# evfro/polara

Hardware: AMD Instinct MI355X
Metric: users scored/sec + SVD build time, ML-20M rank-50 PureSVD (higher is better)
Workload: dtype bf16x3

## Files before the change

include/polara_hip.h:

```cpp
#ifndef POLARA_HIP_H
#define POLARA_HIP_H

#include <stdint.h>

#ifdef __cplusplus
extern "C" {
#endif

#define PK_OK 0
#define PK_E_INVALID (-1)
#define PK_E_LAUNCH (-2)
#define PK_E_UNSUPPORTED (-3)
#define PK_E_NOCONV (-4)

#define PK_VAL_F32 0
#define PK_VAL_F64 1

const char *pk_last_error(void);
int pk_version(void);
int pk_set_option(const char *name, int32_t value, int32_t unset);
int pk_copy_to_host_async(void *stream, void *dst_host, const void *src_dev, int64_t bytes);
int pk_device_info(int device, char *name, int name_len, int *cu_count, int64_t *hbm_bytes);
int pk_warm_up(void);

// ... 5 lines not shown
                    const int32_t *indices_dev, const void *vals_dev, int val_kind,
                    const double *X_dev, int64_t ldx, int32_t nc,
                    double *out_dev, int64_t ldo, double *partial_dev );
int pk_spmm_csr_x(void *stream,
                  int64_t n_tasks, const int32_t *task_row_dev, const int64_t *task_begin_dev,
                  const int64_t *task_end_dev, const int32_t *task_slot_dev,
                  int64_t n_long, const int32_t *long_row_dev, const int32_t *long_slot_begin_dev,
                  const int32_t *long_slot_end_dev,
                  const int32_t *indices_dev, const void *vals_dev, int val_kind,
                  const void *X_dev, int x_kind, int64_t ldx, int32_t nc,
                  double *out_dev, int64_t ldo, double *partial_dev);
int pk_spmm_csr_ex(void *stream,
                   int64_t n_tasks, const int32_t *task_row_dev, const int64_t *task_begin_dev,
                   const int64_t *task_end_dev, const int32_t *task_slot_dev,
                   int64_t n_long, const int32_t *long_row_dev, const int32_t *long_slot_begin_dev,
                   const int32_t *long_slot_end_dev,
                   const int32_t *indices_dev, const void *vals_dev, int val_kind,
                   const void *X_dev, int x_kind, int64_t ldx, int32_t nc,
                   double *out_dev, int64_t ldo, double *partial_dev, int64_t row_base, int32_t accumulate,
                   int64_t x_rows );

int64_t pk_scan_work_bytes(int64_t n);
int pk_exclusive_scan_i32(void *stream, int64_t n, const int32_t *in_dev, int64_t *out_dev, void *work_dev);
int64_t pk_radix_work_bytes(int64_t n);
int pk_radix_sort_pairs(void *stream, int64_t n, int32_t key_bytes, void *keys_dev, uint32_t *vals_dev,
                        void *keys_tmp_dev, uint32_t *vals_tmp_dev, int32_t key_bits, void *work_dev,
                        int32_t *result_in_tmp);
int64_t pk_row_norm_order_work_bytes(int64_t n);
int pk_row_norm_order_f64(void *stream, int64_t n, int32_t K, const double *V_dev, int64_t ldv, int32_t *order_dev,
                          int32_t *rank_dev, double *V_sorted_dev, void *work_dev);
int64_t pk_coo_to_csr_work_bytes(int64_t nnz);
int pk_coo_to_csr(void *stream, int64_t nnz, const int64_t *rows_dev, const int64_t *cols_dev, int64_t idx_stride,
                  const void *vals_dev,
                  int val_kind, int64_t n_rows, int64_t n_cols, int64_t *indptr_dev, int32_t *indices_dev,
                  void *values_dev, int64_t *n_unique_dev, int32_t *err_dev, void *work_dev);
int64_t pk_csr_transpose_work_bytes(int64_t nnz);
int pk_csr_transpose(void *stream, int64_t n_rows, int64_t n_cols, int64_t nnz, const int64_t *indptr_dev,
                     const int32_t *indices_dev, const void *values_dev, int val_kind, int64_t rows_per_block,
                     int64_t *t_indptr_dev, int32_t *t_indices_dev, void *t_values_dev, void *work_dev);
int64_t pk_csr_relabel_work_bytes(int64_t nnz);
int pk_csr_relabel_sorted(void *stream, int64_t n_rows, int64_t n_cols, int64_t nnz, const int64_t *indptr_dev,
                          const int32_t *indices_dev, const void *values_dev, int val_kind, const int32_t *col_map_dev,
                          int32_t *indices_out_dev, void *values_out_dev, void *work_dev);
int64_t pk_csr_rows_by_length_work_bytes(int64_t n_rows);
int pk_csr_rows_by_length(void *stream, int64_t n_rows, int64_t nnz, const int64_t *indptr_dev, const int32_t *indices_dev,
                          const void *values_dev, int val_kind, int32_t *perm_out_dev, int64_t *new_indptr_dev,
                          int32_t *indices_out_dev, void *values_out_dev, void *work_dev);
int pk_count_i32(void *stream, int64_t n, const int32_t *keys_dev, int64_t n_bins, int32_t *counts_dev);
int pk_csr_scale_f64(void *stream, int64_t n_rows, const int64_t *indptr_dev, const int32_t *indices_dev, const void *vals_dev,
                     int val_kind, const double *row_scale_dev, const double *col_scale_dev, double *vals_out_dev);
int64_t pk_row_plan_work_bytes(int64_t n_rows);
int pk_row_plan_count(void *stream, int64_t n_rows, const int64_t *indptr_dev, int32_t split, int64_t *counts_dev,
                      void *work_dev);
int pk_row_plan_fill(void *stream, int64_t n_rows, const int64_t *indptr_dev, const void *work_dev,
                     int32_t *task_row_dev, int64_t *task_begin_dev, int64_t *task_end_dev, int32_t *task_slot_dev,
                     int32_t *long_row_dev, int32_t *long_slot_begin_dev, int32_t *long_slot_end_dev,
                     int64_t *row_first_task_dev, int64_t *row_long_index_dev);

int64_t pk_gram_work_bytes(int64_t n, int32_t la, int32_t lb);
int pk_gram_f64(void *stream, int64_t n, int32_t la, int32_t lb, const double *A_dev, int64_t lda,
                const double *B_dev, int64_t ldb, double *G_dev, int64_t ldg, void *work_dev);
int pk_tsmm_f64(void *stream, int64_t n, int32_t lin, int32_t lout, const double *X_dev, int64_t ldx,
                const double *C_dev, int64_t ldc, double *out_dev, int64_t ldo);
int pk_tsmm_sub_f64(void *stream, int64_t n, int32_t lin, int32_t lout, const double *X_dev, int64_t ldx,
                    const double *C_dev, int64_t ldc, const double *Z_dev, int64_t ldz, double *out_dev, int64_t ldo);
int pk_tsmm_axpby_f64(void *stream, int64_t n, int32_t lin, int32_t lout, const double *X_dev, int64_t ldx,
                      const double *C_dev, int64_t ldc, double alpha, double beta, const double *Z1_dev, int64_t ldz1,
                      double gamma, const double *Z2_dev, int64_t ldz2, double *out_dev, int64_t ldo);
int pk_orth_check_f64(void *stream, int32_t l, const double *G_dev, int64_t ldg, int32_t *info_dev, int32_t n_info,
                      double *flags_dev);
int pk_eigh_psd_f64(void *stream, int32_t n, double *S_dev, int64_t lds_, double *evecs_dev, int64_t ldv,
                    double *evals_dev, int32_t max_sweeps, double tol, int32_t *info_dev);
int pk_eigh_psd_rounds_f64(void *stream, int32_t n, double *S_dev, int64_t lds_, double *evecs_dev, int64_t ldv,
                           double *evals_dev, int32_t max_sweeps, double tol, int32_t *info_dev);
int pk_eigh_top_supported(int32_t n, int32_t r);
int64_t pk_eigh_top_work_bytes(int32_t n);
int pk_eigh_top_f64(void *stream, int32_t n, const double *S_dev, int64_t lds_, int32_t r, double *evecs_dev, int64_t ldv,
                    double *evals_dev, void *work_dev, int32_t *info_dev);
int64_t pk_chol_work_bytes(int32_t n);
int pk_chol_rinv_f64(void *stream, int32_t n, const double *G_dev, int64_t ldg, double shift_rel, double *Rinv_dev,
                     int64_t ldr, void *work_dev, int32_t *info_dev);
int pk_chol_rinv_scaled_f64(void *stream, int32_t n, const double *G_dev, int64_t ldg, double shift_rel, double *Rinv_dev,
                     int64_t ldr, void *work_dev, int32_t *info_dev);
int pk_axpbypcz_f64(void *stream, int64_t n_elems, double alpha, const double *Z_dev, double beta,
                    const double *Y_dev, double gamma, const double *X_dev, double *out_dev);
int32_t pk_resid_blocks(int64_t n);
int pk_resid_colnorm2_f64(void *stream, int64_t n, int32_t l, const double *Z_dev, int64_t ldz,
                          const double *X_dev, int64_t ldx, const double *theta_dev, double *partial_dev);
int pk_dgemm_small_f64(void *stream, int transA, int transB, int32_t M, int32_t N, int32_t K,
                       const double *A_dev, int64_t lda, const double *B_dev, int64_t ldb,
                       double *C_dev, int64_t ldc);
int pk_scale_cols_f64(void *stream, int64_t n, int32_t l, double *X_dev, int64_t ldx, const double *s_dev);

int64_t pk_pack_elems(int64_t n, int32_t K);
int32_t pk_pack_kq(int32_t K);
int pk_pack_frag_f32(void *stream, int64_t n, int32_t K, const double *src_dev, int64_t ld, float *dst_dev);
int32_t pk_candidate_capacity(int32_t topk);
int64_t pk_score_state_bytes(int64_t n_users, int32_t splits);
int32_t pk_score_splits(int64_t n_users, int32_t KC);
int pk_seen_tiles_build(void *stream, int64_t n_users, const int64_t *seen_ptr_dev, const int32_t *seen_idx_dev,
                        int32_t rows_sorted ,
                        int64_t max_row_len ,
                        uint64_t *tiles_dev, int32_t *ntiles_dev);
int32_t pk_seen_tiles_max_unsorted_row(void);
int pk_score_candidates_f32(void *stream, int64_t n_users, int64_t n_items, int32_t K,
                            const float *Vp_dev, const float *Ep_dev,
                            const int64_t *seen_ptr_dev, const uint64_t *seen_tiles_dev,
                            const int32_t *seen_ntiles_dev ,
                            int32_t KC, int32_t splits ,
                            float *cand_score_dev, int32_t *cand_idx_dev ,
                            void *state_dev ,
                            int32_t tiles_per_chunk ,
                            const float *user_bound_dev ,
                            const float *tile_bound_dev ,
                            const uint32_t *seen_dense_dev, const int32_t *seen_skip_dev,
                            int32_t dense_tiles );
int pk_sweep_takes_rows(void);
int pk_score_candidates_rows_f32(void *stream, int64_t n_users, int64_t n_items, int32_t K, const float *Vp_dev,
                                 const double *E_dev, int64_t lde, const double *extra_dev, int64_t extra_ld,
                                 double extra_scale, const int64_t *seen_ptr_dev, const uint64_t *seen_tiles_dev,
                                 const int32_t *seen_ntiles_dev, int32_t KC, int32_t splits, float *cand_score_dev,
                                 int32_t *cand_idx_dev, void *state_dev, int32_t tiles_per_chunk ,
                                 const float *tile_bound_dev , const uint32_t *seen_dense_dev,
                                 const int32_t *seen_skip_dev, int32_t dense_tiles);
int pk_score_two_phase_plan(int64_t n_users, int64_t n_items, int32_t KC, int32_t *head_tiles, int32_t *splits);
int pk_score_two_phase_f32(void *stream, int64_t n_users, int64_t n_items, int32_t K,
                           const float *Vp_dev, const float *Ep_dev,
                           const int64_t *seen_ptr_dev, const uint64_t *seen_tiles_dev, const int32_t *seen_ntiles_dev,
                           int32_t KC, int32_t head_tiles, int32_t splits ,
                           float *work_score_dev, int32_t *work_idx_dev, float *cand_score_dev, int32_t *cand_idx_dev,
                           void *state_dev, int32_t tiles_per_chunk ,
                           const float *user_bound_dev, const float *tile_bound_dev ,
                           const uint32_t *seen_dense_dev, const int32_t *seen_skip_dev, int32_t dense_tiles);
int pk_score_two_phase_rows_f32(void *stream, int64_t n_users, int64_t n_items, int32_t K, const float *Vp_dev,
                                const double *E_dev, int64_t lde, const double *extra_dev, int64_t extra_ld,
                                double extra_scale, const int64_t *seen_ptr_dev, const uint64_t *seen_tiles_dev,
                                const int32_t *seen_ntiles_dev, int32_t KC, int32_t head_tiles, int32_t splits,
                                float *work_score_dev, int32_t *work_idx_dev, float *cand_score_dev, int32_t *cand_idx_dev,
                                void *state_dev, int32_t tiles_per_chunk, const float *tile_bound_dev,
                                const uint32_t *seen_dense_dev, const int32_t *seen_skip_dev, int32_t dense_tiles);
int64_t pk_seen_dense_bytes(int64_t n_users, int32_t dense_tiles);
int pk_seen_dense_build(void *stream, int64_t n_users, const int64_t *seen_ptr_dev, const uint64_t *seen_tiles_dev,
                        const int32_t *seen_ntiles_dev, int32_t dense_tiles, uint32_t *dense_dev, int32_t *skip_dev);
int32_t pk_score_chunk_launches(int64_t n_items, int32_t K, int32_t splits, int32_t tiles_per_chunk, int32_t pruned);
int pk_row_norm_bound_f32(void *stream, int64_t n, int32_t K, const double *src_dev, int64_t ld, float *out_dev);
int pk_v32_image_f32(void *stream, int64_t n, int32_t K, int32_t ld32, const double *V_dev, int64_t ldv, const float *bound_dev,
                     float *out_dev, uint32_t *stat_dev);
int pk_pack_frag_bound_f32(void *stream, int64_t n, int32_t K, const double *src_dev, int64_t ld, float *dst_dev,
                           float *bound_dev, const double *extra_dev, int64_t extra_ld, double extra_scale);
int pk_tile_norm_bound_f32(void *stream, int64_t n_items, int32_t K, const double *V_dev, int64_t ld,
                           float *work_dev, float *out_dev);
int pk_rescore_topk_f64(void *stream, int64_t n_users, int64_t n_items, int32_t K,
                        const double *V_dev, int64_t ldv, const double *E_dev, int64_t lde,
                        const int64_t *seen_ptr_dev, int32_t KC, int32_t splits,
                        const float *cand_score_dev, const int32_t *cand_idx_dev, int32_t topk,
                        double v_row_norm_max,
                        int64_t *out_idx_dev, double *out_score_dev , int32_t *flags_dev);
int pk_rescore_topk_rows_f64(void *stream, int64_t n_rows, const int32_t *rows_dev,
                             const int32_t *n_rows_dev ,
                             int64_t n_users, int64_t n_items,
                             int32_t K, const double *V_dev, int64_t ldv,
                             const float *V32_dev , int64_t ldv32,
                             const double *E_dev, int64_t lde,
                             const double *e_err_dev, int64_t e_err_ld ,
                             int32_t e_exact ,
                             const int64_t *seen_ptr_dev, int32_t KC, int32_t splits,
// ... 212 lines not shown
```

polara_amd/_lib.py:

```python
import ctypes as C
import os

_HERE = os.path.dirname(os.path.abspath(__file__))
LIB_PATH = os.environ.get('POLARA_HIP_LIB') or os.path.join(_HERE, 'libpolarahip.so')

PK_VAL_F32, PK_VAL_F64 = 0, 1

_vp, _i32, _i64, _f64 = C.c_void_p, C.c_int32, C.c_int64, C.c_double

PROTOTYPES = {
    'pk_last_error': (C.c_char_p, []),
    'pk_version': (C.c_int, []),
    'pk_warm_up': (C.c_int, []),
    'pk_device_info': (C.c_int, [C.c_int, C.c_char_p, C.c_int, C.POINTER(C.c_int), C.POINTER(_i64)]),
    'pk_spmm_csr_f64': (C.c_int, [_vp, _i64, _vp, _vp, _vp, _vp, _i64, _vp, _vp, _vp, _vp, _vp, C.c_int,
                                  _vp, _i64, _i32, _vp, _i64, _vp]),
    'pk_spmm_csr_x': (C.c_int, [_vp, _i64, _vp, _vp, _vp, _vp, _i64, _vp, _vp, _vp, _vp, _vp, C.c_int,
                                _vp, C.c_int, _i64, _i32, _vp, _i64, _vp]),
    'pk_spmm_csr_ex': (C.c_int, [_vp, _i64, _vp, _vp, _vp, _vp, _i64, _vp, _vp, _vp, _vp, _vp, C.c_int,
                                 _vp, C.c_int, _i64, _i32, _vp, _i64, _vp, _i64, _i32, _i64]),
    'pk_scan_work_bytes': (_i64, [_i64]),
    'pk_exclusive_scan_i32': (C.c_int, [_vp, _i64, _vp, _vp, _vp]),
    'pk_radix_work_bytes': (_i64, [_i64]),
    'pk_radix_sort_pairs': (C.c_int, [_vp, _i64, _i32, _vp, _vp, _vp, _vp, _i32, _vp, C.POINTER(_i32)]),
# ... 45 lines not shown
                                              _vp, _vp, _vp, _vp, _vp, _i32, _vp, _vp, _vp, _i32]),
    'pk_score_two_phase_plan': (C.c_int, [_i64, _i64, _i32, _vp, _vp]),
    'pk_score_two_phase_f32': (C.c_int, [_vp, _i64, _i64, _i32, _vp, _vp, _vp, _vp, _vp, _i32, _i32, _i32, _vp, _vp, _vp, _vp, _vp,
                                         _i32, _vp, _vp, _vp, _vp, _i32]),
    'pk_seen_dense_bytes': (_i64, [_i64, _i32]),
    'pk_seen_dense_build': (C.c_int, [_vp, _i64, _vp, _vp, _vp, _i32, _vp, _vp]),
    'pk_score_chunk_launches': (_i32, [_i64, _i32, _i32, _i32, _i32]),
    'pk_pack_frag_bound_f32': (C.c_int, [_vp, _i64, _i32, _vp, _i64, _vp, _vp, _vp, _i64, _f64]),
    'pk_row_norm_bound_f32': (C.c_int, [_vp, _i64, _i32, _vp, _i64, _vp]),
    'pk_tile_norm_bound_f32': (C.c_int, [_vp, _i64, _i32, _vp, _i64, _vp, _vp]),
    'pk_rescore_topk_f64': (C.c_int, [_vp, _i64, _i64, _i32, _vp, _i64, _vp, _i64, _vp, _i32, _i32, _vp, _vp,
                                      _i32, _f64, _vp, _vp, _vp]),
    'pk_flag_compact': (C.c_int, [_vp, _i64, _vp, _i32, _vp, _vp]),
    'pk_fold_rows_f64': (C.c_int, [_vp, _i64, _vp, _vp, _i64, _vp, _vp, _vp, C.c_int, _vp, _i64, _i32, _vp, _i64]),
    'pk_spmm_csr_flagged_f64': (C.c_int, [_vp, _i64, _vp, _vp, _vp, _vp, _i64, _vp, _vp, _vp, _vp, _vp, C.c_int, _vp, _i64, _i32,
                                          _vp, _i64, _vp, _i64, _vp, _i32]),
    'pk_spmm_csr_rows_list_f64': (C.c_int, [_vp, _i64, _vp, _vp, _i64, _vp, _vp, _vp, _vp, _vp, _i64, _vp, _vp, _vp, _vp, _vp, C.c_int,
                                            _vp, _i64, _i32, _vp, _i64, _vp, _i64, _vp, _i32]),
    'pk_q20_lanes': (_i32, [_i32]),
    'pk_q20_kappa': (_f64, [_i32]),
    'pk_q20_image_bytes': (_i64, [_i64, _i32]),
    'pk_q20_encode_f64': (C.c_int, [_vp, _i64, _i32, _vp, _i64, _vp, _vp, _vp, _vp]),
    'pk_q20_decode_f64': (C.c_int, [_vp, _i64, _i32, _vp, _vp, _vp, _i64]),
    'pk_fold_q20': (C.c_int, [_vp, _i64, _vp, _vp, _vp, _vp, _i64, _vp, _vp, _vp, _vp, _vp, C.c_int, _vp, _vp, _i64, _i32, _i32,
                              _vp, _i64, _vp]),
    'pk_rescore_topk_rows_f64': (C.c_int, [_vp, _i64, _vp, _vp, _i64, _i64, _i32, _vp, _i64, _vp, _i64, _vp, _i64, _vp, _i64, _i32, _vp, _i32, _i32,
                                           _vp, _vp, _i32, _f64, _vp, _vp, _vp]),
    'pk_rescore_topk_rows_list_f64': (C.c_int, [_vp, _i64, _vp, _vp, _i64, _i64, _i32, _vp, _i64, _vp, _i64, _vp, _i64, _vp, _i64, _i32, _vp, _i32, _i32,
                                           _vp, _vp, _i32, _f64, _vp, _vp, _vp, _vp, _vp, _i32]),
    'pk_rescore_topk_rows_norms_f64': (C.c_int, [_vp, _i64, _vp, _vp, _i64, _i64, _i32, _vp, _i64, _vp, _i64, _vp, _i64, _vp, _i64, _i32, _vp, _i32, _i32,
                                           _vp, _vp, _i32, _f64, _vp, _vp, _vp, _vp, _vp, _i32, _vp]),
    'pk_zero_i32': (C.c_int, [_vp, _vp, _i32]),
    'pk_scatter_rows_i64': (C.c_int, [_vp, _i64, _i32, _vp, _vp, _vp]),
    'pk_map_ids_i64': (C.c_int, [_vp, _i64, _vp, _vp, _i64, _vp]),
    'pk_exact_work_bytes': (_i64, [_i32, _i64]),
    'pk_score_exact_rows_f64': (C.c_int, [_vp, _i32, _vp, _i64, _i32, _vp, _i64, _vp, _i64, _vp, _vp, _i32,
                                          _vp, _vp, _vp]),
    'pk_score_exact_list_f64': (C.c_int, [_vp, _i32, _vp, _vp, _i64, _i32, _vp, _i64, _vp, _i64, _vp, _vp, _i32,
                                          _vp, _vp, _vp]),
    'pk_eval_ranks': (C.c_int, [_vp, _i64, _vp, _i32, _vp, _vp, _vp]),
    'pk_eval_cols': (_i32, []),
    'pk_eval_user_metrics': (C.c_int, [_vp, _i64, _i32, _vp, _i64, _vp, _vp, _vp, _vp, _f64, _f64, _i32, _vp]),
    'pk_eval_reduce_work_bytes': (_i64, [_i64]),
    'pk_eval_reduce': (C.c_int, [_vp, _i64, _vp, _vp, _vp]),
    'pk_unique_count_i64': (C.c_int, [_vp, _i64, _vp, _i64, _vp, _vp]),
    'pk_dense_scores_f64': (C.c_int, [_vp, _i32, _i64, _i32, _vp, _i64, _vp, _i64, _vp, _i64]),
    'pk_topk_rows_f64': (C.c_int, [_vp, _i64, _i64, _vp, _i64, _i32, _vp]),
    'pk_i2i_max_topk': (_i32, []),
    'pk_i2i_window': (_i32, []),
    'pk_i2i_build_window': (_i32, []),
    'pk_i2i_ld': (_i64, [_i64]),
    'pk_i2i_chunk_users': (_i64, [_i64, _i64, _i32]),
    'pk_i2i_topk_work_bytes': (_i64, [_i64, _i64, _i32]),
    'pk_i2i_build_f64': (C.c_int, [_vp, _i64, _i64, _vp, _vp, _vp, C.c_int, _vp, _vp, _vp, _vp, _i64]),
    'pk_i2i_image_f32': (C.c_int, [_vp, _i64, _vp, _vp, _vp]),
    'pk_i2i_topk': (C.c_int, [_vp, _i64, _i64, _vp, _vp, _vp, C.c_int, _vp, C.c_int, _i64, _i32, _i32, _i32, _vp, _vp, _vp]),
    'pk_popular_order_work_bytes': (_i64, [_i64]),
    'pk_popular_order': (C.c_int, [_vp, _i64, _vp, _vp, _vp]),
    'pk_popular_topk': (C.c_int, [_vp, _i64, _i64, _vp, _vp, _vp, _i32, _i32, _vp]),
    'pk_hybrid_ld': (_i64, [_i64]),
    'pk_hybrid_max_nc': (_i32, []),
    'pk_trmm_work_bytes': (_i64, [_i64, _i32]),
    'pk_hybrid_densify_f64': (C.c_int, [_vp, _i64, _vp, _vp, _vp, _vp, _f64, _vp, _i64]),
    'pk_chol_f64': (C.c_int, [_vp, _i64, _vp, _i64, _vp]),
    'pk_trmm_f64': (C.c_int, [_vp, _i32, _i64, _i32, _vp, _i64, _vp, _i64, _vp, _i64, _vp]),
    'pk_trsm_f64': (C.c_int, [_vp, _i64, _i32, _vp, _i64, _vp, _i64]),
    'pk_lce_fused_max_rank': (_i32, []),
    'pk_lce_update_f64': (C.c_int, [_vp, _i64, _i32, _vp, _i64, _vp, _i64, _vp, _i64, _f64, _vp, _i64, _f64, _f64, _f64, _vp]),
    'pk_lce_update_ew_f64': (C.c_int, [_vp, _i64, _i32, _vp, _i64, _vp, _i64, _vp, _i64, _f64, _f64, _vp]),
    'pk_lce_dot_blocks': (_i32, [_i64]),
    'pk_lce_dots_work_bytes': (_i64, []),
    'pk_lce_dots_f64': (C.c_int, [_vp, _i32, _vp, _vp, _vp, _vp, _vp, _vp, _vp, _vp, _f64, _vp, _vp]),
    'pk_clamp_min_f64': (C.c_int, [_vp, _i64, _i32, _vp, _i64, _f64]),
    'pk_ctx_create': (C.c_int, [_i32, C.POINTER(_vp)]),
    'pk_ctx_destroy': (None, [_vp]),
    'pk_ctx_error': (C.c_char_p, [_vp]),
    'pk_mat_from_csr': (C.c_int, [_vp, _i64, _i64, _i64, _vp, _vp, _vp, _i32, C.POINTER(_vp)]),
    'pk_mat_from_coo': (C.c_int, [_vp, _i64, _i64, _i64, _vp, _vp, _i64, _vp, _i32, C.POINTER(_vp)]),
    'pk_mat_free': (None, [_vp, _vp]),
    'pk_mat_nnz': (_i64, [_vp]),
    'pk_svd_build': (C.c_int, [_vp, _vp, _i32, _i32, _f64, _i32, C.c_uint64, _vp, _vp, _vp, _vp]),
    'pk_sym_eig_topk_f64': (C.c_int, [_vp, _vp, _i32, _vp, _i64, _i32, _i32, _vp, _i64, _i32, _f64, _i32, C.c_uint64,
                                      _vp, _i64, _vp, _vp, _vp, _vp, _f64]),
    'pk_svd_build_sharded': (C.c_int, [_vp, _vp, _vp, _i32, _i32, _f64, _i32, C.c_uint64, _vp, _vp, _vp, _vp]),
    'pk_ctx_stream': (_vp, [_vp]),
    'pk_ctx_set_option': (C.c_int, [_vp, C.c_char_p, _i32]),
    'pk_set_option': (C.c_int, [C.c_char_p, _i32, _i32]),
    'pk_copy_to_host_async': (C.c_int, [_vp, _vp, _vp, _i64]),
    'pk_v32_image_f32': (C.c_int, [_vp, _i64, _i32, _i32, _vp, _i64, _vp, _vp, _vp]),
    'pk_row_norm_order_work_bytes': (_i64, [_i64]),
    'pk_row_norm_order_f64': (C.c_int, [_vp, _i64, _i32, _vp, _i64, _vp, _vp, _vp, _vp]),
    'pk_sweep_takes_rows': (C.c_int, []),
    'pk_ctx_spmm_timings': (_i64, [_vp, _vp, _vp, _i64]),
    'pk_mat_wrap_device': (C.c_int, [_vp, _vp, _i64, _i64, _i64, _vp, _vp, _vp, _i32, _i32, C.POINTER(_vp)]),
    'pk_lanczos_steps': (C.c_int, [_vp, _vp, _vp, _i32, _i32, _i32, _i32, _vp, _i64, _vp, _i64, _vp, _vp, _i32]),
    'pk_gramian_apply_f64': (C.c_int, [_vp, _vp, _vp, _i32, _vp, _i64, _vp, _i64]),
    'pk_lanczos_products': (C.c_int, [_vp, _vp, _vp, _i32, _i32, _vp, _i64, _vp, _i32]),
    'pk_lanczos_orth': (C.c_int, [_vp, _vp, _i64, _i32, _i32, _i32, _vp, _i64, _vp, _i64, _vp, _vp, _vp, _i32]),
    'pk_score_topk': (C.c_int, [_vp, _i64, _i32, _vp, _vp, _i32, _i32, _vp, _vp]),
    'pk_serving_create': (C.c_int, [_vp, _i64, _i32, _vp, _vp, C.POINTER(_vp)]),
    'pk_serving_score': (C.c_int, [_vp, _vp, _i32, _i32, _vp, _vp]),
    'pk_serving_free': (None, [_vp, _vp]),
    'pk_hooi': (C.c_int, [_vp, _i64, _vp, _vp, _vp, _vp, _i32, _f64, _vp, _vp, C.c_uint64, _vp, _vp, _vp, _vp, _vp, _vp]),
    'pk_ttm_f64': (C.c_int, [_vp, _i64, _vp, _vp, _vp, _vp, _i64, _vp, _vp, _vp, _vp, _vp, _vp,
                             _vp, _i64, _i32, _vp, _i64, _i32, _vp, _i64, _vp]),
    'pk_tucker_predict_f64': (C.c_int, [_vp, _i64, _vp, _vp, _vp, _i64, _vp, _i64, _vp, _i64, _vp, _i32, _i32, _i32, _i32, _vp, _vp]),
}


class PolaraHipError(RuntimeError):
    pass


_lib = None


def load():
    global _lib
    if _lib is not None:
        return _lib
    import torch
    if not os.path.exists(LIB_PATH):
        raise PolaraHipError(
            'libpolarahip.so is not built (%s). Run `python -m polara_amd.build_native` '
            '(needs hipcc; cross-compiles for gfx950 without a GPU). There is no CPU fallback.' % LIB_PATH)
    lib = C.CDLL(LIB_PATH)
    for name, (res, args) in PROTOTYPES.items():
        fn = getattr(lib, name)
        fn.restype = res
        fn.argtypes = args
    _lib = lib
    return lib


def check(rc, what='', lib=None, ctx=None):
    if rc != 0:
        lib = lib or load()
        msg = lib.pk_ctx_error(ctx) if ctx is not None else None
        msg = msg or lib.pk_last_error()
        raise PolaraHipError('%s failed (rc=%d): %s' % (what, rc, msg.decode() if msg else ''))


def device_info(device=0):
    lib = load()
    name = C.create_string_buffer(64)
    cu = C.c_int(0)
    mem = C.c_int64(0)
    n = lib.pk_device_info(device, name, 64, C.byref(cu), C.byref(mem))
    if n <= 0:
        check(n, 'pk_device_info')
    return dict(n_devices=n, arch=name.value.decode(), cu_count=cu.value, hbm_bytes=mem.value)
```

polara_amd/csrc/api.cpp:

```cpp
#include "pk_common.h"
#include <string.h>

static thread_local char g_err[512] = "";

void pk_set_error(const char *fmt, ...) {
    va_list ap;
    va_start(ap, fmt);
    vsnprintf(g_err, sizeof(g_err), fmt, ap);
    va_end(ap);
}

extern "C" const char *pk_last_error(void) { return g_err; }

#include <atomic>
namespace {
struct Option { const char *name; std::atomic<int> value; std::atomic<bool> set; };
Option g_options[] = {{"score_boot_tiles", {0}, {false}}, {"score_head_tiles", {0}, {false}}, {"score_phase2_splits", {0}, {false}}};
}
int pk_option(const char *name, int dflt) {
    for (auto &o : g_options)
        if (!strcmp(o.name, name)) return o.set.load() ? o.value.load() : dflt;
    return dflt;
}
extern "C" int pk_set_option(const char *name, int32_t value, int32_t unset) {
    if (name)
        for (auto &o : g_options)
            if (!strcmp(o.name, name)) {
                o.value.store(value);
                o.set.store(!unset);
                return PK_OK;
            }
    pk_set_error("pk_set_option: unknown option '%s'", name ? name : "(null)");
    return PK_E_INVALID;
}
extern "C" int pk_version(void) { return 100; }

extern "C" int pk_copy_to_host_async(void *stream, void *dst_host, const void *src_dev, int64_t bytes) {
    if (bytes < 0 || (bytes > 0 && (!dst_host || !src_dev))) {
        pk_set_error("pk_copy_to_host_async: bad arguments");
        return PK_E_INVALID;
    }
    if (bytes == 0) return PK_OK;
    const hipError_t e = hipMemcpyAsync(dst_host, src_dev, (size_t)bytes, hipMemcpyDeviceToHost, static_cast<hipStream_t>(stream));
    if (e != hipSuccess) {
        pk_set_error("pk_copy_to_host_async: %s", hipGetErrorString(e));
        return PK_E_LAUNCH;
    }
    return PK_OK;
}

extern "C" int pk_device_info(int device, char *name, int name_len, int *cu_count, int64_t *hbm_bytes) {
    int n = 0;
    hipError_t e = hipGetDeviceCount(&n);
    if (e != hipSuccess || n <= 0) {
        pk_set_error("pk_device_info: no HIP device visible (%s)", hipGetErrorString(e));
        return PK_E_LAUNCH;
    }
    if (device < 0 || device >= n) {
        pk_set_error("pk_device_info: device %d out of range [0,%d)", device, n);
        return PK_E_INVALID;
    }
    hipDeviceProp_t prop;
    e = hipGetDeviceProperties(&prop, device);
    if (e != hipSuccess) {
        pk_set_error("pk_device_info: %s", hipGetErrorString(e));
        return PK_E_LAUNCH;
    }
    if (name && name_len > 0) {
        strncpy(name, prop.gcnArchName, name_len - 1);
        name[name_len - 1] = 0;
    }
    if (cu_count) *cu_count = prop.multiProcessorCount;
    if (hbm_bytes) *hbm_bytes = (int64_t)prop.totalGlobalMem;
    return n;
}

hipError_t pk_tu_load_dense();
hipError_t pk_tu_load_driver();
hipError_t pk_tu_load_eigh();
hipError_t pk_tu_load_eigh_top();
hipError_t pk_tu_load_evalmetrics();
hipError_t pk_tu_load_hybrid();
hipError_t pk_tu_load_i2i();
hipError_t pk_tu_load_foldq();
hipError_t pk_tu_load_ingest();
hipError_t pk_tu_load_lce();
hipError_t pk_tu_load_rescore();
hipError_t pk_tu_load_score();
hipError_t pk_tu_load_spmm();
hipError_t pk_tu_load_ttm();

extern "C" int pk_warm_up(void) {
    hipError_t (*const loaders[])() = {pk_tu_load_dense, pk_tu_load_driver, pk_tu_load_eigh, pk_tu_load_eigh_top, pk_tu_load_evalmetrics, pk_tu_load_foldq, pk_tu_load_hybrid, pk_tu_load_i2i, pk_tu_load_ingest, pk_tu_load_lce, pk_tu_load_rescore, pk_tu_load_score, pk_tu_load_spmm, pk_tu_load_ttm};
    for (auto f : loaders) {
        const hipError_t e = f();
        if (e != hipSuccess) {
            pk_set_error("pk_warm_up: %s", hipGetErrorString(e));
            return PK_E_LAUNCH;
        }
    }
    return PK_OK;
}
```

polara_amd/csrc/dense.hip:

```cpp
#include "pk_common.h"

static int gram_splits(int64_t n, int la, int lb) {
    int64_t tiles = pk_ceil_div(la, 64) * pk_ceil_div(lb, 64);
    int64_t s = pk_ceil_div(tiles >= 4 ? 1024 : 2048, tiles);
    int64_t max_by_rows = pk_ceil_div(n, 64);
    if (s > max_by_rows) s = max_by_rows;
    if (s > 1024) s = 1024;
    if (n <= 64) s = 1;
    if (s < 1) s = 1;
    return (int)s;
}

extern "C" int64_t pk_gram_work_bytes(int64_t n, int32_t la, int32_t lb) {
    return (int64_t)gram_splits(n, la, lb) * la * lb * (int64_t)sizeof(double);
}

typedef double f64x4 __attribute__((ext_vector_type(4)));

__global__ __launch_bounds__(256) void gram_kernel(int64_t n, int la, int lb, const double *__restrict__ A,
                                                   int64_t lda, const double *__restrict__ B, int64_t ldb,
                                                   double *__restrict__ partial, int tiles_j,
                                                   int64_t rows_per_split) {
    constexpr int RT = 32;
    __shared__ __attribute__((aligned(16))) double sA[RT][64];
    __shared__ __attribute__((aligned(16))) double sB[RT][64];
    const int tid = threadIdx.x;
    const int lane = tid & 63, wave = tid >> 6;
    const int ti = blockIdx.x / tiles_j, tj = blockIdx.x % tiles_j;
    const int split = blockIdx.y;
    const int64_t r_begin = (int64_t)split * rows_per_split;
    int64_t r_end = r_begin + rows_per_split;
    if (r_end > n) r_end = n;
    const bool vec = ((lda | ldb) & 1) == 0 && ((((uintptr_t)A) | ((uintptr_t)B)) & 15) == 0 && (la & 1) == 0 && (lb & 1) == 0;
    f64x4 acc[4];
#pragma unroll
    for (int b = 0; b < 4; ++b) acc[b] = f64x4{0.0, 0.0, 0.0, 0.0};
    double2 ra[4], rb[4];
    auto fetch = [&](int64_t r0) {
#pragma unroll
        for (int q = 0; q < 4; ++q) {
            const int slot = tid + 256 * q;
            const int rr = slot >> 5, c = (slot & 31) * 2;
            const int64_t row = r0 + rr;
            const int ca = ti * 64 + c, cb = tj * 64 + c;
            double2 va = make_double2(0.0, 0.0), vb = make_double2(0.0, 0.0);
            if (row < r_end) {
                const double *pa = A + row * lda + ca, *pb = B + row * ldb + cb;
                if (vec && ca + 1 < la) va = *reinterpret_cast<const double2 *>(pa);
                else {
                    if (ca < la) va.x = pa[0];
                    if (ca + 1 < la) va.y = pa[1];
                }
                if (vec && cb + 1 < lb) vb = *reinterpret_cast<const double2 *>(pb);
                else {
                    if (cb < lb) vb.x = pb[0];
                    if (cb + 1 < lb) vb.y = pb[1];
                }
            }
            ra[q] = va;
            rb[q] = vb;
        }
    };
    if (r_begin < r_end) fetch(r_begin);
    for (int64_t r0 = r_begin; r0 < r_end; r0 += RT) {
#pragma unroll
        for (int q = 0; q < 4; ++q) {
            const int slot = tid + 256 * q;
            *reinterpret_cast<double2 *>(&sA[slot >> 5][(slot & 31) * 2]) = ra[q];
            *reinterpret_cast<double2 *>(&sB[slot >> 5][(slot & 31) * 2]) = rb[q];
        }
        __syncthreads();
        if (r0 + RT < r_end) fetch(r0 + RT);
#pragma unroll
        for (int k0 = 0; k0 < RT; k0 += 4) {
            const double p = sA[k0 + (lane >> 4)][16 * wave + (lane & 15)];
#pragma unroll
            for (int b = 0; b < 4; ++b)
                acc[b] = __builtin_amdgcn_mfma_f64_16x16x4f64(p, sB[k0 + (lane >> 4)][16 * b + (lane & 15)], acc[b], 0, 0, 0);
        }
        __syncthreads();
    }
    double *dst = partial + (int64_t)split * la * lb;
#pragma unroll
// ... 286 lines not shown
                acc = fma(d, d, acc);
            }
        }
        red[tid] = acc;
        __syncthreads();
        for (int s = nrl / 2; s > 0; s >>= 1) {
            if (rl < s) red[tid] += red[tid + s * cw];
            __syncthreads();
        }
        if (rl == 0 && j < l) partial[(int64_t)blockIdx.x * l + j] = red[tid];
        __syncthreads();
    }
}

extern "C" int pk_resid_colnorm2_f64(void *stream, int64_t n, int32_t l, const double *Z_dev, int64_t ldz,
                                     const double *X_dev, int64_t ldx, const double *theta_dev,
                                     double *partial_dev) {
    PK_REQUIRE(n >= 1 && l >= 1 && ldz >= l && ldx >= l, "pk_resid_colnorm2_f64: bad sizes");
    hipLaunchKernelGGL(resid_colnorm2_kernel, dim3((unsigned)pk_resid_blocks(n)), dim3(256), 0, pk_stream(stream),
                       n, l, Z_dev, ldz, X_dev, ldx, theta_dev, partial_dev);
    PK_CHECK_LAUNCH("resid_colnorm2_kernel");
    return PK_OK;
}

__global__ __launch_bounds__(256) void scale_cols_kernel(int64_t n, int l, double *__restrict__ X, int64_t ldx,
                                                         const double *__restrict__ s) {
    int64_t e = (int64_t)blockIdx.x * blockDim.x + threadIdx.x;
    const int64_t total = n * l, stride = (int64_t)gridDim.x * blockDim.x;
    for (; e < total; e += stride) {
        int64_t i = e / l;
        int j = (int)(e % l);
        X[i * ldx + j] *= s[j];
    }
}

extern "C" int pk_scale_cols_f64(void *stream, int64_t n, int32_t l, double *X_dev, int64_t ldx,
                                 const double *s_dev) {
    PK_REQUIRE(n >= 1 && l >= 1 && ldx >= l, "pk_scale_cols_f64: bad sizes");
    int64_t blocks = pk_ceil_div(n * l, 256);
    if (blocks > 8192) blocks = 8192;
    hipLaunchKernelGGL(scale_cols_kernel, dim3((unsigned)blocks), dim3(256), 0, pk_stream(stream), n, l, X_dev, ldx,
                       s_dev);
    PK_CHECK_LAUNCH("scale_cols_kernel");
    return PK_OK;
}

__global__ __launch_bounds__(256) void dgemm_small_kernel(int tA, int tB, int M, int N, int K,
                                                          const double *__restrict__ A, int64_t lda,
                                                          const double *__restrict__ B, int64_t ldb,
                                                          double *__restrict__ C, int64_t ldc) {
    int64_t e = (int64_t)blockIdx.x * blockDim.x + threadIdx.x;
    if (e >= (int64_t)M * N) return;
    const int i = (int)(e / N), j = (int)(e % N);
    double acc = 0.0;
    for (int k = 0; k < K; ++k) {
        double a = tA ? A[(int64_t)k * lda + i] : A[(int64_t)i * lda + k];
        double b = tB ? B[(int64_t)j * ldb + k] : B[(int64_t)k * ldb + j];
        acc = fma(a, b, acc);
    }
    C[(int64_t)i * ldc + j] = acc;
}

extern "C" int pk_dgemm_small_f64(void *stream, int transA, int transB, int32_t M, int32_t N, int32_t K,
                                  const double *A_dev, int64_t lda, const double *B_dev, int64_t ldb,
                                  double *C_dev, int64_t ldc) {
    PK_REQUIRE(M >= 1 && N >= 1 && K >= 1 && ldc >= N, "pk_dgemm_small_f64: bad sizes");
    hipLaunchKernelGGL(dgemm_small_kernel, dim3((unsigned)pk_ceil_div((int64_t)M * N, 256)), dim3(256), 0,
                       pk_stream(stream), transA, transB, M, N, K, A_dev, lda, B_dev, ldb, C_dev, ldc);
    PK_CHECK_LAUNCH("dgemm_small_kernel");
    return PK_OK;
}

#define PK_CHOL_LDS_MAX 136
#define PK_CHOL_THREADS 1024
template <bool IN_LDS, bool SCALED = false>
__global__ __launch_bounds__(PK_CHOL_THREADS) void chol_rinv_kernel(int n, const double *__restrict__ G, int64_t ldg,
                                                                    double shift_rel, double *__restrict__ Rinv,
                                                                    int64_t ldr, double *__restrict__ work,
                                                                    int32_t *__restrict__ info, int tx_log2) {
    extern __shared__ double chol_lds[];
    __shared__ double s_shift;
    double *A = IN_LDS ? chol_lds : work;
    const int ld = IN_LDS ? n + 1 : n;
    const int tid = threadIdx.x;
    const int TX = 1 << tx_log2, TY = (int)blockDim.x >> tx_log2;
    const int tx = tid & (TX - 1), ty = tid >> tx_log2;
    if (tid < 64) {
        double tr = 0.0;
        for (int i = tid; i < n; i += 64) tr += SCALED ? 1.0 : G[(int64_t)i * ldg + i];
        for (int o = 32; o > 0; o >>= 1) tr += __shfl_xor(tr, o);
        if (tid == 0) s_shift = shift_rel * tr;
    }
    __syncthreads();
    const double shift = s_shift;
    for (int i = ty; i < n; i += TY)
        for (int c = tx; c < n; c += TX) {
            double g = (c >= i) ? G[(int64_t)i * ldg + c] : 0.0;
            if constexpr (SCALED) {
                const double gi = G[(int64_t)i * ldg + i], gc = G[(int64_t)c * ldg + c];
                g = (c > i) ? g / (sqrt(gi) * sqrt(gc)) : (c == i ? (gi > 0.0 ? 1.0 : -1.0) : 0.0);
            }
            A[i * ld + c] = (c > i) ? g : (c == i ? g + shift : 0.0);
        }
    int fail = 0;
    for (int j = 0; j < n; ++j) {
        __syncthreads();
        const double d = A[j * ld + j];
        if (!(d > 0.0)) {
            fail = j + 1;
            break;
        }
        const double invd = 1.0 / d;
        for (int c = tx; c < n; c += TX) {
            const double pj = (c == j) ? 1.0 : A[j * ld + c];
            for (int i = j + 1 + ty; i < n; i += TY)
                if (c <= j || c >= i) {
                    const double f = A[j * ld + i] * invd;
                    A[i * ld + c] = fma(-f, pj, A[i * ld + c]);
                }
        }
    }
    __syncthreads();
    if (tid == 0) info[0] = fail;
    if (fail) return;
    for (int k = ty; k < n; k += TY)
        for (int c = tx; c < n; c += TX) {
            double v = 0.0;
            if (c >= k) {
                const double rs = 1.0 / sqrt(A[c * ld + c]);
                v = (c == k) ? rs : A[c * ld + k] * rs;
                if constexpr (SCALED) v /= sqrt(G[(int64_t)k * ldg + k]);
            }
            Rinv[(int64_t)k * ldr + c] = v;
        }
}

extern "C" int64_t pk_chol_work_bytes(int32_t n) { return (n > PK_CHOL_LDS_MAX) ? (int64_t)n * n * 8 : 0; }

static int chol_rinv_launch(void *stream, int32_t n, const double *G_dev, int64_t ldg, double shift_rel, double *Rinv_dev, int64_t ldr,
                            void *work_dev, int32_t *info_dev, bool scaled);

extern "C" int pk_chol_rinv_f64(void *stream, int32_t n, const double *G_dev, int64_t ldg, double shift_rel,
                                double *Rinv_dev, int64_t ldr, void *work_dev, int32_t *info_dev) {
    return chol_rinv_launch(stream, n, G_dev, ldg, shift_rel, Rinv_dev, ldr, work_dev, info_dev, false);
}

extern "C" int pk_chol_rinv_scaled_f64(void *stream, int32_t n, const double *G_dev, int64_t ldg, double shift_rel,
                                       double *Rinv_dev, int64_t ldr, void *work_dev, int32_t *info_dev) {
    return chol_rinv_launch(stream, n, G_dev, ldg, shift_rel, Rinv_dev, ldr, work_dev, info_dev, true);
}

static int chol_rinv_launch(void *stream, int32_t n, const double *G_dev, int64_t ldg, double shift_rel, double *Rinv_dev, int64_t ldr,
                            void *work_dev, int32_t *info_dev, bool scaled) {
    PK_REQUIRE(n >= 1 && n <= 1024 && ldg >= n && ldr >= n, "pk_chol_rinv_f64: bad sizes");
    PK_REQUIRE(G_dev && Rinv_dev && info_dev && (n <= PK_CHOL_LDS_MAX || work_dev), "pk_chol_rinv_f64: bad pointers");
    static PkDeviceOnce attr_set;   
    if (attr_set.pending()) {
        hipError_t e1 = hipFuncSetAttribute(reinterpret_cast<const void *>(&chol_rinv_kernel<true, false>),
                                            hipFuncAttributeMaxDynamicSharedMemorySize,
                                            PK_CHOL_LDS_MAX * (PK_CHOL_LDS_MAX + 1) * 8);
        if (e1 == hipSuccess)
            e1 = hipFuncSetAttribute(reinterpret_cast<const void *>(&chol_rinv_kernel<true, true>),
                                     hipFuncAttributeMaxDynamicSharedMemorySize, PK_CHOL_LDS_MAX * (PK_CHOL_LDS_MAX + 1) * 8);
        if (e1 != hipSuccess) {
            pk_set_error("pk_chol_rinv_f64: cannot raise the dynamic LDS limit: %s", hipGetErrorString(e1));
            return PK_E_LAUNCH;
        }
        attr_set.done();   
    }
    int tx_log2 = 4;
    while ((1 << tx_log2) < n && tx_log2 < 8) ++tx_log2;
    const int threads = PK_CHOL_THREADS;
#define PK_CHOL_LAUNCH(SC)                                                                                                   \
    do {                                                                                                                     \
        if (n <= PK_CHOL_LDS_MAX)                                                                                            \
            hipLaunchKernelGGL((chol_rinv_kernel<true, SC>), dim3(1), dim3(threads), (size_t)n * (n + 1) * sizeof(double),   \
                               pk_stream(stream), n, G_dev, ldg, shift_rel, Rinv_dev, ldr, static_cast<double *>(work_dev),  \
                               info_dev, tx_log2);                                                                           \
        else                                                                                                                 \
            hipLaunchKernelGGL((chol_rinv_kernel<false, SC>), dim3(1), dim3(PK_CHOL_THREADS), 0, pk_stream(stream), n, G_dev, \
                               ldg, shift_rel, Rinv_dev, ldr, static_cast<double *>(work_dev), info_dev, tx_log2);           \
    } while (0)
    if (scaled) PK_CHOL_LAUNCH(true); else PK_CHOL_LAUNCH(false);
#undef PK_CHOL_LAUNCH
    PK_CHECK_LAUNCH("chol_rinv_kernel");
    return PK_OK;
}

hipError_t pk_tu_load_dense() {
    hipFuncAttributes a;
    return hipFuncGetAttributes(&a, reinterpret_cast<const void *>(&gram_reduce_kernel));
}
```

polara_amd/csrc/driver.hip:

```cpp
#include "pk_common.h"
#include <algorithm>
#include <cmath>
#include <cstdarg>
#include <cstring>
#include <map>
#include <memory>
#include <mutex>
#include <numeric>
#include <random>
#include <string>
#include <type_traits>
#include <vector>

namespace model {
constexpr double kDenseF64Flops = 20e12;
constexpr double kLanczosStepFixedS = 0.3e-3;
constexpr double kNestedSolveS = 1.5e-3;
constexpr double kXgmiBusBps = 100e9;
constexpr double kCollectiveStepS = 5e-6;
}

struct DevPool {
    std::multimap<size_t, void *> free_blocks;
    void *get(size_t &bytes) {
        auto it = free_blocks.lower_bound(bytes);
        if (it != free_blocks.end() && it->first <= bytes + bytes / 4 + 4096) {
            void *p = it->second;
            bytes = it->first;
            free_blocks.erase(it);
            return p;
        }
        void *p = nullptr;
        if (hipMalloc(&p, bytes) != hipSuccess) {
            trim();
            if (hipMalloc(&p, bytes) != hipSuccess) return nullptr;
        }
        return p;
    }
    void put(void *p, size_t bytes) { free_blocks.emplace(bytes, p); }
    void trim() {
        for (auto &kv : free_blocks) (void)hipFree(kv.second);
        free_blocks.clear();
    }
};

struct CtxOptions {
    int svd_method = 0;
    int krylov_block = 0;
    int dist_overlap = 1;
    int hooi_ttm = 0;
    int time_spmm = 0;
};

struct SpmmTiming {
    hipEvent_t e0, e1;
    int64_t meta[6];
};

struct pk_ctx {
    int device = 0;
    hipStream_t stream = nullptr;
    std::mutex mu;
    std::string err;
    DevPool pool;
    CtxOptions opt;
    std::vector<SpmmTiming> spmm_timings;
    std::vector<hipEvent_t> event_pool;
};

static thread_local DevPool *g_pool = nullptr;
struct PoolScope {
    DevPool *prev;
    explicit PoolScope(pk_ctx *ctx) : prev(g_pool) { g_pool = &ctx->pool; }
    ~PoolScope() { g_pool = prev; }
};

namespace {

int fail(pk_ctx *ctx, int code, const char *fmt, ...) {
    char buf[512];
    va_list ap;
    va_start(ap, fmt);
    vsnprintf(buf, sizeof(buf), fmt, ap);
    va_end(ap);
    if (ctx) ctx->err = buf;
    pk_set_error("%s", buf);
    return code;
}
#define CK(call)                                                          \
    do {                                                                  \
        int rc_ = (call);                                                 \
        if (rc_ != PK_OK) {                                               \
            ctx->err = pk_last_error();                                   \
            return rc_;                                                   \
        }                                                                 \
    } while (0)
#define HIPCK(call)                                                                              \
    do {                                                                                         \
        hipError_t e_ = (call);                                                                  \
        if (e_ != hipSuccess) return fail(ctx, PK_E_LAUNCH, "%s: %s", #call, hipGetErrorString(e_)); \
    } while (0)

struct Dev {
    void *p = nullptr;
    size_t bytes = 0;
    size_t cap = 0;
    DevPool *pool = nullptr;
    bool borrowed = false;
    Dev() {}
    explicit Dev(size_t b) { alloc(b); }
    Dev(const Dev &) = delete;
    Dev &operator=(const Dev &) = delete;
    Dev(Dev &&o) noexcept : p(o.p), bytes(o.bytes), cap(o.cap), pool(o.pool), borrowed(o.borrowed) { o.p = nullptr; o.bytes = o.cap = 0; o.borrowed = false; }
    Dev &operator=(Dev &&o) noexcept {
        if (this != &o) {
            release();
            p = o.p; bytes = o.bytes; cap = o.cap; pool = o.pool; borrowed = o.borrowed; o.p = nullptr; o.bytes = o.cap = 0; o.borrowed = false;
        }
        return *this;
    }
    void borrow(const void *ptr, size_t b) {
        release();
        p = const_cast<void *>(ptr); bytes = b; cap = 0; pool = nullptr; borrowed = true;
    }
    ~Dev() { release(); }
    bool alloc(size_t b) {
        release();
        bytes = b;
        if (b == 0) return true;
        pool = g_pool;
        cap = ((b + 65535) / 65536) * 65536;
        if (pool) p = pool->get(cap);
        else if (hipMalloc(&p, cap) != hipSuccess) p = nullptr;
        if (!p) { bytes = cap = 0; return false; }
// ... 430 lines not shown
        const int nb = pk_resid_blocks(Z.n);
        Dev part((size_t)nb * Z.l * 8);
        if (!part.p) return fail(ctx, PK_E_LAUNCH, "out of device memory (resid)");
        CK(pk_resid_colnorm2_f64(st, Z.n, Z.l, Z.p(), Z.l, X.p(), X.l, theta_dev.as<double>(), part.as<double>()));
        std::vector<double> h((size_t)nb * Z.l);
        CK(to_host(part.p, h.data(), h.size() * 8));
        res.assign((size_t)Z.l, 0.0);
        for (int b = 0; b < nb; ++b)
            for (int j = 0; j < Z.l; ++j) res[(size_t)j] += h[(size_t)b * Z.l + j];
        for (auto &v : res) v = std::sqrt(std::max(v, 0.0));
        return PK_OK;
    }
};

int cheb_degree(double theta_top, double b, double spread, int m_max) {
    if (b <= 0.0) return 2;
    const double x_top = 2.0 * theta_top / b - 1.0;
    if (x_top <= 1.0 + 1e-12) return m_max;
    const int m = (int)(std::log(2.0 * spread) / std::acosh(x_top));
    return std::max(2, std::min(m_max, m));
}

int upload_csr(pk_ctx *ctx, Csr &M, int64_t n_rows, int64_t n_cols, int64_t nnz, const int64_t *indptr, const int32_t *indices,
               const void *values, int val_kind) {
    M.n_rows = n_rows; M.n_cols = n_cols; M.nnz = nnz; M.val_kind = val_kind;
    const size_t ve = val_kind == PK_VAL_F32 ? 4 : 8;
    if (!M.indptr.alloc((size_t)(n_rows + 1) * 8) || !M.indices.alloc((size_t)std::max<int64_t>(nnz, 1) * 4) ||
        !M.values.alloc((size_t)std::max<int64_t>(nnz, 1) * ve))
        return fail(ctx, PK_E_LAUNCH, "out of device memory (matrix)");
    HIPCK(hipMemcpyAsync(M.indptr.p, indptr, (size_t)(n_rows + 1) * 8, hipMemcpyHostToDevice, ctx->stream));
    if (nnz) {
        HIPCK(hipMemcpyAsync(M.indices.p, indices, (size_t)nnz * 4, hipMemcpyHostToDevice, ctx->stream));
        HIPCK(hipMemcpyAsync(M.values.p, values, (size_t)nnz * ve, hipMemcpyHostToDevice, ctx->stream));
    }
    HIPCK(hipStreamSynchronize(ctx->stream));
    return PK_OK;
}

}

extern "C" int pk_ctx_create(int32_t device, pk_ctx **out) {
    if (!out) return PK_E_INVALID;
    int n = 0;
    if (hipGetDeviceCount(&n) != hipSuccess || device < 0 || device >= n) {
        pk_set_error("pk_ctx_create: device %d not available (%d visible)", device, n);
        return PK_E_LAUNCH;
    }
    auto *ctx = new pk_ctx();
    ctx->device = device;
    if (hipSetDevice(device) != hipSuccess || hipStreamCreate(&ctx->stream) != hipSuccess) {
        delete ctx;
        pk_set_error("pk_ctx_create: cannot create a stream on device %d", device);
        return PK_E_LAUNCH;
    }
    if (pk_warm_up() != PK_OK) {
        (void)hipStreamDestroy(ctx->stream);
        delete ctx;
        return PK_E_LAUNCH;
    }
    *out = ctx;
    return PK_OK;
}

extern "C" void pk_ctx_destroy(pk_ctx *ctx) {
    if (!ctx) return;
    for (auto &t : ctx->spmm_timings) { (void)hipEventDestroy(t.e0); (void)hipEventDestroy(t.e1); }
    for (hipEvent_t e : ctx->event_pool) (void)hipEventDestroy(e);
    ctx->spmm_timings.clear();
    ctx->event_pool.clear();
    (void)hipSetDevice(ctx->device);
    (void)hipStreamSynchronize(ctx->stream);
    ctx->pool.trim();
    (void)hipStreamDestroy(ctx->stream);
    delete ctx;
}

extern "C" const char *pk_ctx_error(pk_ctx *ctx) { return ctx ? ctx->err.c_str() : "null context"; }

extern "C" int pk_ctx_set_option(pk_ctx *ctx, const char *name, int32_t value) {
    if (!ctx || !name) return PK_E_INVALID;
    std::lock_guard<std::mutex> lock(ctx->mu);
    struct { const char *name; int *slot; int lo, hi; } table[] = {
        {"svd_method", &ctx->opt.svd_method, 0, 2},   {"krylov_block", &ctx->opt.krylov_block, 0, 1024},
        {"dist_overlap", &ctx->opt.dist_overlap, 0, 2}, {"hooi_ttm", &ctx->opt.hooi_ttm, 0, 1}, {"time_spmm", &ctx->opt.time_spmm, 0, 1}};
    for (auto &e : table)
        if (!strcmp(name, e.name)) {
            if (value < e.lo || value > e.hi) return fail(ctx, PK_E_INVALID, "pk_ctx_set_option: %s takes %d..%d", name, e.lo, e.hi);
            *e.slot = value;
            return PK_OK;
        }
    return fail(ctx, PK_E_INVALID, "pk_ctx_set_option: unknown option '%s'", name);
}

extern "C" int64_t pk_ctx_spmm_timings(pk_ctx *ctx, double *ms_out, int64_t *meta_out, int64_t cap) {
    if (!ctx) return -1;
    std::lock_guard<std::mutex> lock(ctx->mu);
    (void)hipSetDevice(ctx->device);
    const int64_t count = (int64_t)ctx->spmm_timings.size();
    for (int64_t i = 0; i < count; ++i) {
        SpmmTiming &t = ctx->spmm_timings[(size_t)i];
        float ms = 0.f;
        (void)hipEventSynchronize(t.e1);
        (void)hipEventElapsedTime(&ms, t.e0, t.e1);
        if (i < cap && ms_out && meta_out) {
            ms_out[i] = (double)ms;
            for (int q = 0; q < 6; ++q) meta_out[6 * i + q] = t.meta[q];
        }
        ctx->event_pool.push_back(t.e0);
        ctx->event_pool.push_back(t.e1);
    }
    ctx->spmm_timings.clear();
    return count;
}

extern "C" int pk_mat_from_csr(pk_ctx *ctx, int64_t n_rows, int64_t n_cols, int64_t nnz, const int64_t *indptr,
                               const int32_t *indices, const void *values, int32_t val_kind, pk_mat **out) {
    if (!ctx || !out) return PK_E_INVALID;
    std::lock_guard<std::mutex> lock(ctx->mu);
    PoolScope pool_scope(ctx);
    (void)hipSetDevice(ctx->device);
    if (n_rows < 1 || n_cols < 1 || nnz < 0 || !indptr || (nnz && (!indices || !values)) ||
        (val_kind != PK_VAL_F32 && val_kind != PK_VAL_F64))
        return fail(ctx, PK_E_INVALID, "pk_mat_from_csr: bad arguments");
    if (indptr[0] != 0 || indptr[n_rows] != nnz) return fail(ctx, PK_E_INVALID, "pk_mat_from_csr: indptr does not span [0, nnz]");
    for (int64_t p = 0; p < nnz; ++p)
        if (indices[p] < 0 || indices[p] >= n_cols) return fail(ctx, PK_E_INVALID, "pk_mat_from_csr: column index out of bounds");
    auto m = std::make_unique<pk_mat>();
    int rc = upload_csr(ctx, m->A, n_rows, n_cols, nnz, indptr, indices, values, val_kind);
    if (rc != PK_OK) return rc;
    m->nonneg = true;
    if (val_kind == PK_VAL_F32) { const float *v = static_cast<const float *>(values); for (int64_t p = 0; p < nnz; ++p) if (v[p] < 0) { m->nonneg = false; break; } }
    else { const double *v = static_cast<const double *>(values); for (int64_t p = 0; p < nnz; ++p) if (v[p] < 0) { m->nonneg = false; break; } }
    rc = build_plan(ctx, m->A);
    if (rc != PK_OK) return rc;
    *out = m.release();
    return PK_OK;
}

static int mat_from_coo_impl(pk_ctx *ctx, int64_t n_rows, int64_t n_cols, int64_t nnz, const int64_t *rows, const int64_t *cols,
                             int64_t idx_stride, const void *values, int32_t val_kind, pk_mat **out);

extern "C" int pk_mat_from_coo(pk_ctx *ctx, int64_t n_rows, int64_t n_cols, int64_t nnz, const int64_t *rows, const int64_t *cols,
                               int64_t idx_stride, const void *values, int32_t val_kind, pk_mat **out) {
    if (!ctx || !out) return PK_E_INVALID;
    std::lock_guard<std::mutex> lock(ctx->mu);
    PoolScope pool_scope(ctx);
    (void)hipSetDevice(ctx->device);
    return mat_from_coo_impl(ctx, n_rows, n_cols, nnz, rows, cols, idx_stride, values, val_kind, out);
}

static int mat_from_coo_impl(pk_ctx *ctx, int64_t n_rows, int64_t n_cols, int64_t nnz, const int64_t *rows, const int64_t *cols,
                             int64_t idx_stride, const void *values, int32_t val_kind, pk_mat **out) {
    if (n_rows < 1 || n_cols < 1 || nnz < 0 || idx_stride < 1 || (nnz && (!rows || !cols || !values)) ||
        (val_kind != PK_VAL_F32 && val_kind != PK_VAL_F64))
        return fail(ctx, PK_E_INVALID, "pk_mat_from_coo: bad arguments");
    hipStream_t st = ctx->stream;
    const size_t ve = val_kind == PK_VAL_F32 ? 4 : 8, n1 = (size_t)std::max<int64_t>(nnz, 1);
    const bool interleaved = idx_stride == 2 && cols == rows + 1;
    Dev idx(interleaved ? n1 * 16 : n1 * 16), vals(n1 * ve), info(16), work((size_t)pk_coo_to_csr_work_bytes(nnz));
    auto m = std::make_unique<pk_mat>();
    Csr &A = m->A;
    A.n_rows = n_rows; A.n_cols = n_cols; A.val_kind = val_kind;
    if (!idx.p || !vals.p || !info.p || !work.p || !A.indptr.alloc((size_t)(n_rows + 1) * 8) || !A.indices.alloc(n1 * 4) || !A.values.alloc(n1 * ve))
        return fail(ctx, PK_E_LAUNCH, "out of device memory (pk_mat_from_coo)");
    const int64_t *r_dev, *c_dev;
    int64_t stride_dev;
    if (nnz) {
// ... 200 lines not shown
        return 2.0 * (comm->world - 1) / comm->world * (double)A->A.n_cols * l * 8.0 / model::kXgmiBusBps >= 4e-4;
    }
    int ritz(const DMat &X, DMat &H, DMat &Y) {
        Y = DMat(A->A.n_rows, X.l);
        if (!Y.ok()) return fail(ctx, PK_E_LAUNCH, "out of device memory (Rayleigh-Ritz)");
        CK(spmm_full(ctx, A->A, X, Y));
        CK(S.gram(Y, Y, H));
        return allreduce(H);
    }
    int rotate(const DMat &Y, const DMat &Cm, DMat &Z) {
        DMat Yr;
        CK(S.tsmm(Y, Cm, Yr));
        Z = DMat(A->A.n_cols, Yr.l);
        if (!Z.ok()) return fail(ctx, PK_E_LAUNCH, "out of device memory (Rayleigh-Ritz)");
        CK(spmm_t(ctx, A, Yr, Z));
        ++steps;
        return allreduce(Z);
    }
    int apply_rounded(const DMat &Xb, DMat &Z) {
        if (comm || Xb.l % 4 != 0) return apply(Xb, Z);
        const int64_t nr = A->A.n_rows, nc = A->A.n_cols;
        const int l = Xb.l;
        Dev X32((size_t)nc * l * 4), Y32((size_t)nr * l * 4);
        DMat Y(nr, l);
        Z = DMat(nc, l);
        if (!X32.p || !Y32.p || !Y.ok() || !Z.ok()) return fail(ctx, PK_E_LAUNCH, "out of device memory (rounded gramian step)");
        hipLaunchKernelGGL(f64_to_f32_kernel, dim3((unsigned)((nc * l + 255) / 256)), dim3(256), 0, ctx->stream, nc * l, Xb.p(), X32.as<float>());
        CK(spmm(ctx, A->A, X32.p, PK_VAL_F32, l, l, Y.p(), l, Range{0, A->A.plan.n_tasks, 0, A->A.plan.n_long}));
        hipLaunchKernelGGL(f64_to_f32_kernel, dim3((unsigned)((nr * l + 255) / 256)), dim3(256), 0, ctx->stream, nr * l, Y.p(), Y32.as<float>());
        for (int64_t bk = 0; bk < A->n_blocks; ++bk) {
            const int64_t shape3[3] = {bk == 0 ? nc : 0, A->rows_per_block, A->block_nnz[(size_t)bk]};
            CK(spmm(ctx, *A->Tb, Y32.p, PK_VAL_F32, l, l, Z.p(), l, A->block_ranges[(size_t)bk], bk * nc, bk > 0, shape3));
        }
        ++steps;
        return PK_OK;
    }
    int apply(const DMat &Xb, DMat &Z) {
        DMat Y(A->A.n_rows, Xb.l);
        if (!Y.ok()) return fail(ctx, PK_E_LAUNCH, "out of device memory (gramian step)");
        CK(spmm_full(ctx, A->A, Xb, Y));
        ++steps;
        if (!split_product(Xb.l)) {
            Z = DMat(A->A.n_cols, Xb.l);
            if (!Z.ok()) return fail(ctx, PK_E_LAUNCH, "out of device memory (gramian step)");
            CK(spmm_t(ctx, A, Y, Z));
            return allreduce(Z);
        }
        if (!side) {
            HIPCK(hipStreamCreateWithFlags(&side, hipStreamNonBlocking));
            HIPCK(hipEventCreateWithFlags(&ev_panel, hipEventDisableTiming));
            HIPCK(hipEventCreateWithFlags(&ev_summed, hipEventDisableTiming));
        }
        const int w0 = Xb.l / 2, w1 = Xb.l - w0;
        DMat Z0(A->A.n_cols, w0), Z1(A->A.n_cols, w1);
        if (!Z0.ok() || !Z1.ok()) return fail(ctx, PK_E_LAUNCH, "out of device memory (gramian step panels)");
        auto rest = [&]() -> int {
            CK(spmm_t_cols(ctx, A, Y, 0, w0, Z0));
            HIPCK(hipEventRecord(ev_panel, ctx->stream));
            HIPCK(hipStreamWaitEvent(side, ev_panel, 0));
            CK(allreduce(Z0, side));
            CK(spmm_t_cols(ctx, A, Y, w0, w1, Z1));
            CK(allreduce(Z1));
            HIPCK(hipEventRecord(ev_summed, side));
            HIPCK(hipStreamWaitEvent(ctx->stream, ev_summed, 0));
            CK(S.hcat(&Z0, Z1, Z));
            return PK_OK;
        };
        const int rc = rest();
        if (rc != PK_OK) {
            (void)hipStreamSynchronize(side);
            (void)hipStreamSynchronize(ctx->stream);
            return rc;
        }
        ++overlapped_panels;
        return PK_OK;
    }
};

struct DenseOp {
    pk_ctx *ctx;
    Solver &S;
    const DMat &T;
    int products = 0;
    int apply(const DMat &X, DMat &Z) {
        ++products;
        return S.tsmm(T, X, Z);
    }
    int filter_step(const DMat &Yc, double a, double b, double c, const DMat &Xc, DMat &Yn) {
        ++products;
        return S.tsmm_axpby(T, Yc, a, b, &Yc, c, &Xc, Yn);
    }
    int ritz(const DMat &X, DMat &H, DMat &Z) {
        DMat G;
        CK(apply(X, Z));
        CK(S.gram(X, Z, G));
        H = DMat(G.l, G.l);
        if (!H.ok()) return fail(ctx, PK_E_LAUNCH, "out of device memory (Rayleigh-Ritz)");
        hipLaunchKernelGGL(symmetrize_kernel, dim3((unsigned)((G.l * G.l + 255) / 256)), dim3(256), 0, S.st, G.l, G.p(), H.p());
        return PK_OK;
    }
    int rotate(const DMat &Z, const DMat &Cm, DMat &out) { return S.tsmm(Z, Cm, out); }
};

static int dense_topk_segments(pk_ctx *ctx, Solver &S, DenseOp &dop, int k, DMat &X, double tol, const double *lam0, double r0_rel,
                               SubspaceOut &out, bool &ok) {
    ok = false;
    const int l = X.l;
    const int64_t N = X.n;
    const double spread = 1e7, u = 1.1102230246251565e-16;
    const int m_max = 24;
    std::vector<double> lam, res;
    DMat Zr;
    auto ritz = [&]() -> int {
        DMat H, Z, Cm, Xr;
        Dev theta_dev;
        CK(dop.ritz(X, H, Z));
        CK(S.eigh(H, lam, Cm, theta_dev));
        CK(S.tsmm(X, Cm, Xr));
        CK(S.tsmm(Z, Cm, Zr));
        CK(S.resid(Zr, Xr, theta_dev, res));
        X = std::move(Xr);
        out.outer += 1;
        return PK_OK;
    };
    auto worst_of = [&]() {
        double w = 0.0;
        const double lam1 = std::max(lam.empty() ? 0.0 : lam[0], 1e-300);
        for (int j = 0; j < k && j < (int)res.size(); ++j) w = std::max(w, res[(size_t)j] / lam1);
        return w;
    };
    double worst = 1e-2;
    bool have_z = false;
    if (lam0) {
        lam.assign(lam0, lam0 + l);
        if (r0_rel >= 0) worst = std::max(r0_rel, tol);
    } else {
        CK(ritz());
        have_z = true;
        worst = worst_of();
        if (worst <= tol) {
            out.lam_all = lam; out.res_act = res; out.n_lock = 0; out.converged = true;
            out.basis = std::move(X);
            ok = true;
            return PK_OK;
        }
    }
    Dev chol_work((size_t)std::max<int64_t>(pk_chol_work_bytes(l), 8)), info(6 * 3 * 4);
    if (!chol_work.p || !info.p) return fail(ctx, PK_E_LAUNCH, "out of device memory (dense_topk_segments)");
    for (int round = 0; round < 10; ++round) {
        const double a0 = lam[0], bnd = lam[(size_t)l - 1];
        const double e = 0.5 * bnd, c = 0.5 * bnd;
        if (!(bnd > 0.0) || !(a0 > c) || k > l) return PK_OK;
        const int m = cheb_degree(a0, bnd, spread, m_max);
        const double xk = std::max(2.0 * lam[(size_t)std::min(k, l) - 1] / bnd - 1.0, 1.0 + 1e-9);
        const double amp = std::cosh(m * std::acosh(xk));
        const double need = std::max(worst / tol, 1.0) * 30.0;
        const int nseg = std::max(1, std::min(6, (int)std::ceil(std::log(need) / std::log(std::max(amp, 1.5)))));
        HIPCK(hipMemsetAsync(info.p, 0, 6 * 3 * 4, S.st));
        for (int seg = 0; seg < nseg; ++seg) {
            DMat Z, Yc, Xc;
            if (seg == 0 && have_z) Z = std::move(Zr); else CK(dop.apply(X, Z));
            have_z = false;
            double sigma = e / (a0 - c);
            const double tau = 2.0 / sigma;
            Xc = std::move(X);
            CK(S.axpbypcz(sigma / e, Z, -c * sigma / e, &Xc, 0.0, nullptr, Yc));
            for (int s2 = 2; s2 <= m; ++s2) {
                const double sigma_new = 1.0 / (tau - sigma);
                DMat Yn;
                CK(dop.filter_step(Yc, 2.0 * sigma_new / e, -2.0 * sigma_new * c / e, -sigma * sigma_new, Xc, Yn));
                Xc = std::move(Yc);
                Yc = std::move(Yn);
                sigma = sigma_new;
            }
            const int passes = (seg + 1 == nseg) ? 2 : 1;
            for (int p = 0; p < passes; ++p) {
                DMat G, Rinv(l, l), Yn;
                if (!Rinv.ok()) return fail(ctx, PK_E_LAUNCH, "out of device memory (dense_topk_segments)");
                CK(S.gram(Yc, Yc, G));
                if (p == 0)
                    CK(pk_chol_rinv_scaled_f64(S.st, l, G.p(), l, 11.0 * ((double)N * l + (double)l * (l + 1)) * u, Rinv.p(), l, chol_work.p,
                                               info.as<int32_t>() + 3 * seg + p));
                else
                    CK(pk_chol_rinv_f64(S.st, l, G.p(), l, 0.0, Rinv.p(), l, chol_work.p, info.as<int32_t>() + 3 * seg + p));
                CK(S.tsmm(Yc, Rinv, Yn));
                Yc = std::move(Yn);
            }
            X = std::move(Yc);
        }
        CK(ritz());
        have_z = true;
        int32_t verdicts[18];
        CK(S.to_host(info.p, verdicts, sizeof verdicts));
        bool broke = false;
        for (int32_t v : verdicts) broke = broke || v != 0;
        for (double v : lam) broke = broke || !(v == v);
        if (broke) {
            X = DMat();
            return PK_OK;
        }
        const double now = worst_of();
        if (now <= tol) {
            out.lam_all = lam; out.res_act = res; out.n_lock = 0; out.converged = true;
            out.basis = std::move(X);
            ok = true;
            return PK_OK;
        }
        if (round >= 1 && now > 0.5 * worst) return PK_OK;
        worst = now;
    }
    return PK_OK;
}

static int dense_topk(pk_ctx *ctx, Solver &S, DenseOp &dop, int k, DMat X, double tol, int max_outer, uint64_t seed, const double *lam0,
                      double r0_rel, SubspaceOut &out, bool cold = false) {
    std::vector<double> lam_cold;
    const int l = X.l;
    const int64_t N = X.n;
    if (cold && l <= 64 && N >= 2 * (int64_t)l) {
        const int w = 2 * l;
        DMat Tl(w, w), C2;
        Dev lam_dev;
        if (!Tl.ok()) return fail(ctx, PK_E_LAUNCH, "out of device memory (dense_topk)");
        HIPCK(hipMemcpy2DAsync(Tl.p(), (size_t)w * 8, dop.T.p(), (size_t)dop.T.l * 8, (size_t)w * 8, (size_t)w, hipMemcpyDeviceToDevice, S.st));
        std::vector<double> lam2;
        CK(S.eigh(Tl, lam2, C2, lam_dev));
        HIPCK(hipMemsetAsync(X.p(), 0, (size_t)N * l * 8, S.st));
        HIPCK(hipMemcpy2DAsync(X.p(), (size_t)l * 8, C2.p(), (size_t)w * 8, (size_t)l * 8, (size_t)w, hipMemcpyDeviceToDevice, S.st));
        lam_cold.assign(lam2.begin(), lam2.begin() + l);
        lam0 = lam_cold.data();
        r0_rel = -1.0;
        out.outer += 1;
    }
    DMat X0;
    CK(S.col_slice(X, 0, X.l, X0));
    bool ok = false;
    if (X.l <= 64) CK(dense_topk_segments(ctx, S, dop, k, X, tol, lam0, r0_rel, out, ok));
    if (ok) return PK_OK;
    const int outer0 = out.outer;
    SubspaceOut so;
    CK(subspace_iteration(ctx, S, dop, k, X.ok() && X.l == X0.l ? std::move(X) : std::move(X0), tol, max_outer, 24, 1e7, seed, false, so));
    so.outer += outer0;
    out = std::move(so);
    return PK_OK;
}

struct LanczosOut {
    DMat Vk;
    std::vector<double> lam_k, res_k;
    int steps = 0, looks = 0, nested_outer = 0, nested_products = 0;
    bool ok = false;
};

struct RitzLook {
    DMat basis, Yk;
    std::vector<double> lam_all, est;
    Dev lam_k_dev;
    double worst = 0.0;
    bool conv = false;
};

static int ritz_look(pk_ctx *ctx, Solver &S, const DMat &T, const DMat &Sc, const DMat *warm, const std::vector<double> *warm_lam, int k,
                     int b, int width, double est_tol, double prior, uint64_t seed, LanczosOut &lo, RitzLook &out) {
    const int N = (int)T.n;
    DMat X0;
    auto pad = [&](const DMat *src, int l) -> int {
        X0 = DMat(N, l);
        if (!X0.ok()) return fail(ctx, PK_E_LAUNCH, "out of device memory (ritz_look)");
        if (src) {
            HIPCK(hipMemsetAsync(X0.p(), 0, (size_t)N * l * 8, S.st));
            HIPCK(hipMemcpy2DAsync(X0.p(), (size_t)l * 8, src->p(), (size_t)src->l * 8, (size_t)l * 8, (size_t)src->n, hipMemcpyDeviceToDevice, S.st));
        } else {
            hipLaunchKernelGGL(unit_block_kernel, dim3((unsigned)(((int64_t)N * l + 255) / 256)), dim3(256), 0, S.st, (int64_t)N, l, X0.p());
        }
        return PK_OK;
    };
    CK(pad(warm, warm ? warm->l : std::min(N, std::max(b, width))));
    double t_in = std::max(0.3 * est_tol, prior < 0 ? 1e-4 : 0.03 * prior);
    bool first_pass = true;
    for (;;) {
        DenseOp dop{ctx, S, T};
        SubspaceOut so;
        const bool warm_pairs = warm && warm_lam && (int)warm_lam->size() == X0.l && prior >= 0;
        CK(dense_topk(ctx, S, dop, k, std::move(X0), t_in, 200, seed, warm_pairs ? warm_lam->data() : nullptr, warm_pairs ? prior : -1.0, so,
                      !warm && first_pass));
        warm_lam = nullptr;
        first_pass = false;
        lo.nested_outer += so.outer;
        lo.nested_products += dop.products;
        out.basis = std::move(so.basis);
        out.lam_all = so.lam_all;
        out.conv = so.converged;
        CK(S.col_slice(out.basis, 0, k, out.Yk));
        DMat TY;
        CK(S.gram(T, out.Yk, TY));
        if (!out.lam_k_dev.alloc((size_t)k * 8)) return fail(ctx, PK_E_LAUNCH, "out of device memory (ritz_look)");
        CK(S.upload(out.lam_all.data(), out.lam_k_dev.p, (size_t)k * 8));
        std::vector<double> r_in;
        CK(S.resid(TY, out.Yk, out.lam_k_dev, r_in));
        DMat yl(b, k), M(b, k);
        if (!yl.ok() || !M.ok()) return fail(ctx, PK_E_LAUNCH, "out of device memory (ritz_look)");
        HIPCK(hipMemcpyAsync(yl.p(), out.Yk.p() + (size_t)(N - b) * k, (size_t)b * k * 8, hipMemcpyDeviceToDevice, S.st));
        CK(pk_dgemm_small_f64(S.st, 0, 0, b, k, b, Sc.p(), b, yl.p(), k, M.p(), k));
        std::vector<double> hy((size_t)b * k), hm((size_t)b * k);
        CK(S.to_host(yl.p(), hy.data(), hy.size() * 8));
        CK(S.to_host(M.p(), hm.data(), hm.size() * 8));
        const double lam1 = std::max(out.lam_all.empty() ? 0.0 : out.lam_all[0], 1e-300);
        out.est.assign((size_t)k, 0.0);
        double cmax = 0.0;
        out.worst = 0.0;
        for (int j = 0; j < k; ++j) {
            double c2 = 0.0;
            for (int i = 0; i < b; ++i) c2 += hy[(size_t)i * k + j] * hm[(size_t)i * k + j];
            c2 = std::max(c2, 0.0);
            cmax = std::max(cmax, c2);
            out.est[(size_t)j] = std::sqrt(r_in[(size_t)j] * r_in[(size_t)j] + c2) / lam1;
            out.worst = std::max(out.worst, out.est[(size_t)j]);
        }
        const double coupling = std::sqrt(cmax) / lam1;
        if (t_in <= 0.3 * est_tol || coupling >= 4.0 * t_in || !out.conv) break;
        t_in = std::max(0.3 * est_tol, 0.1 * coupling);
        CK(pad(&out.basis, out.basis.l));
    }
    lo.looks += 1;
    return PK_OK;
}

__global__ void sym_block_kernel(int N, int ld, const double *__restrict__ T, double *__restrict__ out) {
    const int i = blockIdx.x * blockDim.x + threadIdx.x;
    if (i >= N * N) return;
    const int r = i / N, c = i - r * N;
    out[i] = 0.5 * (T[(int64_t)r * ld + c] + T[(int64_t)c * ld + r]);
}
__global__ void mirror_block_kernel(int rows, int b, int ldt, const double *__restrict__ C, double *__restrict__ T) {
    const int i = blockIdx.x * blockDim.x + threadIdx.x;
    if (i >= rows * b) return;
    const int r = i / b, c = i - r * b;
    T[(int64_t)(rows + c) * ldt + r] = C[i];
}
__global__ void band_block_kernel(int N, int b, int ldt, const double *__restrict__ C, double *__restrict__ T) {
    const int i = blockIdx.x * blockDim.x + threadIdx.x;
    if (i >= N * b) return;
    const int r = i / b, c = i - r * b;
    const bool in_band = r >= N - 2 * b;
    T[(int64_t)r * ldt + (N - b) + c] = in_band ? C[i] : 0.0;
    if (r < N - b) T[(int64_t)(N - b + c) * ldt + r] = in_band ? C[i] : 0.0;
}
__global__ void lanczos_flags_kernel(int l, const double *__restrict__ G, const int32_t *__restrict__ info, double *__restrict__ flags) {
    __shared__ double s_max[256];
    double m = 0.0;
    for (int i = threadIdx.x; i < l * l; i += blockDim.x) {
        const int r = i / l, c = i - r * l;
        const double d = fabs(G[i] - (r == c ? 1.0 : 0.0));
        m = (d == d) ? fmax(m, d) : 1.0;
    }
    s_max[threadIdx.x] = m;
    __syncthreads();
    for (int s = 128; s > 0; s >>= 1) {
        if ((int)threadIdx.x < s) s_max[threadIdx.x] = fmax(s_max[threadIdx.x], s_max[threadIdx.x + s]);
        __syncthreads();
    }
    if (threadIdx.x == 0) {
        flags[0] += (double)(abs(info[0]) + abs(info[1]) + abs(info[2]));
        flags[1] = fmax(flags[1], s_max[0]);
// ... 407 lines not shown
    if (!info.p || !chol_work.p) return fail(ctx, PK_E_LAUNCH, "out of device memory (pk_lanczos_orth)");
    DMat W = DMat::view(W_dev, n_items, b), Sc;
    CK(lanczos_orth(ctx, S, n_items, b, j, last_closes != 0, LanczosBuffers{Q_dev, ldq, T_dev, ldt, flags_dev, info.as<int32_t>(), chol_work.p}, W, Sc,
                    rounded != 0));
    HIPCK(hipMemcpyAsync(S_out_dev, Sc.p(), (size_t)b * b * 8, hipMemcpyDeviceToDevice, ctx->stream));
    return PK_OK;
}

extern "C" int pk_gramian_apply_f64(pk_ctx *ctx, void *stream, pk_mat *A, int32_t nc, const double *X_dev, int64_t ldx, double *Z_dev,
                                    int64_t ldz) {
    if (!ctx || !A) return PK_E_INVALID;
    std::lock_guard<std::mutex> lock(ctx->mu);
    PoolScope pool_scope(ctx);
    StreamScope stream_scope(ctx, stream);
    (void)hipSetDevice(ctx->device);
    if (nc < 1 || nc > 1024 || !X_dev || !Z_dev || ldx < nc || ldz < nc || !A->Tb)
        return fail(ctx, PK_E_INVALID, "pk_gramian_apply_f64: bad arguments (nc=%d)", nc);
    const int64_t n = A->A.n_cols;
    Solver S{ctx, ctx->stream, Dev()};
    GramianOp gop{ctx, S, A, nullptr};
    DMat X(n, nc), Z;
    if (!X.ok()) return fail(ctx, PK_E_LAUNCH, "out of device memory (pk_gramian_apply_f64)");
    HIPCK(hipMemcpy2DAsync(X.p(), (size_t)nc * 8, X_dev, (size_t)ldx * 8, (size_t)nc * 8, (size_t)n, hipMemcpyDeviceToDevice, ctx->stream));
    CK(gop.apply(X, Z));
    HIPCK(hipMemcpy2DAsync(Z_dev, (size_t)ldz * 8, Z.p(), (size_t)nc * 8, (size_t)nc * 8, (size_t)n, hipMemcpyDeviceToDevice, ctx->stream));
    return PK_OK;
}

__global__ void v32_image_stat_kernel(int64_t n, int K, int ld32, const double *__restrict__ V, int64_t ldv, const float *__restrict__ bound,
                                      float *__restrict__ out, uint32_t *__restrict__ stat) {
    const int64_t i = (int64_t)blockIdx.x * blockDim.x + threadIdx.x;
    if (i >= n * ld32) return;
    const int64_t r = i / ld32;
    const int c = (int)(i - r * ld32);
    float v = 0.0f;
    if (c < K) {
        const double d = V[r * ldv + c];
        v = (float)d;
        if (!(fabs(d) <= 1.7976931348623157e308)) atomicOr(&stat[1], 1u);
    } else if (c == K) {
        v = bound[r];
        if (!(v >= 0.0f && v <= 3.4028234e38f)) atomicOr(&stat[1], 1u); else atomicMax(&stat[0], __float_as_uint(v));
    }
    out[i] = v;
}

extern "C" int pk_v32_image_f32(void *stream, int64_t n, int32_t K, int32_t ld32, const double *V_dev, int64_t ldv, const float *bound_dev,
                                float *out_dev, uint32_t *stat_dev) {
    PK_REQUIRE(n >= 0 && K >= 1 && ld32 > K && ldv >= K && V_dev && bound_dev && out_dev && stat_dev, "pk_v32_image_f32: bad arguments");
    hipStream_t st = pk_stream(stream);
    (void)hipMemsetAsync(stat_dev, 0, 8, st);
    if (n > 0)
        hipLaunchKernelGGL(v32_image_stat_kernel, dim3((unsigned)(((size_t)n * ld32 + 255) / 256)), dim3(256), 0, st, n, K, ld32, V_dev, ldv, bound_dev,
                           out_dev, stat_dev);
    PK_CHECK_LAUNCH("v32_image_stat_kernel");
    return PK_OK;
}

extern "C" int pk_sym_eig_topk_f64(pk_ctx *ctx, void *stream, int32_t n, const double *T_dev, int64_t ldt, int32_t k, int32_t l,
                                   const double *X0_dev, int64_t ldx0, int32_t x0_rows, double tol, int32_t max_outer, uint64_t seed,
                                   double *basis_out_dev, int64_t ldb, double *lam_out_host, double *res_out_host,
                                   int32_t *counts_out, const double *lam0_host, double r0_rel) {
    if (!ctx) return PK_E_INVALID;
    std::lock_guard<std::mutex> lock(ctx->mu);
    PoolScope pool_scope(ctx);
    (void)hipSetDevice(ctx->device);
    if (n < 1 || k < 1 || l < k || l > n || l > 1024 || !T_dev || ldt < n || !basis_out_dev || ldb < l || !lam_out_host || !res_out_host ||
        !counts_out || (X0_dev && (x0_rows < 1 || x0_rows > n || ldx0 < l)))
        return fail(ctx, PK_E_INVALID, "pk_sym_eig_topk_f64: bad arguments (n=%d, k=%d, l=%d)", n, k, l);
    if (tol <= 0) tol = 1e-13;
    if (max_outer <= 0) max_outer = 200;
    hipStream_t st = stream ? pk_stream(stream) : ctx->stream;
    Solver S{ctx, st, Dev()};
    DMat T(n, n), X(n, l);
    if (!T.ok() || !X.ok()) return fail(ctx, PK_E_LAUNCH, "out of device memory (pk_sym_eig_topk_f64)");
    HIPCK(hipMemcpy2DAsync(T.p(), (size_t)n * 8, T_dev, (size_t)ldt * 8, (size_t)n * 8, (size_t)n, hipMemcpyDeviceToDevice, st));
    if (X0_dev) {
        HIPCK(hipMemsetAsync(X.p(), 0, (size_t)n * l * 8, st));
        HIPCK(hipMemcpy2DAsync(X.p(), (size_t)l * 8, X0_dev, (size_t)ldx0 * 8, (size_t)l * 8, (size_t)x0_rows, hipMemcpyDeviceToDevice, st));
    } else {
        hipLaunchKernelGGL(unit_block_kernel, dim3((unsigned)(((int64_t)n * l + 255) / 256)), dim3(256), 0, st, (int64_t)n, l, X.p());
    }
    DenseOp dop{ctx, S, T};
    SubspaceOut so;
    CK(dense_topk(ctx, S, dop, k, std::move(X), tol, max_outer, seed, X0_dev ? lam0_host : nullptr, r0_rel, so, X0_dev == nullptr));
    const int w = std::min<int>(l, so.basis.l);
    HIPCK(hipMemcpy2DAsync(basis_out_dev, (size_t)ldb * 8, so.basis.p(), (size_t)so.basis.l * 8, (size_t)w * 8, (size_t)n,
                           hipMemcpyDeviceToDevice, st));
    HIPCK(hipStreamSynchronize(st));
    for (int j = 0; j < l; ++j) lam_out_host[j] = j < (int)so.lam_all.size() ? so.lam_all[(size_t)j] : 0.0;
    for (int j = 0; j < l; ++j) res_out_host[j] = j < (int)so.res_act.size() ? so.res_act[(size_t)j] : 0.0;
    counts_out[0] = so.n_lock;
    counts_out[1] = w - so.n_lock;
    counts_out[2] = so.converged ? 1 : 0;
    counts_out[3] = so.outer;
    counts_out[4] = dop.products;
    return PK_OK;
}

struct pk_serving {
    int64_t n_items = 0, n_users = 0;
    int K = 0, ld32 = 0, Kx_full = 0;
    double vmax = 0.0;
    bool nonneg = true, have_tiles = false, have_v32 = false, fused = false;
    Dev inv64;
    DMat V;
    Csr Ts;
    Dev Vp, tile_bound, V32, tiles, ntiles, dense, skip;
    Dev vnorm, q20_raw, q20_tab;
    char *q20_img = nullptr;
    int dense_tiles = 0;
};

namespace {

int serving_build(pk_ctx *ctx, pk_serving *sv, int64_t n_items, int32_t K, const double *V_host, pk_mat *T) {
    hipStream_t st = ctx->stream;
    const int64_t n_users = T->A.n_rows;
    Solver S{ctx, st, Dev()};
    sv->n_items = n_items; sv->n_users = n_users; sv->K = K; sv->nonneg = T->nonneg; sv->fused = K <= 256;
    std::vector<double> norm((size_t)n_items, 0.0);
    for (int j = 0; j < K; ++j)
        for (int64_t i = 0; i < n_items; ++i) { const double v = V_host[(size_t)j * n_items + i]; norm[(size_t)i] += v * v; }
    double vmax = 0.0;
    for (auto &v : norm) { v = std::sqrt(v); vmax = std::max(vmax, v); }
    if (!std::isfinite(vmax) || (vmax != 0.0 && !(vmax > 1e-30 && vmax < 1e30)))
        return fail(ctx, PK_E_INVALID, "pk_score_topk: item factors with max row norm %g are outside the fp32 range of the candidate sweep", vmax);
    sv->vmax = vmax;
    std::vector<int32_t> inv((size_t)n_items), rank_of((size_t)n_items);
    std::iota(inv.begin(), inv.end(), 0);
    std::stable_sort(inv.begin(), inv.end(), [&](int32_t a, int32_t b) { return norm[(size_t)a] > norm[(size_t)b]; });
    for (int64_t i = 0; i < n_items; ++i) rank_of[(size_t)inv[(size_t)i]] = (int32_t)i;
    {
        std::vector<int64_t> inv_l(inv.begin(), inv.end());
        if (!sv->inv64.alloc((size_t)n_items * 8)) return fail(ctx, PK_E_LAUNCH, "out of device memory (item ids)");
        CK(S.upload(inv_l.data(), sv->inv64.p, (size_t)n_items * 8));
    }
    std::vector<double> vr((size_t)n_items * K);
    for (int64_t i = 0; i < n_items; ++i)
        for (int j = 0; j < K; ++j) vr[(size_t)i * K + j] = V_host[(size_t)j * n_items + inv[(size_t)i]];
    sv->V = DMat(n_items, K);
    DMat &V = sv->V;
    if (!V.ok()) return fail(ctx, PK_E_LAUNCH, "out of device memory (factors)");
    CK(S.upload(vr.data(), V.p(), vr.size() * 8));
    Csr &Ts = sv->Ts;
    Ts.n_rows = n_users; Ts.n_cols = n_items; Ts.nnz = T->A.nnz; Ts.val_kind = T->A.val_kind;
    const size_t ve = Ts.val_kind == PK_VAL_F32 ? 4 : 8, n1 = (size_t)std::max<int64_t>(Ts.nnz, 1);
    {
        Dev cmap((size_t)n_items * 4), work((size_t)pk_csr_relabel_work_bytes(Ts.nnz));
        if (!cmap.p || !work.p || !Ts.indptr.alloc((size_t)(n_users + 1) * 8) || !Ts.indices.alloc(n1 * 4) || !Ts.values.alloc(n1 * ve))
            return fail(ctx, PK_E_LAUNCH, "out of device memory (test matrix)");
        CK(S.upload(rank_of.data(), cmap.p, (size_t)n_items * 4));
        HIPCK(hipMemcpyAsync(Ts.indptr.p, T->A.indptr.p, (size_t)(n_users + 1) * 8, hipMemcpyDeviceToDevice, st));
        CK(pk_csr_relabel_sorted(st, n_users, n_items, Ts.nnz, T->A.indptr.as<int64_t>(), T->A.indices.as<int32_t>(), T->A.values.p,
                                 Ts.val_kind, cmap.as<int32_t>(), Ts.indices.as<int32_t>(), Ts.values.p, work.p));
        HIPCK(hipStreamSynchronize(st));
    }
    CK(build_plan(ctx, Ts));
    if (!sv->fused) return PK_OK;
    Dev tb_work((size_t)n_items * 4), rowb((size_t)n_items * 4);
    if (!sv->Vp.alloc((size_t)pk_pack_elems(n_items, K) * 4) || !sv->tile_bound.alloc((size_t)((n_items + 31) / 32) * 4) || !tb_work.p || !rowb.p)
        return fail(ctx, PK_E_LAUNCH, "out of device memory (factor images)");
    CK(pk_pack_frag_f32(st, n_items, K, V.p(), K, sv->Vp.as<float>()));
    CK(pk_tile_norm_bound_f32(st, n_items, K, V.p(), K, tb_work.as<float>(), sv->tile_bound.as<float>()));
    sv->Kx_full = ((K + 1 + 3) / 4) * 4;
    sv->ld32 = sv->Kx_full > 16 ? ((sv->Kx_full + 31) / 32) * 32 : (sv->Kx_full <= 4 ? 4 : sv->Kx_full <= 8 ? 8 : 16);
// ... 499 lines not shown
```

polara_amd/csrc/eigh.hip:

```cpp
#include "pk_common.h"
#include <math.h>

#define EIGH_THREADS 1024
#define EIGH_WAVES (EIGH_THREADS / 64)

__device__ __forceinline__ void rr_pair(int m, int step, int k, int &p, int &q) {
    const int r = m - 1;
    if (k == 0) {
        p = r;
        q = step;
    } else {
        p = step + k;
        p -= (p >= r) ? r : 0;
        q = step - k + r;
        q -= (q >= r) ? r : 0;
    }
    if (p > q) {
        int t = p;
        p = q;
        q = t;
    }
}

__device__ __forceinline__ double eigh_rsqrt(double x, int newton) {
    double y = __builtin_amdgcn_rsq(x);
    for (int i = 0; i < newton; ++i) y = y * fma(-0.5 * x, y * y, 1.5);
    return y;
}
__device__ __forceinline__ bool eigh_rotation(double alpha, double beta, double gamma, double tol2, double &cs, double &sn) {
    const int e = __builtin_amdgcn_frexp_exp(fmax(alpha, beta));
    alpha = ldexp(alpha, -e);
    beta = ldexp(beta, -e);
    gamma = ldexp(gamma, -e);
    if (!(gamma * gamma > tol2 * alpha * beta) || gamma == 0.0) return false;
    const double d = beta - alpha, g2 = 2.0 * gamma;
    const double x = fma(d, d, g2 * g2);
    const double h = x * eigh_rsqrt(x, 2);
    const double s = fabs(d) + h;
    double r = __builtin_amdgcn_rcp(s);
    r = r * fma(-s, r, 2.0);
    r = r * fma(-s, r, 2.0);
    const double t = (d >= 0.0 ? g2 : -g2) * r;
    cs = eigh_rsqrt(fma(t, t, 1.0), 3);
    sn = cs * t;
    return true;
}

#define EIGH_PW 4

template <int CTRL>
__device__ __forceinline__ double eigh_dpp_add(double v) {
    const int lo = __double2loint(v), hi = __double2hiint(v);
    const int lo2 = __builtin_amdgcn_update_dpp(0, lo, CTRL, 0xf, 0xf, false);
    const int hi2 = __builtin_amdgcn_update_dpp(0, hi, CTRL, 0xf, 0xf, false);
    return v + __hiloint2double(hi2, lo2);
}
__device__ __forceinline__ double eigh_row16_sum(double v) {
    v = eigh_dpp_add<0xB1>(v);
    v = eigh_dpp_add<0x4E>(v);
    v = eigh_dpp_add<0x141>(v);
    v = eigh_dpp_add<0x140>(v);
    return v;
}

template <int NC>
__device__ __forceinline__ bool eigh_pair_step(double *wp, double *wq, int n, int t, bool act, double tol2) {
    double alpha = 0.0, beta = 0.0, gamma = 0.0;
    double cs = 1.0, sn = 0.0;
    if constexpr (NC > 0) {
        double a[NC], b[NC];
#pragma unroll
        for (int j = 0; j < NC; ++j) {
            const int c = t + 16 * j;
            const bool in = act && c < n;
            a[j] = in ? wp[c] : 0.0;
            b[j] = in ? wq[c] : 0.0;
            alpha = fma(a[j], a[j], alpha);
            beta = fma(b[j], b[j], beta);
            gamma = fma(a[j], b[j], gamma);
        }
        alpha = eigh_row16_sum(alpha);
        beta = eigh_row16_sum(beta);
        gamma = eigh_row16_sum(gamma);
        const bool rot = act && eigh_rotation(alpha, beta, gamma, tol2, cs, sn);
        if (rot) {
#pragma unroll
            for (int j = 0; j < NC; ++j) {
                const int c = t + 16 * j;
                if (c < n) {
                    wp[c] = cs * a[j] - sn * b[j];
                    wq[c] = sn * a[j] + cs * b[j];
                }
            }
        }
        return rot;
    } else {
        if (act) {
            for (int c = t; c < n; c += 16) {
                const double a = wp[c], b = wq[c];
                alpha = fma(a, a, alpha);
                beta = fma(b, b, beta);
                gamma = fma(a, b, gamma);
            }
        }
        alpha = eigh_row16_sum(alpha);
        beta = eigh_row16_sum(beta);
        gamma = eigh_row16_sum(gamma);
        const bool rot = act && eigh_rotation(alpha, beta, gamma, tol2, cs, sn);
        if (rot) {
            for (int c = t; c < n; c += 16) {
                const double a = wp[c], b = wq[c];
                wp[c] = cs * a - sn * b;
                wq[c] = sn * a + cs * b;
            }
        }
        return rot;
    }
}
#define EIGH_LDS_MAX 136
template <bool IN_LDS, int NC>
__global__ __launch_bounds__(EIGH_THREADS) void eigh_psd_kernel(int n, double *__restrict__ Wg, int64_t ldwg,
                                                                double *__restrict__ Rg, int64_t ldrg,
                                                                double *__restrict__ evals, int max_sweeps,
                                                                double tol, int *__restrict__ info, int precondition,
                                                                const int *__restrict__ chol_flag) {
    extern __shared__ __attribute__((aligned(16))) double eigh_smem[];
    constexpr int NMAX = IN_LDS ? EIGH_LDS_MAX : 1024;
    __shared__ int s_rot;
    __shared__ int s_flag;
    __shared__ double s_lam[NMAX];
    __shared__ int s_rank[NMAX];
    __shared__ double s_vec[NMAX];
    const int tid = threadIdx.x;
    const int lane = tid & 63;
    const int wave = __builtin_amdgcn_readfirstlane(tid >> 6);
    double *W = IN_LDS ? eigh_smem : Wg;
    const int64_t ldw = IN_LDS ? n : ldwg;
    if (IN_LDS) {
        for (int e = tid; e < n * n; e += EIGH_THREADS) W[e] = Wg[(int64_t)(e / n) * ldwg + (e % n)];
    }
    __syncthreads();
    bool chol_ok = (!IN_LDS && chol_flag) ? (*chol_flag != 0) : false;
    if (IN_LDS && n >= 4 && max_sweeps > 0 && precondition) {
        int tx_log2 = 4;
        while ((1 << tx_log2) < n) ++tx_log2;
        const int TX = 1 << tx_log2, TY = EIGH_THREADS >> tx_log2;
        const int tx = tid & (TX - 1), ty = tid >> tx_log2;
        int fail = 0;
        for (int j = 0; j < n; ++j) {
            __syncthreads();
            const double d = W[j * n + j];
            if (!(d > 0.0)) {
                fail = 1;
                break;
            }
            const double invd = 1.0 / d;
            for (int c = j + 1 + tx; c < n; c += TX) {
                const double pj = W[j * n + c];
                for (int i = j + 1 + ty; i <= c; i += TY) W[i * n + c] = fma(-W[j * n + i] * invd, pj, W[i * n + c]);
            }
        }
        __syncthreads();
        if (!fail) {
            for (int i = tid; i < n; i += EIGH_THREADS) s_lam[i] = 1.0 / sqrt(W[i * n + i]);
            __syncthreads();
            for (int e = tid; e < n * n; e += EIGH_THREADS) {
                const int i = e / n, c = e - i * n;
                W[e] = (c >= i) ? W[e] * s_lam[i] : 0.0;
            }
            chol_ok = true;
        } else {
            for (int e = tid; e < n * n; e += EIGH_THREADS) W[e] = Wg[(int64_t)(e / n) * ldwg + (e % n)];
        }
        __syncthreads();
    }

    const int m = (n + 1) & ~1;
    const double tol2 = tol * tol;
    int sweep = 0, converged = (n <= 1);
    for (; sweep < max_sweeps && !converged; ++sweep) {
        if (tid == 0) s_rot = 0;
        __syncthreads();
        for (int step = 0; step < m - 1; ++step) {
            for (int k0 = wave * EIGH_PW; k0 < m / 2; k0 += EIGH_WAVES * EIGH_PW) {
                const int slot = lane >> 4, t = lane & 15;
                const int k = k0 + slot;
                bool act = k < m / 2;
                int p = 0, q = 0;
                if (act) {
                    rr_pair(m, step, k, p, q);
                    act = q < n;
                }
                double *wp = W + (int64_t)p * ldw, *wq = W + (int64_t)q * ldw;
                const bool rot = eigh_pair_step<NC>(wp, wq, n, t, act, tol2);
                const unsigned long long rb = __ballot(rot && t == 0);
                if (lane == 0 && rb) atomicAdd(&s_rot, __popcll(rb));
            }
            __syncthreads();
        }
        converged = (s_rot == 0);
        __syncthreads();
    }

    for (int i = wave; i < n; i += EIGH_WAVES) {
        const double *wi = W + (int64_t)i * ldw;
        double a = 0.0;
        for (int c = lane; c < n; c += 64) a = fma(wi[c], wi[c], a);
        a = sqrt(pk_wave_sum(a));
        if (lane == 0) s_lam[i] = a;
    }
    __syncthreads();
    if (tid == 0) {
        double mx = 0.0;
        for (int i = 0; i < n; ++i) mx = fmax(mx, s_lam[i]);
        s_vec[0] = mx * 1e-100;
    }
    __syncthreads();
    const double noise = s_vec[0];
    __syncthreads();
    for (int i = wave; i < n; i += EIGH_WAVES) {
        double *wi = W + (int64_t)i * ldw;
        const double a = s_lam[i];
        const bool ok = (a > noise) && (a > 1e-290);
        const double inv = ok ? 1.0 / a : 0.0;
        for (int c = lane; c < n; c += 64) wi[c] *= inv;
        if (lane == 0) s_rank[i] = ok ? 1 : 0;
    }
    __syncthreads();
    if (chol_ok) {
        for (int i = tid; i < n; i += EIGH_THREADS) s_lam[i] *= s_lam[i];
        __syncthreads();
    }
    for (int i = 0; i < n; ++i) {
        if (s_rank[i]) continue;
        for (int j = 0; j < n; ++j) {
            for (int c = tid; c < n; c += EIGH_THREADS) {
                double v = (c == j) ? 1.0 : 0.0;
                for (int r = 0; r < n; ++r) {
                    if (!s_rank[r]) continue;
                    const double *wr = W + (int64_t)r * ldw;
                    v -= wr[j] * wr[c];
                }
                s_vec[c] = v;
            }
            __syncthreads();
            if (tid == 0) {
                double nn = 0.0;
                for (int c = 0; c < n; ++c) nn += s_vec[c] * s_vec[c];
                s_flag = (nn > 0.25);
                if (s_flag) {
                    const double inv = 1.0 / sqrt(nn);
                    double *wi = W + (int64_t)i * ldw;
                    for (int c = 0; c < n; ++c) wi[c] = s_vec[c] * inv;
                    s_rank[i] = 1;
                }
            }
            __syncthreads();
            const int done = s_flag;
            __syncthreads();
            if (done) break;
        }
    }
    __syncthreads();
    for (int i = tid; i < n; i += EIGH_THREADS) {
        const double li = s_lam[i];
        int r = 0;
        for (int j = 0; j < n; ++j) {
            const double lj = s_lam[j];
            r += (lj > li) || (lj == li && j < i);
        }
        s_rank[i] = r;
        evals[r] = li;
    }
    __syncthreads();
    for (int i = wave; i < n; i += EIGH_WAVES) {
        const double *ri = W + (int64_t)i * ldw;
        double best = 0.0;
        int bestc = 0x7fffffff;
        for (int c = lane; c < n; c += 64) {
            double v = fabs(ri[c]);
            if (v > best) {
                best = v;
                bestc = c;
            }
        }
#pragma unroll
        for (int off = 32; off > 0; off >>= 1) {
            double ob = __shfl_xor(best, off, 64);
            int oc = __shfl_xor(bestc, off, 64);
            if (ob > best || (ob == best && oc < bestc)) {
                best = ob;
                bestc = oc;
            }
        }
        const double sgn = (bestc != 0x7fffffff && ri[bestc] < 0.0) ? -1.0 : 1.0;
        double *dst = Rg + (int64_t)s_rank[i] * ldrg;
        for (int c = lane; c < n; c += 64) dst[c] = sgn * ri[c];
    }
    if (tid == 0 && info) {
        info[0] = sweep;
        info[1] = converged;
    }
}

#define EIGH_BLOCK_LDS (144 * 1024)
template <int NC>
__device__ __forceinline__ void eigh_block_round_body(int n, double *__restrict__ Wg, int64_t ldwg, int w, int nb, int round,
                                                      int pair, int sweep, int *__restrict__ counters, double tol,
                                                      double *W, int *s_rot) {
    const int tid = threadIdx.x;
    const int lane = tid & 63;
    const int wave = __builtin_amdgcn_readfirstlane(tid >> 6);
    int bi, bj;
    rr_pair(nb, round, pair, bi, bj);
    const int i0 = bi * w, j0 = bj * w;
    const int ci = max(0, min(n, i0 + w) - i0), cj = max(0, min(n, j0 + w) - j0);
    const int nr = ci + cj;
    if (nr < 2) return;
    for (int e = tid; e < nr * n; e += EIGH_THREADS) {
        const int r = e / n, c = e - r * n;
        const int gr = r < ci ? i0 + r : j0 + (r - ci);
        W[e] = Wg[(int64_t)gr * ldwg + c];
    }
    if (tid == 0) *s_rot = 0;
    __syncthreads();
    const int m = (nr + 1) & ~1;
    const double tol2 = tol * tol;
    for (int step = 0; step < m - 1; ++step) {
        for (int k0 = wave * EIGH_PW; k0 < m / 2; k0 += EIGH_WAVES * EIGH_PW) {
            const int slot = lane >> 4, t = lane & 15;
            const int k = k0 + slot;
            bool act = k < m / 2;
            int p = 0, q = 0;
            if (act) {
                rr_pair(m, step, k, p, q);
                act = q < nr;
            }
            double *wp = W + (int64_t)p * n, *wq = W + (int64_t)q * n;
            const bool rot = eigh_pair_step<NC>(wp, wq, n, t, act, tol2);
            const unsigned long long rb = __ballot(rot && t == 0);
            if (lane == 0 && rb) atomicAdd(s_rot, __popcll(rb));
        }
        __syncthreads();
    }
    for (int e = tid; e < nr * n; e += EIGH_THREADS) {
        const int r = e / n, c = e - r * n;
        const int gr = r < ci ? i0 + r : j0 + (r - ci);
        Wg[(int64_t)gr * ldwg + c] = W[e];
    }
    if (tid == 0 && *s_rot) atomicAdd(&counters[sweep], *s_rot);
}

template <int NC>
__global__ __launch_bounds__(EIGH_THREADS) void eigh_block_round_kernel(int n, double *__restrict__ Wg, int64_t ldwg, int w,
                                                                        int nb, int round, int sweep,
                                                                        int *__restrict__ counters, double tol) {
    extern __shared__ __attribute__((aligned(16))) double eigh_smem[];
    __shared__ int s_rot;
    if (sweep > 0 && counters[sweep - 1] == 0) return;
    eigh_block_round_body<NC>(n, Wg, ldwg, w, nb, round, blockIdx.x, sweep, counters, tol, eigh_smem, &s_rot);
}

__device__ __forceinline__ void eigh_grid_barrier(int *bar, int n_wg, int &epoch, int *err) {
    __threadfence();
    __syncthreads();
    if (threadIdx.x == 0) {
        ++epoch;
        __hip_atomic_fetch_add(bar, 1, __ATOMIC_RELEASE, __HIP_MEMORY_SCOPE_AGENT);
        const int target = epoch * n_wg;
        long spins = 0;
        while (__hip_atomic_load(bar, __ATOMIC_ACQUIRE, __HIP_MEMORY_SCOPE_AGENT) < target) {
            __builtin_amdgcn_s_sleep(2);
            if (++spins > (1L << 24)) {
                atomicExch(err, 1);
                break;
            }
        }
    }
    __syncthreads();
    __threadfence();
}

template <int NC>
__global__ __launch_bounds__(EIGH_THREADS) void eigh_block_persistent_kernel(int n, double *__restrict__ Wg, int64_t ldwg, int w,
                                                                             int nb, int max_sweeps, int *__restrict__ counters,
// ... 173 lines not shown
```

polara_amd/csrc/pk_common.h:

```cpp
#pragma once
#include <hip/hip_runtime.h>
#include <stdint.h>
#include <stdio.h>
#include <stdarg.h>
#include <atomic>
#include "../../include/polara_hip.h"

#define PK_WAVE 64

void pk_set_error(const char *fmt, ...);
int pk_option(const char *name, int dflt);

#define PK_REQUIRE(cond, ...)                 \
    do {                                      \
        if (!(cond)) {                        \
            pk_set_error(__VA_ARGS__);        \
            return PK_E_INVALID;              \
        }                                     \
    } while (0)

#define PK_CHECK_LAUNCH(name)                                                          \
    do {                                                                               \
        hipError_t e_ = hipGetLastError();                                             \
        if (e_ != hipSuccess) {                                                        \
            pk_set_error("%s: launch failed: %s", name, hipGetErrorString(e_));        \
            return PK_E_LAUNCH;                                                        \
        }                                                                              \
    } while (0)

static inline hipStream_t pk_stream(void *s) { return reinterpret_cast<hipStream_t>(s); }

static inline int64_t pk_ceil_div(int64_t a, int64_t b) { return (a + b - 1) / b; }

struct PkDeviceOnce {
    std::atomic<uint64_t> mask{0};
    uint64_t bit() const {
        int d = 0;
        (void)hipGetDevice(&d);
        return 1ull << (d & 63);
    }
    bool pending() const { return (mask.load(std::memory_order_acquire) & bit()) == 0; }
    void done() { mask.fetch_or(bit(), std::memory_order_release); }
};

__device__ __forceinline__ double pk_wave_sum(double v) {
#pragma unroll
    for (int off = 32; off > 0; off >>= 1) v += __shfl_xor(v, off, 64);
    return v;
}
__device__ __forceinline__ float pk_wave_max(float v) {
#pragma unroll
    for (int off = 32; off > 0; off >>= 1) v = fmaxf(v, __shfl_xor(v, off, 64));
    return v;
}
__device__ __forceinline__ int pk_lane() { return threadIdx.x & 63; }

template <int J>
__device__ __forceinline__ int pk_lane_xor(int v) {
    static_assert(J == 1 || J == 2 || J == 4 || J == 8 || J == 16 || J == 32, "pk_lane_xor: J must be a power of two < 64");
    if constexpr (J == 1) {
        return __builtin_amdgcn_update_dpp(0, v, 0xB1, 0xf, 0xf, true);
    } else if constexpr (J == 2) {
        return __builtin_amdgcn_update_dpp(0, v, 0x4E, 0xf, 0xf, true);
    } else if constexpr (J == 4) {
        const int y = __builtin_amdgcn_update_dpp(0, v, 0x141, 0xf, 0xf, true);
        return __builtin_amdgcn_update_dpp(0, y, 0x1B, 0xf, 0xf, true);
    } else if constexpr (J == 8) {
        return __builtin_amdgcn_update_dpp(0, v, 0x128, 0xf, 0xf, true);
    } else if constexpr (J == 16) {
        const auto r = __builtin_amdgcn_permlane16_swap((unsigned)v, (unsigned)v, false, false);
        return ((threadIdx.x >> 4) & 1) ? (int)r[0] : (int)r[1];
    } else {
        const auto r = __builtin_amdgcn_permlane32_swap((unsigned)v, (unsigned)v, false, false);
        return ((threadIdx.x >> 5) & 1) ? (int)r[0] : (int)r[1];
    }
}
template <int J>
__device__ __forceinline__ float pk_lane_xor(float v) {
    return __int_as_float(pk_lane_xor<J>(__float_as_int(v)));
}
template <int J>
__device__ __forceinline__ double pk_lane_xor(double v) {
    const long long b = __double_as_longlong(v);
    const int lo = pk_lane_xor<J>((int)(unsigned)(b & 0xffffffffll)), hi = pk_lane_xor<J>((int)(b >> 32));
    return __longlong_as_double(((long long)hi << 32) | (unsigned)lo);
}
```

polara_amd/ops.py:

```python
import ctypes as C

import numpy as np
import torch

from . import _lib
from .csr import SPLIT_NNZ


_PTR_KEEP = None


def _ptr(t, offset=0):
    if t is None:
        return None
    if _PTR_KEEP is not None:
        _PTR_KEEP.append(t)
    return C.c_void_p(t.data_ptr() + offset * t.element_size())


def _raw_stream(index):
    return torch._C._cuda_getCurrentRawStream(index)


class _KernelTimer:
    __slots__ = ('ops', 'name', 'meta', 'e0', 'e1')

    def __init__(self, ops, name, meta):
        self.ops, self.name, self.meta = ops, name, meta

    def __enter__(self):
        if self.ops.timers is not None:
            self.e0 = torch.cuda.Event(enable_timing=True)
            self.e1 = torch.cuda.Event(enable_timing=True)
            self.e0.record(torch.cuda.current_stream(self.ops.device))

    def __exit__(self, *exc):
        if self.ops.timers is not None:
            self.e1.record(torch.cuda.current_stream(self.ops.device))
            self.ops.timers.setdefault(self.name, []).append((self.e0, self.e1, self.meta))
        return False


class DeviceCSR:

    def __init__(self, ops, indptr, indices, values, shape, split=SPLIT_NNZ):
        indptr = np.ascontiguousarray(indptr, dtype=np.int64)
        indices = np.ascontiguousarray(indices, dtype=np.int32)
        values = np.ascontiguousarray(values)
        if values.dtype == np.float64:
            v32 = values.astype(np.float32)
            if np.array_equal(v32.astype(np.float64), values):
                values = v32
        elif values.dtype != np.float32:
            values = values.astype(np.float64)
        dev = ops.device
        self._setup(ops, torch.from_numpy(indptr).to(dev), torch.from_numpy(indices).to(dev),
                    torch.from_numpy(values).to(dev), shape, split, nnz=int(indptr[-1]))
        self._host = (indptr, indices, values)

    def _setup(self, ops, indptr, indices, values, shape, split, nnz=None):
        self.ops = ops
        self.shape = (int(shape[0]), int(shape[1]))
        self.indptr, self.indices, self.values = indptr, indices, values
        self.val_kind = _lib.PK_VAL_F32 if values.dtype == torch.float32 else _lib.PK_VAL_F64
        self._host = None
        self.split = split
        self._partial = None
        self._T = None
        self._seen_tiles = None
        self._seen_dense = None
        self.sorted_cols = True
        self._nnz = nnz
        self._plan = None

    @property
    def nnz(self):
        if self._nnz is None:
            self._nnz = int(self.indptr[-1].item()) - int(self.indptr[0].item())
        return self._nnz

    def _ensure_plan(self):
        if self._plan is None:
            self._plan = self.ops.row_plan(self.indptr, self.shape[0], self.split)
# ... 176 lines not shown
    def _timing(self):
        want = 1 if self.ops.timers is not None else 0
        if want != getattr(self.ops, '_rec_timing_on', 0):
            _lib.check(self.ops.lib.pk_ctx_set_option(self.ctx, b'time_spmm', want), 'pk_ctx_set_option', self.ops.lib, self.ctx)
            if not want:
                self.ops.lib.pk_ctx_spmm_timings(self.ctx, None, None, 0)
            self.ops._rec_timing_on = want

    def collect_timings(self):
        if not getattr(self.ops, '_rec_timing_on', 0):
            return
        cap = 1 << 14
        ms = np.zeros(cap)
        meta = np.zeros((cap, 6), dtype=np.int64)
        n = int(self.ops.lib.pk_ctx_spmm_timings(self.ctx, ms.ctypes.data_as(C.c_void_p), meta.ctypes.data_as(C.c_void_p), cap))
        if self.ops.timers is not None:
            rows = self.ops.timers.setdefault('spmm', [])
            for i in range(min(n, cap)):
                rows.append((_Elapsed(float(ms[i])), None, tuple(int(v) for v in meta[i])))

    def steps(self, Q, T, S_out, flags, j0, m, last_closes, rounded=False):
        self._timing()
        assert Q.stride(1) == 1 and T.stride(1) == 1 and S_out.is_contiguous() and S_out.shape == (self.b, self.b)
        _lib.check(self.ops.lib.pk_lanczos_steps(self.ctx, self._stream(), self.handle, self.b, int(j0), int(m), 1 if last_closes else 0,
                                                 _ptr(Q), Q.stride(0), _ptr(T), T.stride(0), _ptr(S_out), _ptr(flags), 1 if rounded else 0),
                   'pk_lanczos_steps', self.ops.lib, self.ctx)

    def products(self, Q, j, rounded=False):
        self._timing()
        assert Q.stride(1) == 1
        W = self.ops.empty(Q.shape[0], self.b)
        _lib.check(self.ops.lib.pk_lanczos_products(self.ctx, self._stream(), self.handle, self.b, int(j), _ptr(Q), Q.stride(0), _ptr(W),
                                                    1 if rounded else 0), 'pk_lanczos_products', self.ops.lib, self.ctx)
        return W

    def orth(self, Q, T, S_out, flags, W, j, last_closes, rounded=False):
        assert Q.stride(1) == 1 and T.stride(1) == 1 and W.is_contiguous() and W.shape == (Q.shape[0], self.b)
        _lib.check(self.ops.lib.pk_lanczos_orth(self.ctx, self._stream(), Q.shape[0], self.b, int(j), 1 if last_closes else 0, _ptr(Q),
                                                Q.stride(0), _ptr(T), T.stride(0), _ptr(W), _ptr(S_out), _ptr(flags), 1 if rounded else 0),
                   'pk_lanczos_orth', self.ops.lib, self.ctx)

    def gramian(self, X):
        self._timing()
        X = X.contiguous()
        Z = self.ops.empty(X.shape[0], X.shape[1])
        _lib.check(self.ops.lib.pk_gramian_apply_f64(self.ctx, self._stream(), self.handle, X.shape[1], _ptr(X), X.stride(0), _ptr(Z),
                                                     Z.stride(0)), 'pk_gramian_apply_f64', self.ops.lib, self.ctx)
        return Z

    def __del__(self):
        try:
            if getattr(self, 'handle', None):
                self.ops._pending_mat_free.append((self.ctx, self.handle, self._keep))
                self.handle = None
        except Exception:
            pass


class HipOps:
    name = 'hip'

    _queues_warned = False
    _warmed = {}
    _warm_lock = __import__('threading').Lock()

    def __init__(self, device=None, warm=None):
        self.lib = _lib.load()
        if not torch.cuda.is_available():
            raise _lib.PolaraHipError('no HIP device visible: polara_amd has no CPU fallback')
        self.device = torch.device(device if device is not None else 'cuda:%d' % torch.cuda.current_device())
        self._dev_index = self.device.index if self.device.index is not None else torch.cuda.current_device()
        self._gram_work = None
        self._score_state = None
        self._score_states = None
        import threading
        self.pass_lock = threading.RLock()
        self._aux_streams = []
        self._pending_mat_free = []
        self.score_tiles_per_chunk = 0
        self.score_splits_override = 0
        self.seen_dense_tiles = None
        self._info = torch.zeros(2, dtype=torch.int32, device=self.device)
        self._ctx = None
        self.timers = None
        self.warm_up_s = 0.0
        from . import runtime_info
        rt = runtime_info()
        if not rt['ok'] and not HipOps._queues_warned:
            import warnings
            HipOps._queues_warned = True
            warnings.warn('polara_amd: the HIP runtime of this process works with %s hardware queue(s) (%s); the solver\'s '
                          'monitor stream, the scoring pass streams and RCCL then share queues and serialise: builds under a '
                          'process group were measured 25 %% slower, pipelined scoring 20 %%.  Import polara_amd (or call '
                          'polara_amd.configure_runtime()) before the first use of the device, or export GPU_MAX_HW_QUEUES=8.'
                          % (rt['hw_queues'], rt['source']), RuntimeWarning, stacklevel=2)
        if warm is None or warm is True:
            warm = 'code'
        if warm not in (False, 'code', 'pipeline'):
            raise ValueError("warm must be False, 'code' or 'pipeline'")
        if warm:
            self.warm_up(pipeline=(warm == 'pipeline'))

    def warm_up(self, pipeline=False):
        key = (self.device.index if self.device.index is not None else torch.cuda.current_device())
        import time
        t0 = time.perf_counter()
        with HipOps._warm_lock:
            done = HipOps._warmed.setdefault(key, set())
            with torch.cuda.device(self.device):
                if 'code' not in done:
                    _lib.check(self.lib.pk_warm_up(), 'pk_warm_up')
                    done.add('code')
                if pipeline and 'pipeline' not in done:
                    self._warm_pipeline()
                    torch.cuda.synchronize(self.device)
                    done.add('pipeline')
        self.warm_up_s += time.perf_counter() - t0

    def _warm_pipeline(self):
        from . import scoring
        from .solver import svd_topk
        rng = np.random.default_rng(0)
        n_users, n_items, per, k = 640, 256, 12, 4
        base = (np.arange(n_users) % 8)[:, None] * 32
        cols = np.sort(base + np.argsort(rng.random((n_users, 32)), axis=1)[:, :per], axis=1).astype(np.int32)
        indptr = np.arange(n_users + 1, dtype=np.int64) * per
        vals = rng.integers(1, 6, n_users * per).astype(np.float32)
        A = self.csr(indptr, cols.ravel(), vals, (n_users, n_items))
        _, _, _, rank_dev = self.item_order(A)
        A = self.csr_relabel_cols(A, rank_dev)
        A.transpose_operator()
        V = None
        for method in ('lanczos', 'subspace'):
            _, _, V, _ = svd_topk(self, A, k, tol=1e-8, max_outer=12, max_steps=8, method=method)
        F = scoring.FactorImage(self, V)
        Ta, perm = A.by_activity()
        self.scatter_rows(scoring.recommend(self, F, Ta, 5, True, order_users=False), perm)
        scoring.recommend(self, F, A, 5, True, return_scores=True)
        scoring.recommend(self, F, A, 5, False)

    def _timed(self, name, meta):
        return _KernelTimer(self, name, meta)

    def stream(self):
        return C.c_void_p(_raw_stream(self._dev_index))

    def stream_key(self):
        return _raw_stream(self._dev_index)

    def recurrence_ctx(self):
        if getattr(self, '_ctx_rec', None) is None:
            ctx = C.c_void_p()
            _lib.check(self.lib.pk_ctx_create(self.device.index or 0, C.byref(ctx)), 'pk_ctx_create')
            self._ctx_rec = ctx
        return self._ctx_rec

    def free_pending_handles(self):
        if not self._pending_mat_free or torch.cuda.is_current_stream_capturing():
            return
        pending, self._pending_mat_free = self._pending_mat_free, []
        torch.cuda.synchronize(self.device)
        for ctx, handle, _keep in pending:
            self.lib.pk_mat_free(ctx, handle)

    def lanczos_recurrence(self, A, block_cols):
        self.free_pending_handles()
# ... 357 lines not shown
        if int(info.item()) != 0:
            return None
        return img, tab

    def q20_decode(self, image, K):
        img, tab = image
        n = img.shape[0]
        out = self.empty(n, K + 1)
        _lib.check(self.lib.pk_q20_decode_f64(self.stream(), n, K, _ptr(img), _ptr(tab), _ptr(out), out.stride(0)),
                   'pk_q20_decode_f64')
        return out

    def fold_q20(self, A, image, K, out, rows=None):
        img, tab = image
        Kx = out.shape[1]
        assert out.dtype == torch.float64 and out.stride(1) == 1 and Kx >= K + 1 and img.shape[0] == A.shape[1]
        t0, n_tasks, l0, n_long = (0, A.n_tasks, 0, A.n_long) if rows is None else A.task_range(int(rows[0]), int(rows[1]))
        p = A.plan
        meta = None
        if self.timers is not None:
            meta = (A.shape[0], A.shape[1], A.nnz, Kx, A.values.element_size(), img.shape[1])
        with self._timed('fold_q20', meta):
            _lib.check(self.lib.pk_fold_q20(
                self.stream(), n_tasks, _ptr(p['task_row'], t0), _ptr(p['task_begin'], t0), _ptr(p['task_end'], t0),
                _ptr(p['task_slot'], t0), n_long, _ptr(p['long_row'], l0), _ptr(p['long_slot_begin'], l0),
                _ptr(p['long_slot_end'], l0), _ptr(A.indices), _ptr(A.values), A.val_kind, _ptr(img), _ptr(tab),
                int(A.shape[1]), int(K), int(Kx), _ptr(out), out.stride(0), _ptr(A.partial(Kx))), 'pk_fold_q20')
        return out

    def gram(self, A, B=None):
        B = A if B is None else B
        assert A.stride(1) == 1 and B.stride(1) == 1 and A.shape[0] == B.shape[0]
        n, la = A.shape
        lb = B.shape[1]
        need = self.lib.pk_gram_work_bytes(n, la, lb)
        key = self.stream_key()
        if self._gram_work is None:
            self._gram_work = {}
        work = self._gram_work.get(key)
        if work is None or work.numel() * 8 < need:
            work = self._gram_work[key] = self.empty((need + 7) // 8)
        G = self.empty(la, lb)
        _lib.check(self.lib.pk_gram_f64(self.stream(), n, la, lb, _ptr(A), A.stride(0), _ptr(B), B.stride(0),
                                        _ptr(G), G.stride(0), _ptr(work)), 'pk_gram_f64')
        return G

    def tsmm(self, X, Cm, out=None):
        assert X.stride(1) == 1 and Cm.stride(1) == 1 and Cm.shape[0] == X.shape[1]
        n, lin = X.shape
        lout = Cm.shape[1]
        if out is None:
            out = self.empty(n, lout)
        _lib.check(self.lib.pk_tsmm_f64(self.stream(), n, lin, lout, _ptr(X), X.stride(0), _ptr(Cm), Cm.stride(0),
                                        _ptr(out), out.stride(0)), 'pk_tsmm_f64')
        return out

    def eigh_psd(self, S, max_sweeps=0, tol=0.0):
        n = S.shape[0]
        W = S.clone().contiguous()
        R = self.empty(n, n)
        lam = self.empty(n)
        info = self._info if n <= 136 else torch.zeros(2, dtype=torch.int32, device=self.device)
        _lib.check(self.lib.pk_eigh_psd_f64(self.stream(), n, _ptr(W), n, _ptr(R), n, _ptr(lam), max_sweeps, tol,
                                            _ptr(info)), 'pk_eigh_psd_f64')
        if n > 136:
            if int(info[1].item()) == 0:
                W.copy_(S)
                _lib.check(self.lib.pk_eigh_psd_rounds_f64(self.stream(), n, _ptr(W), n, _ptr(R), n, _ptr(lam), max_sweeps, tol,
                                                           _ptr(info)), 'pk_eigh_psd_rounds_f64')
                if int(info[1].item()) == 0:
                    raise RuntimeError('pk_eigh_psd_f64: the block Jacobi sweeps did not converge (n=%d)' % n)
        return lam, R.t()

    def tsmm_sub(self, Z, X, Cm, out=None):
        assert X.stride(1) == 1 and Cm.stride(1) == 1 and Z.stride(1) == 1 and Cm.shape[0] == X.shape[1] and Z.shape == (X.shape[0], Cm.shape[1])
        n, lin = X.shape
        lout = Cm.shape[1]
        if out is None:
            out = self.empty(n, lout)
        _lib.check(self.lib.pk_tsmm_sub_f64(self.stream(), n, lin, lout, _ptr(X), X.stride(0), _ptr(Cm), Cm.stride(0),
                                            _ptr(Z), Z.stride(0), _ptr(out), out.stride(0)), 'pk_tsmm_sub_f64')
        return out

    def sym_eig_topk(self, T, k, X0=None, tol=1e-13, max_outer=200, seed=0, stats=None, lam0=None, r0_rel=-1.0, width=None):
        n = int(T.shape[0])
        assert T.stride(1) == 1 and T.shape[1] == n
        if X0 is not None:
            X0 = X0.contiguous()
            l = int(X0.shape[1])
            if lam0 is not None:
                lam0 = np.ascontiguousarray(lam0, dtype=np.float64)
                lam0 = lam0 if len(lam0) == l else None
        else:
            l = min(n, max(int(k), 8, int(width or 0)))
        if self._ctx is None:
            ctx = C.c_void_p()
            _lib.check(self.lib.pk_ctx_create(self.device.index or 0, C.byref(ctx)), 'pk_ctx_create')
            self._ctx = ctx
        basis = self.empty(n, l)
        lam = np.zeros(l)
        res = np.zeros(l)
        counts = np.zeros(5, dtype=np.int32)
        rc = self.lib.pk_sym_eig_topk_f64(self._ctx, self.stream(), n, _ptr(T), T.stride(0), int(k), l,
                                          _ptr(X0) if X0 is not None else None, l, int(X0.shape[0]) if X0 is not None else 0,
                                          float(tol), int(max_outer), int(seed) & 0xFFFFFFFFFFFFFFFF, _ptr(basis), l,
                                          lam.ctypes.data_as(C.c_void_p), res.ctypes.data_as(C.c_void_p),
                                          counts.ctypes.data_as(C.c_void_p),
                                          lam0.ctypes.data_as(C.c_void_p) if lam0 is not None else None, float(r0_rel))
        if rc != 0:
            raise RuntimeError('pk_sym_eig_topk_f64: ' + (self.lib.pk_ctx_error(self._ctx) or b'').decode())
        if stats is not None:
            stats['outer'] = stats.get('outer', 0) + int(counts[3])
            stats['steps'] = stats.get('steps', 0) + int(counts[4])
        n_lock, n_act = int(counts[0]), int(counts[1])
        return basis[:, :n_lock + n_act], lam[:n_lock + n_act], res[:n_act], n_lock, bool(counts[2])

    def eigh_top(self, S, r):
        n = int(S.shape[0])
        r = int(r)
        if self.lib.pk_eigh_top_supported(n, r):
            S = S.contiguous()
            R = self.empty(r, n)
            lam = self.empty(r)
            info = torch.zeros(1, dtype=torch.int32, device=self.device)
            work = self._work(self.lib.pk_eigh_top_work_bytes(n))
            _lib.check(self.lib.pk_eigh_top_f64(self.stream(), n, _ptr(S), n, r, _ptr(R), n, _ptr(lam), _ptr(work), _ptr(info)),
                       'pk_eigh_top_f64')
            if int(info.item()) == 1:
                return lam, R.t()
        lam, C = self.eigh_psd(S)
        return lam[:r], C[:, :r]

    def eigh_top_deferred(self, S, r):
        n, r = int(S.shape[0]), int(r)
        assert self.lib.pk_eigh_top_supported(n, r)
        S = S.contiguous()
        R = self.zeros(r, n)
        lam = self.zeros(r)
        info = torch.zeros(1, dtype=torch.int32, device=self.device)
        work = self._work(self.lib.pk_eigh_top_work_bytes(n))
        _lib.check(self.lib.pk_eigh_top_f64(self.stream(), n, _ptr(S), n, r, _ptr(R), n, _ptr(lam), _ptr(work), _ptr(info)),
                   'pk_eigh_top_f64')
        return lam, R.t(), info

    def chol_rinv(self, G, shift_rel=0.0, info=None):
        n = G.shape[0]
        assert G.stride(1) == 1
        Rinv = self.empty(n, n)
        if info is None:
            info = torch.zeros(1, dtype=torch.int32, device=self.device)
        need = self.lib.pk_chol_work_bytes(n)
        work = self.empty((need + 7) // 8) if need else None
        _lib.check(self.lib.pk_chol_rinv_f64(self.stream(), n, _ptr(G), G.stride(0), float(shift_rel), _ptr(Rinv), n,
                                             _ptr(work), _ptr(info)), 'pk_chol_rinv_f64')
        return Rinv, info

    def orth_check(self, G, info, flags):
        assert G.stride(1) == 1 and G.shape[0] == G.shape[1] and info.dtype == torch.int32 and flags.dtype == torch.float64
        _lib.check(self.lib.pk_orth_check_f64(self.stream(), G.shape[0], _ptr(G), G.stride(0), _ptr(info), info.numel(),
                                              _ptr(flags)), 'pk_orth_check_f64')

    def axpbypcz(self, alpha, Z, beta=0.0, Y=None, gamma=0.0, X=None, out=None):
        assert Z.is_contiguous() and (Y is None or Y.is_contiguous()) and (X is None or X.is_contiguous())
        if out is None:
            out = torch.empty_like(Z)
        _lib.check(self.lib.pk_axpbypcz_f64(self.stream(), Z.numel(), float(alpha), _ptr(Z), float(beta), _ptr(Y),
                                            float(gamma), _ptr(X), _ptr(out)), 'pk_axpbypcz_f64')
        return out

    def resid_colnorm2(self, Z, X, theta):
        assert Z.stride(1) == 1 and X.stride(1) == 1 and theta.is_contiguous()
        n, l = Z.shape
        nb = self.lib.pk_resid_blocks(n)
        part = self.empty(nb, l)
        _lib.check(self.lib.pk_resid_colnorm2_f64(self.stream(), n, l, _ptr(Z), Z.stride(0), _ptr(X), X.stride(0),
                                                  _ptr(theta), _ptr(part)), 'pk_resid_colnorm2_f64')
        return part.sum(dim=0)

    def small_mm(self, A, B, transA=False, transB=False):
        A = A.contiguous()
        B = B.contiguous()
        M = A.shape[1] if transA else A.shape[0]
        K = A.shape[0] if transA else A.shape[1]
        N = B.shape[0] if transB else B.shape[1]
        out = self.empty(M, N)
        _lib.check(self.lib.pk_dgemm_small_f64(self.stream(), int(transA), int(transB), M, N, K, _ptr(A),
                                               A.stride(0), _ptr(B), B.stride(0), _ptr(out), out.stride(0)),
                   'pk_dgemm_small_f64')
        return out

    def scale_cols(self, X, s):
        assert X.stride(1) == 1
        _lib.check(self.lib.pk_scale_cols_f64(self.stream(), X.shape[0], X.shape[1], _ptr(X), X.stride(0),
                                              _ptr(s.contiguous())), 'pk_scale_cols_f64')
        return X

    def pack_frag(self, M):
        assert M.stride(1) == 1 and M.dtype == torch.float64
# ... 572 lines not shown
```

polara_amd/solver.py:

```python
import math

import numpy as np
import torch

DEFAULT_PRODUCTS = 'f64'
DEFAULT_METHOD = 'auto'
MAX_KRYLOV_COLS = 4096


class NoConvergence(RuntimeError):

    def __init__(self, msg, sigma=None, V=None, stats=None):
        super().__init__(msg)
        self.sigma, self.V, self.stats = sigma, V, stats


class NoComm:
    rank = 0
    world = 1

    def allreduce(self, t):
        return t


# ... 245 lines not shown
            V_lock = newV if V_lock is None else torch.cat([V_lock, newV], dim=1).contiguous()
            lam_lock.extend(float(t) for t in theta_host[:n_new])
            n_lock += n_new
            stats.setdefault('locked_at', []).append((it, n_lock))
            X = X[:, n_new:].contiguous()
            Z = Z[:, n_new:].contiguous()
            theta_host = theta_host[n_new:]
            res_host = res_host[n_new:]
        b = float(theta_host[-1])
        a0 = float(theta_host[0])
        m = _cheb_degree(a0, b, spread, m_max)
        stats.setdefault('degrees', []).append(m)
        e = 0.5 * b
        c = 0.5 * b
        if e <= 0.0 or a0 <= c:
            Yc = Z if V_lock is None else _project_out(lay, Z, V_lock)
        else:
            sigma = e / (a0 - c)
            tau = 2.0 / sigma
            Zp = Z if V_lock is None else _project_out(lay, Z, V_lock)
            Xc = X
            Yc = ops.axpbypcz(sigma / e, Zp, -c * sigma / e, Xc)
            for _ in range(2, m + 1):
                sigma_new = 1.0 / (tau - sigma)
                Zc = op.apply(Yc)
                if V_lock is not None:
                    Zc = _project_out(lay, Zc, V_lock)
                Yn = ops.axpbypcz(2.0 * sigma_new / e, Zc, -2.0 * sigma_new * c / e, Yc,
                                  -sigma * sigma_new, Xc)
                Xc, Yc = Yc, Yn
                sigma = sigma_new
        X = orthonormalize(lay, Yc, V_lock, seed=seed + 1 + it)
    basis = X if V_lock is None else torch.cat([V_lock, X], dim=1)
    lam_all = np.r_[np.asarray(lam_lock, dtype=np.float64), theta_host]
    return basis, lam_all, res_host, n_lock, converged


def _next_lanczos_block(lay, W, Qbuf, N, C, flags):
    ops = lay.ops
    m, l = lay.n, W.shape[1]
    u = 1.1102230246251565e-16
    fused = hasattr(ops, 'orth_check')
    if fused:
        info = getattr(ops, '_orth_info', None)
        if info is None:
            info = ops._orth_info = torch.zeros(3, dtype=torch.int32, device=W.device)
    else:
        info = torch.zeros(3, dtype=torch.int32, device=W.device)
    Qall, Ydst = Qbuf[:, :N], Qbuf[:, N:N + l]
    S = G = None
    for p in range(3):
        if p == 0:
            Yp = ops.tsmm_sub(W, Qall, C)
            S = G = lay.gram(Yp)
        else:
            M = lay.gram(Qbuf[:, :N + l], Ydst)
            G = M[N:]
            Yp = ops.tsmm_sub(Ydst, Qall, M[:N])
        Rinv, _ = ops.chol_rinv(G, 11.0 * (m * l + l * (l + 1)) * u if p == 0 else 0.0, info=info[p:p + 1])
        ops.tsmm(Yp, Rinv, out=Ydst)
    if fused:
        ops.orth_check(G, info, flags)
    else:
        err = (G - torch.eye(l, dtype=G.dtype, device=G.device)).abs().max()
        flags[0] += info.abs().sum().to(flags.dtype)
        flags[1] = torch.maximum(flags[1], torch.nan_to_num(err, nan=1.0, posinf=1.0).to(flags.dtype))
    return S


class _LanczosBreakdown(RuntimeError):
    """The block Krylov recurrence cannot continue (rank-deficient residual block, lost orthogonality, space exhausted):
    `svd_topk` then runs the filtered subspace iteration, which has a rebuild path for exactly these matrices."""


def _ritz_check(ops, Tj, S, X0, k, b, est_tol, prior, seed, inner, final=False, width=None, lam0=None):
    N = Tj.shape[0]
    cold_width = None
    if X0 is None:
        cold_width = min(N, max(b, width or b))
    t_in = max(0.3 * est_tol, 1e-4 if prior is None else 0.03 * prior)
    if final:
        t_in = 0.3 * est_tol
    r0 = -1.0 if (lam0 is None or prior is None) else float(prior)
    while True:
        basis, lam_all, res_in, n_lock, conv_in = ops.sym_eig_topk(Tj, k, X0, t_in, 200, seed, inner, lam0=lam0, r0_rel=r0, width=cold_width)
        cold_width = None
        lam0, r0 = None, -1.0
        X0 = basis.contiguous()
        Yk = X0[:, :k].contiguous()
        TY = ops.gram(Tj, Yk)
        lam_k = torch.as_tensor(lam_all[:k].copy(), device=Yk.device)
        r_in2 = ops.resid_colnorm2(TY, Yk, lam_k)
        yl = Yk[N - b:].contiguous()
        c2 = (yl * ops.small_mm(S, yl)).sum(0)
        both = ops.to_host(torch.stack([r_in2, c2]))
        lam1 = max(float(lam_all[0]), 1e-300)
        est = np.sqrt(np.maximum(both[0] + both[1], 0.0)) / lam1
        coupling = float(np.sqrt(max(both[1].max(), 0.0)) / lam1)
        if t_in <= 0.3 * est_tol or coupling >= 4.0 * t_in or not conv_in:
            break
        t_in = max(0.3 * est_tol, 0.1 * coupling)
    return dict(est=est, worst=float(est.max()), coupling=coupling, conv=bool(conv_in), basis=X0, lam_all=lam_all, Yk=Yk,
                lam_k=lam_k)


def _raise_on_breakdown(fl, j):
    if fl[0] != 0 or not (fl[1] < 1e-4):
        raise _LanczosBreakdown('residual block lost rank at step <= %d (Cholesky verdicts %g, orthonormality %.1e)' % (j, fl[0], fl[1]))


class _Monitor:

    def __init__(self, ops, j, Tj, S, X0, k, b, est_tol, prior, seed, inner, flags=None, width=None, lam0=None):
        import threading
        self.j = j
        self.out = self.err = None
        fsnap = flags.clone() if flags is not None else None
        dev = getattr(ops, 'device', None)
        cuda = dev is not None and getattr(dev, 'type', 'cpu') == 'cuda'
        side = None
        if cuda:
            side = ops.monitor_stream() if hasattr(ops, 'monitor_stream') else ops.aux_streams(1)[0]
            side.wait_stream(torch.cuda.current_stream(dev))
            for t in (Tj, S, X0, fsnap):
                if t is not None:
                    t.record_stream(side)

        def work():
            try:
                if cuda:
                    torch.cuda.set_device(dev)
                    with torch.cuda.stream(side):
                        if fsnap is not None:
                            _raise_on_breakdown(ops.to_host(fsnap), j)
                        self.out = _ritz_check(ops, Tj, S, X0, k, b, est_tol, prior, seed, inner, width=width, lam0=lam0)
                        side.synchronize()
                else:
                    if fsnap is not None:
                        _raise_on_breakdown(ops.to_host(fsnap), j)
                    self.out = _ritz_check(ops, Tj, S, X0, k, b, est_tol, prior, seed, inner, width=width, lam0=lam0)
            except BaseException as exc:
                self.err = exc
        self.thread = threading.Thread(target=work, name='pk-lanczos-monitor', daemon=True)
        self.thread.start()

    def join(self):
        self.thread.join()
        if self.err is not None:
            raise self.err
        return self.out


def _block_lanczos(ops, A, At, lay, comm, k, l, tol, seed, stats, verbose, max_steps, m_max, spread, even_lock, kb=None,
                   monitor_lag=None, t_step=None, steps_model=None, first_look=None, products='f64'):
    import time
    n = lay.n
    b = int(kb or l)
    qcap = min(n // b, MAX_KRYLOV_COLS // b)
    if qcap < 4 or max_steps < 4:
        raise _LanczosBreakdown('Krylov space of at most %d blocks' % qcap)
    qcap = min(qcap, max_steps)
    gop = _Gramian(ops, A, At, lay, comm, stats)
    rec = None
    if _library_recurrence(ops, A, comm, lay.sharded):
        rec = ops.lanczos_recurrence(A, b)
    halves = comm.world > 1 or getattr(comm, 'split_step', False)
    stats['recurrence'] = 'library' if rec is not None else 'composition'
    if rec is not None:
# ... 336 lines not shown
```

Measured before the change: 188.0 million.

## Fuse Chebyshev filter round into single persistent kernel with banded tridiagonal products

Adds a single-workgroup kernel that runs a whole Chebyshev-filtered subspace round (band-limited products with the block-tridiagonal Lanczos matrix, Cholesky QR passes, Ritz step, verdicts) on device and writes a compact record that is read back once. It replaces many small launches, per-segment allocations and host syncs with one launch. It also exploits the 2b bandwidth of the Krylov tridiagonal matrix to skip zero blocks in T*X. The fused path runs only when the size is supported and can be switched off by an option. The cost is a large new kernel confined to one workgroup, with different numerics from the unfused path.

```diff
diff --git a/include/polara_hip.h b/include/polara_hip.h
--- a/include/polara_hip.h
+++ b/include/polara_hip.h
@@ -111,6 +111,11 @@
                      int64_t ldr, void *work_dev, int32_t *info_dev);
 int pk_chol_rinv_scaled_f64(void *stream, int32_t n, const double *G_dev, int64_t ldg, double shift_rel, double *Rinv_dev,
                      int64_t ldr, void *work_dev, int32_t *info_dev);
+int32_t pk_eig_round_supported(int32_t N, int32_t l, int32_t w);
+int32_t pk_eig_round_record_doubles(int32_t l);
+int pk_eig_round_f64(void *stream, int32_t N, int32_t l, int32_t w, const double *T_dev, int64_t ldt, double *buf0, double *buf1,
+                     double *buf2, int32_t have_z, int32_t m, int32_t nseg, const double *coef_host, double shift_scaled,
+                     double *H_work_dev, double *record_dev);
 int pk_axpbypcz_f64(void *stream, int64_t n_elems, double alpha, const double *Z_dev, double beta,
                     const double *Y_dev, double gamma, const double *X_dev, double *out_dev);
 int32_t pk_resid_blocks(int64_t n);
diff --git a/polara_amd/_lib.py b/polara_amd/_lib.py
--- a/polara_amd/_lib.py
+++ b/polara_amd/_lib.py
@@ -151,6 +151,9 @@
     'pk_svd_build': (C.c_int, [_vp, _vp, _i32, _i32, _f64, _i32, C.c_uint64, _vp, _vp, _vp, _vp]),
     'pk_sym_eig_topk_f64': (C.c_int, [_vp, _vp, _i32, _vp, _i64, _i32, _i32, _vp, _i64, _i32, _f64, _i32, C.c_uint64,
                                       _vp, _i64, _vp, _vp, _vp, _vp, _f64]),
+    'pk_eig_round_supported': (_i32, [_i32, _i32, _i32]),
+    'pk_eig_round_record_doubles': (_i32, [_i32]),
+    'pk_eig_round_f64': (C.c_int, [_vp, _i32, _i32, _i32, _vp, _i64, _vp, _vp, _vp, _i32, _i32, _i32, _vp, _f64, _vp, _vp]),
     'pk_svd_build_sharded': (C.c_int, [_vp, _vp, _vp, _i32, _i32, _f64, _i32, C.c_uint64, _vp, _vp, _vp, _vp]),
     'pk_ctx_stream': (_vp, [_vp]),
     'pk_ctx_set_option': (C.c_int, [_vp, C.c_char_p, _i32]),
diff --git a/polara_amd/csrc/api.cpp b/polara_amd/csrc/api.cpp
--- a/polara_amd/csrc/api.cpp
+++ b/polara_amd/csrc/api.cpp
@@ -15,7 +15,8 @@
 #include <atomic>
 namespace {
 struct Option { const char *name; std::atomic<int> value; std::atomic<bool> set; };
-Option g_options[] = {{"score_boot_tiles", {0}, {false}}, {"score_head_tiles", {0}, {false}}, {"score_phase2_splits", {0}, {false}}};
+Option g_options[] = {{"score_boot_tiles", {0}, {false}}, {"score_head_tiles", {0}, {false}}, {"score_phase2_splits", {0}, {false}},
+                      {"eig_round_fused", {0}, {false}}, {"eig_round_no_shift", {0}, {false}}};
 }
 int pk_option(const char *name, int dflt) {
     for (auto &o : g_options)
@@ -77,6 +78,7 @@
 
 hipError_t pk_tu_load_dense();
 hipError_t pk_tu_load_driver();
+hipError_t pk_tu_load_eig_round();
 hipError_t pk_tu_load_eigh();
 hipError_t pk_tu_load_eigh_top();
 hipError_t pk_tu_load_evalmetrics();
@@ -91,7 +93,7 @@
 hipError_t pk_tu_load_ttm();
 
 extern "C" int pk_warm_up(void) {
-    hipError_t (*const loaders[])() = {pk_tu_load_dense, pk_tu_load_driver, pk_tu_load_eigh, pk_tu_load_eigh_top, pk_tu_load_evalmetrics, pk_tu_load_foldq, pk_tu_load_hybrid, pk_tu_load_i2i, pk_tu_load_ingest, pk_tu_load_lce, pk_tu_load_rescore, pk_tu_load_score, pk_tu_load_spmm, pk_tu_load_ttm};
+    hipError_t (*const loaders[])() = {pk_tu_load_dense, pk_tu_load_driver, pk_tu_load_eig_round, pk_tu_load_eigh, pk_tu_load_eigh_top, pk_tu_load_evalmetrics, pk_tu_load_foldq, pk_tu_load_hybrid, pk_tu_load_i2i, pk_tu_load_ingest, pk_tu_load_lce, pk_tu_load_rescore, pk_tu_load_score, pk_tu_load_spmm, pk_tu_load_ttm};
     for (auto f : loaders) {
         const hipError_t e = f();
         if (e != hipSuccess) {
diff --git a/polara_amd/csrc/dense.hip b/polara_amd/csrc/dense.hip
--- a/polara_amd/csrc/dense.hip
+++ b/polara_amd/csrc/dense.hip
@@ -1,4 +1,5 @@
 #include "pk_common.h"
+#include "small_dense_dev.h"
 
 static int gram_splits(int64_t n, int la, int lb) {
     int64_t tiles = pk_ceil_div(la, 64) * pk_ceil_div(lb, 64);
@@ -451,57 +452,8 @@
     __shared__ double s_shift;
     double *A = IN_LDS ? chol_lds : work;
     const int ld = IN_LDS ? n + 1 : n;
-    const int tid = threadIdx.x;
-    const int TX = 1 << tx_log2, TY = (int)blockDim.x >> tx_log2;
-    const int tx = tid & (TX - 1), ty = tid >> tx_log2;
-    if (tid < 64) {
-        double tr = 0.0;
-        for (int i = tid; i < n; i += 64) tr += SCALED ? 1.0 : G[(int64_t)i * ldg + i];
-        for (int o = 32; o > 0; o >>= 1) tr += __shfl_xor(tr, o);
-        if (tid == 0) s_shift = shift_rel * tr;
-    }
-    __syncthreads();
-    const double shift = s_shift;
-    for (int i = ty; i < n; i += TY)
-        for (int c = tx; c < n; c += TX) {
-            double g = (c >= i) ? G[(int64_t)i * ldg + c] : 0.0;
-            if constexpr (SCALED) {
-                const double gi = G[(int64_t)i * ldg + i], gc = G[(int64_t)c * ldg + c];
-                g = (c > i) ? g / (sqrt(gi) * sqrt(gc)) : (c == i ? (gi > 0.0 ? 1.0 : -1.0) : 0.0);
-            }
-            A[i * ld + c] = (c > i) ? g : (c == i ? g + shift : 0.0);
-        }
-    int fail = 0;
-    for (int j = 0; j < n; ++j) {
-        __syncthreads();
-        const double d = A[j * ld + j];
-        if (!(d > 0.0)) {
-            fail = j + 1;
-            break;
-        }
-        const double invd = 1.0 / d;
-        for (int c = tx; c < n; c += TX) {
-            const double pj = (c == j) ? 1.0 : A[j * ld + c];
-            for (int i = j + 1 + ty; i < n; i += TY)
-                if (c <= j || c >= i) {
-                    const double f = A[j * ld + i] * invd;
-                    A[i * ld + c] = fma(-f, pj, A[i * ld + c]);
-                }
-        }
-    }
-    __syncthreads();
-    if (tid == 0) info[0] = fail;
-    if (fail) return;
-    for (int k = ty; k < n; k += TY)
-        for (int c = tx; c < n; c += TX) {
-            double v = 0.0;
-            if (c >= k) {
-                const double rs = 1.0 / sqrt(A[c * ld + c]);
-                v = (c == k) ? rs : A[c * ld + k] * rs;
-                if constexpr (SCALED) v /= sqrt(G[(int64_t)k * ldg + k]);
-            }
-            Rinv[(int64_t)k * ldr + c] = v;
-        }
+    const int fail = pk_chol_rinv_body<SCALED>(n, G, ldg, shift_rel, Rinv, ldr, A, ld, &s_shift, tx_log2);
+    if (threadIdx.x == 0) info[0] = fail;
 }
 
 extern "C" int64_t pk_chol_work_bytes(int32_t n) { return (n > PK_CHOL_LDS_MAX) ? (int64_t)n * n * 8 : 0; }
diff --git a/polara_amd/csrc/driver.hip b/polara_amd/csrc/driver.hip
--- a/polara_amd/csrc/driver.hip
+++ b/polara_amd/csrc/driver.hip
@@ -50,6 +50,7 @@
     int dist_overlap = 1;
     int hooi_ttm = 0;
     int time_spmm = 0;
+    int eig_band = 0;
 };
 
 struct SpmmTiming {
@@ -646,7 +647,8 @@
     std::lock_guard<std::mutex> lock(ctx->mu);
     struct { const char *name; int *slot; int lo, hi; } table[] = {
         {"svd_method", &ctx->opt.svd_method, 0, 2},   {"krylov_block", &ctx->opt.krylov_block, 0, 1024},
-        {"dist_overlap", &ctx->opt.dist_overlap, 0, 2}, {"hooi_ttm", &ctx->opt.hooi_ttm, 0, 1}, {"time_spmm", &ctx->opt.time_spmm, 0, 1}};
+        {"dist_overlap", &ctx->opt.dist_overlap, 0, 2}, {"hooi_ttm", &ctx->opt.hooi_ttm, 0, 1}, {"time_spmm", &ctx->opt.time_spmm, 0, 1},
+        {"eig_band", &ctx->opt.eig_band, 0, 1024}};
     for (auto &e : table)
         if (!strcmp(name, e.name)) {
             if (value < e.lo || value > e.hi) return fail(ctx, PK_E_INVALID, "pk_ctx_set_option: %s takes %d..%d", name, e.lo, e.hi);
@@ -1013,6 +1015,7 @@
     Solver &S;
     const DMat &T;
     int products = 0;
+    int band = 0;
     int apply(const DMat &X, DMat &Z) {
         ++products;
         return S.tsmm(T, X, Z);
@@ -1078,6 +1081,11 @@
     }
     Dev chol_work((size_t)std::max<int64_t>(pk_chol_work_bytes(l), 8)), info(6 * 3 * 4);
     if (!chol_work.p || !info.p) return fail(ctx, PK_E_LAUNCH, "out of device memory (dense_topk_segments)");
+    const bool fused = pk_eig_round_supported((int32_t)std::min<int64_t>(N, INT32_MAX), l, dop.band) && pk_option("eig_round_fused", 1) != 0;
+    const double shift_scaled = pk_option("eig_round_no_shift", 0) ? 0.0 : 11.0 * ((double)N * l + (double)l * (l + 1)) * u;
+    Dev round_rec, round_h;
+    if (fused && (!round_rec.alloc((size_t)PK_EIG_ROUND_RECORD(l) * 8) || !round_h.alloc((size_t)l * l * 8)))
+        return fail(ctx, PK_E_LAUNCH, "out of device memory (dense_topk_segments)");
     for (int round = 0; round < 10; ++round) {
         const double a0 = lam[0], bnd = lam[(size_t)l - 1];
         const double e = 0.5 * bnd, c = 0.5 * bnd;
@@ -1087,42 +1095,74 @@
         const double amp = std::cosh(m * std::acosh(xk));
         const double need = std::max(worst / tol, 1.0) * 30.0;
         const int nseg = std::max(1, std::min(6, (int)std::ceil(std::log(need) / std::log(std::max(amp, 1.5)))));
-        HIPCK(hipMemsetAsync(info.p, 0, 6 * 3 * 4, S.st));
-        for (int seg = 0; seg < nseg; ++seg) {
-            DMat Z, Yc, Xc;
-            if (seg == 0 && have_z) Z = std::move(Zr); else CK(dop.apply(X, Z));
-            have_z = false;
+        int32_t verdicts[18];
+        if (fused) {
+            double coef[PK_EIG_ROUND_MAX_DEGREE][3];
             double sigma = e / (a0 - c);
             const double tau = 2.0 / sigma;
-            Xc = std::move(X);
-            CK(S.axpbypcz(sigma / e, Z, -c * sigma / e, &Xc, 0.0, nullptr, Yc));
+            coef[0][0] = sigma / e; coef[0][1] = -c * sigma / e; coef[0][2] = 0.0;
             for (int s2 = 2; s2 <= m; ++s2) {
                 const double sigma_new = 1.0 / (tau - sigma);
-                DMat Yn;
-                CK(dop.filter_step(Yc, 2.0 * sigma_new / e, -2.0 * sigma_new * c / e, -sigma * sigma_new, Xc, Yn));
-                Xc = std::move(Yc);
-                Yc = std::move(Yn);
+                coef[s2 - 1][0] = 2.0 * sigma_new / e; coef[s2 - 1][1] = -2.0 * sigma_new * c / e; coef[s2 - 1][2] = -sigma * sigma_new;
                 sigma = sigma_new;
             }
-            const int passes = (seg + 1 == nseg) ? 2 : 1;
-            for (int p = 0; p < passes; ++p) {
-                DMat G, Rinv(l, l), Yn;
-                if (!Rinv.ok()) return fail(ctx, PK_E_LAUNCH, "out of device memory (dense_topk_segments)");
-                CK(S.gram(Yc, Yc, G));
-                if (p == 0)
-                    CK(pk_chol_rinv_scaled_f64(S.st, l, G.p(), l, 11.0 * ((double)N * l + (double)l * (l + 1)) * u, Rinv.p(), l, chol_work.p,
-                                               info.as<int32_t>() + 3 * seg + p));
-                else
-                    CK(pk_chol_rinv_f64(S.st, l, G.p(), l, 0.0, Rinv.p(), l, chol_work.p, info.as<int32_t>() + 3 * seg + p));
-                CK(S.tsmm(Yc, Rinv, Yn));
-                Yc = std::move(Yn);
+            DMat B[3];
+            B[0] = std::move(X);
+            B[1] = have_z ? std::move(Zr) : DMat(N, l);
+            B[2] = DMat(N, l);
+            if (!B[1].ok() || !B[2].ok()) return fail(ctx, PK_E_LAUNCH, "out of device memory (dense_topk_segments)");
+            CK(pk_eig_round_f64(S.st, (int32_t)N, l, dop.band, dop.T.p(), dop.T.l, B[0].p(), B[1].p(), B[2].p(), have_z ? 1 : 0, m, nseg,
+                                &coef[0][0], shift_scaled, round_h.as<double>(), round_rec.as<double>()));
+            dop.products += nseg * m - (have_z ? 1 : 0) + 1;
+            out.outer += 1;
+            std::vector<double> rec((size_t)PK_EIG_ROUND_RECORD(l));
+            CK(S.to_host(round_rec.p, rec.data(), rec.size() * 8));
+            lam.assign(rec.begin(), rec.begin() + l);
+            res.assign((size_t)l, 0.0);
+            for (int j = 0; j < l; ++j) res[(size_t)j] = std::sqrt(std::max(rec[(size_t)(l + j)], 0.0));
+            const double *tail = rec.data() + 2 * l + PK_EIG_ROUND_VERDICTS;
+            for (int i = 0; i < 18; ++i) verdicts[i] = (int32_t)rec[(size_t)(2 * l + i)];
+            if (tail[0] != 0.0 || tail[3] != 1.0) verdicts[17] = verdicts[17] ? verdicts[17] : -1;
+            const int xi = std::min(2, std::max(0, (int)tail[1])), zi = std::min(2, std::max(0, (int)tail[2]));
+            X = std::move(B[xi]);
+            if (zi != xi) Zr = std::move(B[zi]);
+            have_z = true;
+        } else {
+            HIPCK(hipMemsetAsync(info.p, 0, 6 * 3 * 4, S.st));
+            for (int seg = 0; seg < nseg; ++seg) {
+                DMat Z, Yc, Xc;
+                if (seg == 0 && have_z) Z = std::move(Zr); else CK(dop.apply(X, Z));
+                have_z = false;
+                double sigma = e / (a0 - c);
+                const double tau = 2.0 / sigma;
+                Xc = std::move(X);
+                CK(S.axpbypcz(sigma / e, Z, -c * sigma / e, &Xc, 0.0, nullptr, Yc));
+                for (int s2 = 2; s2 <= m; ++s2) {
+                    const double sigma_new = 1.0 / (tau - sigma);
+                    DMat Yn;
+                    CK(dop.filter_step(Yc, 2.0 * sigma_new / e, -2.0 * sigma_new * c / e, -sigma * sigma_new, Xc, Yn));
+                    Xc = std::move(Yc);
+                    Yc = std::move(Yn);
+                    sigma = sigma_new;
+                }
+                const int passes = (seg + 1 == nseg) ? 2 : 1;
+                for (int p = 0; p < passes; ++p) {
+                    DMat G, Rinv(l, l), Yn;
+                    if (!Rinv.ok()) return fail(ctx, PK_E_LAUNCH, "out of device memory (dense_topk_segments)");
+                    CK(S.gram(Yc, Yc, G));
+                    if (p == 0)
+                        CK(pk_chol_rinv_scaled_f64(S.st, l, G.p(), l, shift_scaled, Rinv.p(), l, chol_work.p, info.as<int32_t>() + 3 * seg + p));
+                    else
+                        CK(pk_chol_rinv_f64(S.st, l, G.p(), l, 0.0, Rinv.p(), l, chol_work.p, info.as<int32_t>() + 3 * seg + p));
+                    CK(S.tsmm(Yc, Rinv, Yn));
+                    Yc = std::move(Yn);
+                }
+                X = std::move(Yc);
             }
-            X = std::move(Yc);
-        }
-        CK(ritz());
-        have_z = true;
-        int32_t verdicts[18];
-        CK(S.to_host(info.p, verdicts, sizeof verdicts));
+            CK(ritz());
+            have_z = true;
+            CK(S.to_host(info.p, verdicts, sizeof verdicts));
+        }
         bool broke = false;
         for (int32_t v : verdicts) broke = broke || v != 0;
         for (double v : lam) broke = broke || !(v == v);
@@ -1211,6 +1251,7 @@
     bool first_pass = true;
     for (;;) {
         DenseOp dop{ctx, S, T};
+        dop.band = 2 * b;
         SubspaceOut so;
         const bool warm_pairs = warm && warm_lam && (int)warm_lam->size() == X0.l && prior >= 0;
         CK(dense_topk(ctx, S, dop, k, std::move(X0), t_in, 200, seed, warm_pairs ? warm_lam->data() : nullptr, warm_pairs ? prior : -1.0, so,
@@ -1784,6 +1825,7 @@
         hipLaunchKernelGGL(unit_block_kernel, dim3((unsigned)(((int64_t)n * l + 255) / 256)), dim3(256), 0, st, (int64_t)n, l, X.p());
     }
     DenseOp dop{ctx, S, T};
+    dop.band = ctx->opt.eig_band;
     SubspaceOut so;
     CK(dense_topk(ctx, S, dop, k, std::move(X), tol, max_outer, seed, X0_dev ? lam0_host : nullptr, r0_rel, so, X0_dev == nullptr));
     const int w = std::min<int>(l, so.basis.l);
diff --git a/polara_amd/csrc/eig_round.hip b/polara_amd/csrc/eig_round.hip
--- /dev/null
+++ b/polara_amd/csrc/eig_round.hip
@@ -0,0 +1,335 @@
+#include "pk_common.h"
+#include "small_dense_dev.h"
+
+typedef double f64x4 __attribute__((ext_vector_type(4)));
+
+#define ER_THREADS 1024
+#define ER_WAVES (ER_THREADS / 64)
+#define ER_LMAX 64
+#define ER_LDS_DOUBLES (ER_LMAX * ER_LMAX + ER_LMAX * (ER_LMAX + 1) + ER_LMAX * ER_LMAX)
+
+struct EigRoundArgs {
+    int N, l, w;
+    int m, nseg, have_z;
+    const double *T;
+    int64_t ldt;
+    double *buf[3];
+    double *Hg;
+    double *rec;
+    double coef[PK_EIG_ROUND_MAX_DEGREE][3];
+    int pass_scaled[2];
+    double pass_shift[2];
+    int passes_mid, passes_last;
+    double eig_tol;
+    int eig_sweeps;
+};
+
+
+__device__ __forceinline__ double er_ld(const double *p, int64_t idx, bool ok) {
+    const double v = p[ok ? idx : 0];
+    return ok ? v : 0.0;
+}
+
+__device__ __forceinline__ void er_band_step(const EigRoundArgs &A, const double *in, const double *prev, double *out, double a,
+                                             double b, double c) {
+    const int lane = threadIdx.x & 63, li = lane & 15, lq = lane >> 4;
+    const int wave = __builtin_amdgcn_readfirstlane((int)threadIdx.x >> 6);
+    const int N = A.N, l = A.l, w = A.w;
+    const double *__restrict__ T = A.T;
+    for (int i0 = wave * 16; i0 < N; i0 += ER_WAVES * 16) {
+        f64x4 acc[4];
+#pragma unroll
+        for (int cb = 0; cb < 4; ++cb) acc[cb] = f64x4{0.0, 0.0, 0.0, 0.0};
+        const int k_lo = max(0, i0 - w + 1) & ~3, k_hi = min(N, i0 + 15 + w);
+        const int row = i0 + li;
+        for (int k0 = k_lo; k0 < k_hi; k0 += 16) {
+            double p[4], q[4][4];
+#pragma unroll
+            for (int u = 0; u < 4; ++u) {
+                const int k = k0 + 4 * u + lq;
+                const int d = row - k;
+                p[u] = er_ld(T, (int64_t)row * A.ldt + k, row < N && k < k_hi && d < w && -d < w);
+#pragma unroll
+                for (int cb = 0; cb < 4; ++cb) {
+                    const int col = 16 * cb + li;
+                    q[u][cb] = er_ld(in, (int64_t)k * l + col, k < k_hi && col < l);
+                }
+            }
+#pragma unroll
+            for (int u = 0; u < 4; ++u)
+#pragma unroll
+                for (int cb = 0; cb < 4; ++cb)
+                    acc[cb] = __builtin_amdgcn_mfma_f64_16x16x4f64(p[u], q[u][cb], acc[cb], 0, 0, 0);
+        }
+#pragma unroll
+        for (int cb = 0; cb < 4; ++cb) {
+            const int col = 16 * cb + li;
+#pragma unroll
+            for (int r = 0; r < 4; ++r) {
+                const int orow = i0 + lq + 4 * r;
+                if (orow < N && col < l) {
+                    double v = a * acc[cb][r];
+                    if (b != 0.0) v = fma(b, in[(int64_t)orow * l + col], v);
+                    if (c != 0.0) v = fma(c, prev[(int64_t)orow * l + col], v);
+                    out[(int64_t)orow * l + col] = v;
+                }
+            }
+        }
+    }
+}
+
+__device__ __forceinline__ void er_gram(const EigRoundArgs &A, const double *Y, const double *Z, double *G) {
+    const int lane = threadIdx.x & 63, li = lane & 15, lq = lane >> 4;
+    const int wave = __builtin_amdgcn_readfirstlane((int)threadIdx.x >> 6);
+    const int N = A.N, l = A.l;
+    const int gi = wave & 3, quarter = wave >> 2;
+    const int rows_q = (((N + 3) / 4) + 3) & ~3;
+    const int r_lo = quarter * rows_q, r_hi = min(N, r_lo + rows_q);
+    f64x4 acc[4];
+#pragma unroll
+    for (int cb = 0; cb < 4; ++cb) acc[cb] = f64x4{0.0, 0.0, 0.0, 0.0};
+    if (16 * gi < l) {
+        const int pc = 16 * gi + li;
+        for (int k0 = r_lo; k0 < r_hi; k0 += 16) {
+            double p[4], q[4][4];
+#pragma unroll
+            for (int u = 0; u < 4; ++u) {
+                const int k = k0 + 4 * u + lq;
+                p[u] = er_ld(Y, (int64_t)k * l + pc, k < r_hi && pc < l);
+#pragma unroll
+                for (int cb = 0; cb < 4; ++cb) {
+                    const int col = 16 * cb + li;
+                    q[u][cb] = er_ld(Z, (int64_t)k * l + col, k < r_hi && col < l);
+                }
+            }
+#pragma unroll
+            for (int u = 0; u < 4; ++u)
+#pragma unroll
+                for (int cb = 0; cb < 4; ++cb)
+                    acc[cb] = __builtin_amdgcn_mfma_f64_16x16x4f64(p[u], q[u][cb], acc[cb], 0, 0, 0);
+        }
+    }
+    for (int s = 0; s < 4; ++s) {
+        if (quarter == s && 16 * gi < l) {
+#pragma unroll
+            for (int cb = 0; cb < 4; ++cb) {
+                const int col = 16 * cb + li;
+#pragma unroll
+                for (int r = 0; r < 4; ++r) {
+                    const int i = 16 * gi + lq + 4 * r;
+                    if (i < l && col < l) G[i * l + col] = (s == 0) ? acc[cb][r] : G[i * l + col] + acc[cb][r];
+                }
+            }
+        }
+        __syncthreads();
+    }
+}
+
+__device__ __forceinline__ void er_rows_times_small(const EigRoundArgs &A, const double *Y, int i0, const double *Cm, int sk, int sj,
+                                                    f64x4 (&acc)[4]) {
+    const int lane = threadIdx.x & 63, li = lane & 15, lq = lane >> 4;
+    const int N = A.N, l = A.l;
+    const int row = i0 + li;
+#pragma unroll
+    for (int cb = 0; cb < 4; ++cb) acc[cb] = f64x4{0.0, 0.0, 0.0, 0.0};
+    for (int k0 = 0; k0 < l; k0 += 8) {
+        double p[2], q[2][4];
+#pragma unroll
+        for (int u = 0; u < 2; ++u) {
+            const int k = k0 + 4 * u + lq;
+            p[u] = er_ld(Y, (int64_t)row * l + k, row < N && k < l);
+#pragma unroll
+            for (int cb = 0; cb < 4; ++cb) {
+                const int col = 16 * cb + li;
+                q[u][cb] = er_ld(Cm, k * sk + col * sj, k < l && col < l);
+            }
+        }
+#pragma unroll
+        for (int u = 0; u < 2; ++u)
+#pragma unroll
+            for (int cb = 0; cb < 4; ++cb)
+                acc[cb] = __builtin_amdgcn_mfma_f64_16x16x4f64(p[u], q[u][cb], acc[cb], 0, 0, 0);
+    }
+}
+
+__device__ __forceinline__ void er_store_rows(const EigRoundArgs &A, double *Y, int i0, const f64x4 (&acc)[4]) {
+    const int lane = threadIdx.x & 63, li = lane & 15, lq = lane >> 4;
+#pragma unroll
+    for (int cb = 0; cb < 4; ++cb) {
+        const int col = 16 * cb + li;
+#pragma unroll
+        for (int r = 0; r < 4; ++r) {
+            const int orow = i0 + lq + 4 * r;
+            if (orow < A.N && col < A.l) Y[(int64_t)orow * A.l + col] = acc[cb][r];
+        }
+    }
+}
+
+__device__ __forceinline__ double *er_buf(const EigRoundArgs &A, int i) { return i == 0 ? A.buf[0] : (i == 1 ? A.buf[1] : A.buf[2]); }
+
+__global__ __launch_bounds__(ER_THREADS) void eig_round_kernel(const EigRoundArgs A) {
+    extern __shared__ __attribute__((aligned(16))) double er_lds[];
+    double *sG = er_lds;
+    double *sA = sG + ER_LMAX * ER_LMAX;
+    double *sC = sA + ER_LMAX * (ER_LMAX + 1);
+    __shared__ EighScratch<ER_LMAX> sc;
+    __shared__ double s_shift;
+    __shared__ double s_theta[ER_LMAX];
+    __shared__ double s_res[ER_WAVES][ER_LMAX];
+    __shared__ double s_coef[PK_EIG_ROUND_MAX_DEGREE][3];
+    const int tid = threadIdx.x;
+    const int lane = tid & 63, li = lane & 15, lq = lane >> 4;
+    const int wave = __builtin_amdgcn_readfirstlane(tid >> 6);
+    const int N = A.N, l = A.l;
+    double *rec = A.rec;
+    double *r_lam = rec, *r_res = rec + l, *r_verdict = rec + 2 * l, *r_tail = rec + 2 * l + PK_EIG_ROUND_VERDICTS;
+    for (int i = tid; i < PK_EIG_ROUND_RECORD(l); i += ER_THREADS) rec[i] = 0.0;
+#pragma unroll
+    for (int s = 0; s < PK_EIG_ROUND_MAX_DEGREE; ++s)
+        if (tid == s) {
+            s_coef[s][0] = A.coef[s][0];
+            s_coef[s][1] = A.coef[s][1];
+            s_coef[s][2] = A.coef[s][2];
+        }
+    __syncthreads();
+    int tx_log2 = 4;
+    while ((1 << tx_log2) < l && tx_log2 < 8) ++tx_log2;
+
+    int xc = 0, yc, sp;
+    for (int seg = 0; seg < A.nseg; ++seg) {
+        if (seg == 0 && A.have_z) {
+            yc = 2; sp = 1;
+            const double *X = er_buf(A, xc), *Z = A.buf[1];
+            double *Y = er_buf(A, yc);
+            for (int e = tid; e < N * l; e += ER_THREADS) Y[e] = fma(s_coef[0][1], X[e], s_coef[0][0] * Z[e]);
+        } else {
+            yc = (xc + 1) % 3; sp = (xc + 2) % 3;
+            er_band_step(A, er_buf(A, xc), nullptr, er_buf(A, yc), s_coef[0][0], s_coef[0][1], 0.0);
+        }
+        __syncthreads();
+        for (int s = 1; s < A.m; ++s) {
+            er_band_step(A, er_buf(A, yc), er_buf(A, xc), er_buf(A, sp), s_coef[s][0], s_coef[s][1], s_coef[s][2]);
+            __syncthreads();
+            const int t = xc; xc = yc; yc = sp; sp = t;
+        }
+        double *Y = er_buf(A, yc);
+        const int passes = (seg + 1 == A.nseg) ? A.passes_last : A.passes_mid;
+        for (int p = 0; p < passes; ++p) {
+            er_gram(A, Y, Y, sG);
+            const bool scaled = p == 0 ? A.pass_scaled[0] != 0 : A.pass_scaled[1] != 0;
+            const double shift = p == 0 ? A.pass_shift[0] : A.pass_shift[1];
+            const int fail = scaled ? pk_chol_rinv_body<true>(l, sG, l, shift, sC, l, sA, l + 1, &s_shift, tx_log2)
+                                    : pk_chol_rinv_body<false>(l, sG, l, shift, sC, l, sA, l + 1, &s_shift, tx_log2);
+            if (fail) {
+                if (tid == 0) r_verdict[3 * seg + p] = (double)fail;
+                return;
+            }
+            __syncthreads();
+            for (int i0 = wave * 16; i0 < N; i0 += ER_WAVES * 16) {
+                f64x4 acc[4];
+                er_rows_times_small(A, Y, i0, sC, l, 1, acc);
+                er_store_rows(A, Y, i0, acc);
+            }
+            __syncthreads();
+        }
+        xc = yc;
+    }
+    const int zi = (xc + 1) % 3;
+    double *X = er_buf(A, xc), *Z = er_buf(A, zi);
+    er_band_step(A, X, nullptr, Z, 1.0, 0.0, 0.0);
+    __syncthreads();
+    er_gram(A, X, Z, sA);
+    for (int e = tid; e < l * l; e += ER_THREADS) {
+        const int r = e / l, c = e - r * l;
+        const double h = 0.5 * (sA[e] + sA[c * l + r]);
+        sG[e] = h;
+        A.Hg[e] = h;
+    }
+    __syncthreads();
+    pk_eigh_psd_body<true, 4, ER_LMAX>(l, sG, l, A.Hg, l, sA, l + 1, s_theta, A.eig_sweeps, A.eig_tol, (int *)nullptr, 1,
+                                       (const int *)nullptr, sc);
+    __syncthreads();
+    double part[4] = {0.0, 0.0, 0.0, 0.0};
+    for (int i0 = wave * 16; i0 < N; i0 += ER_WAVES * 16) {
+        f64x4 ax[4], az[4];
+        er_rows_times_small(A, X, i0, sA, 1, l + 1, ax);
+        er_rows_times_small(A, Z, i0, sA, 1, l + 1, az);
+        er_store_rows(A, X, i0, ax);
+        er_store_rows(A, Z, i0, az);
+#pragma unroll
+        for (int cb = 0; cb < 4; ++cb) {
+            const int col = 16 * cb + li;
+            const double th = col < l ? s_theta[col] : 0.0;
+#pragma unroll
+            for (int r = 0; r < 4; ++r) {
+                const double d = az[cb][r] - th * ax[cb][r];
+                part[cb] = fma(d, d, part[cb]);
+            }
+        }
+    }
+#pragma unroll
+    for (int cb = 0; cb < 4; ++cb) {
+        double v = part[cb];
+        v += __shfl_xor(v, 16, 64);
+        v += __shfl_xor(v, 32, 64);
+        if (lq == 0) s_res[wave][16 * cb + li] = v;
+    }
+    __syncthreads();
+    if (tid < l) {
+        double r2 = 0.0;
+        for (int wv = 0; wv < ER_WAVES; ++wv) r2 += s_res[wv][tid];
+        const double th = s_theta[tid];
+        r_lam[tid] = th;
+        r_res[tid] = r2;
+        if (!(th == th) || !(r2 == r2)) r_tail[0] = 1.0;
+    }
+    if (tid == 0) {
+        r_tail[1] = (double)xc;
+        r_tail[2] = (double)zi;
+        r_tail[3] = 1.0;
+    }
+}
+
+extern "C" int32_t pk_eig_round_supported(int32_t N, int32_t l, int32_t w) {
+    return l >= 1 && l <= ER_LMAX && N >= l && N <= 1024 && w >= 1 && 2 * (int64_t)w <= N;
+}
+extern "C" int32_t pk_eig_round_record_doubles(int32_t l) { return PK_EIG_ROUND_RECORD(l); }
+
+extern "C" int pk_eig_round_f64(void *stream, int32_t N, int32_t l, int32_t w, const double *T_dev, int64_t ldt, double *buf0, double *buf1,
+                                double *buf2, int32_t have_z, int32_t m, int32_t nseg, const double *coef_host, double shift_scaled,
+                                double *H_work_dev, double *record_dev) {
+    PK_REQUIRE(pk_eig_round_supported(N, l, w), "pk_eig_round_f64: unsupported sizes (N=%d, l=%d, w=%d)", N, l, w);
+    PK_REQUIRE(m >= 1 && m <= PK_EIG_ROUND_MAX_DEGREE && nseg >= 1 && nseg <= 6, "pk_eig_round_f64: bad plan (m=%d, nseg=%d)", m, nseg);
+    PK_REQUIRE(T_dev && ldt >= N && buf0 && buf1 && buf2 && buf0 != buf1 && buf0 != buf2 && buf1 != buf2 && coef_host && H_work_dev && record_dev,
+               "pk_eig_round_f64: bad pointers");
+    static PkDeviceOnce attr_set;
+    if (attr_set.pending()) {
+        const hipError_t e1 = hipFuncSetAttribute(reinterpret_cast<const void *>(&eig_round_kernel), hipFuncAttributeMaxDynamicSharedMemorySize,
+                                                  ER_LDS_DOUBLES * 8);
+        if (e1 != hipSuccess) {
+            pk_set_error("pk_eig_round_f64: cannot raise the dynamic LDS limit: %s", hipGetErrorString(e1));
+            return PK_E_LAUNCH;
+        }
+        attr_set.done();
+    }
+    EigRoundArgs A;
+    A.N = N; A.l = l; A.w = w; A.m = m; A.nseg = nseg; A.have_z = have_z ? 1 : 0;
+    A.T = T_dev; A.ldt = ldt;
+    A.buf[0] = buf0; A.buf[1] = buf1; A.buf[2] = buf2;
+    A.Hg = H_work_dev; A.rec = record_dev;
+    for (int s = 0; s < PK_EIG_ROUND_MAX_DEGREE; ++s)
+        for (int c = 0; c < 3; ++c) A.coef[s][c] = s < m ? coef_host[3 * s + c] : 0.0;
+    A.pass_scaled[0] = 1; A.pass_shift[0] = shift_scaled;
+    A.pass_scaled[1] = 0; A.pass_shift[1] = 0.0;
+    A.passes_mid = 1; A.passes_last = 2;
+    A.eig_tol = 2.0 * 2.220446049250313e-16 * sqrt((double)l);
+    A.eig_sweeps = 40;
+    hipLaunchKernelGGL(eig_round_kernel, dim3(1), dim3(ER_THREADS), ER_LDS_DOUBLES * 8, pk_stream(stream), A);
+    PK_CHECK_LAUNCH("eig_round_kernel");
+    return PK_OK;
+}
+
+hipError_t pk_tu_load_eig_round() {
+    hipFuncAttributes a;
+    return hipFuncGetAttributes(&a, reinterpret_cast<const void *>(&eig_round_kernel));
+}
diff --git a/polara_amd/csrc/eigh.hip b/polara_amd/csrc/eigh.hip
--- a/polara_amd/csrc/eigh.hip
+++ b/polara_amd/csrc/eigh.hip
@@ -1,122 +1,7 @@
 #include "pk_common.h"
+#include "small_dense_dev.h"
 #include <math.h>
 
-#define EIGH_THREADS 1024
-#define EIGH_WAVES (EIGH_THREADS / 64)
-
-__device__ __forceinline__ void rr_pair(int m, int step, int k, int &p, int &q) {
-    const int r = m - 1;
-    if (k == 0) {
-        p = r;
-        q = step;
-    } else {
-        p = step + k;
-        p -= (p >= r) ? r : 0;
-        q = step - k + r;
-        q -= (q >= r) ? r : 0;
-    }
-    if (p > q) {
-        int t = p;
-        p = q;
-        q = t;
-    }
-}
-
-__device__ __forceinline__ double eigh_rsqrt(double x, int newton) {
-    double y = __builtin_amdgcn_rsq(x);
-    for (int i = 0; i < newton; ++i) y = y * fma(-0.5 * x, y * y, 1.5);
-    return y;
-}
-__device__ __forceinline__ bool eigh_rotation(double alpha, double beta, double gamma, double tol2, double &cs, double &sn) {
-    const int e = __builtin_amdgcn_frexp_exp(fmax(alpha, beta));
-    alpha = ldexp(alpha, -e);
-    beta = ldexp(beta, -e);
-    gamma = ldexp(gamma, -e);
-    if (!(gamma * gamma > tol2 * alpha * beta) || gamma == 0.0) return false;
-    const double d = beta - alpha, g2 = 2.0 * gamma;
-    const double x = fma(d, d, g2 * g2);
-    const double h = x * eigh_rsqrt(x, 2);
-    const double s = fabs(d) + h;
-    double r = __builtin_amdgcn_rcp(s);
-    r = r * fma(-s, r, 2.0);
-    r = r * fma(-s, r, 2.0);
-    const double t = (d >= 0.0 ? g2 : -g2) * r;
-    cs = eigh_rsqrt(fma(t, t, 1.0), 3);
-    sn = cs * t;
-    return true;
-}
-
-#define EIGH_PW 4
-
-template <int CTRL>
-__device__ __forceinline__ double eigh_dpp_add(double v) {
-    const int lo = __double2loint(v), hi = __double2hiint(v);
-    const int lo2 = __builtin_amdgcn_update_dpp(0, lo, CTRL, 0xf, 0xf, false);
-    const int hi2 = __builtin_amdgcn_update_dpp(0, hi, CTRL, 0xf, 0xf, false);
-    return v + __hiloint2double(hi2, lo2);
-}
-__device__ __forceinline__ double eigh_row16_sum(double v) {
-    v = eigh_dpp_add<0xB1>(v);
-    v = eigh_dpp_add<0x4E>(v);
-    v = eigh_dpp_add<0x141>(v);
-    v = eigh_dpp_add<0x140>(v);
-    return v;
-}
-
-template <int NC>
-__device__ __forceinline__ bool eigh_pair_step(double *wp, double *wq, int n, int t, bool act, double tol2) {
-    double alpha = 0.0, beta = 0.0, gamma = 0.0;
-    double cs = 1.0, sn = 0.0;
-    if constexpr (NC > 0) {
-        double a[NC], b[NC];
-#pragma unroll
-        for (int j = 0; j < NC; ++j) {
-            const int c = t + 16 * j;
-            const bool in = act && c < n;
-            a[j] = in ? wp[c] : 0.0;
-            b[j] = in ? wq[c] : 0.0;
-            alpha = fma(a[j], a[j], alpha);
-            beta = fma(b[j], b[j], beta);
-            gamma = fma(a[j], b[j], gamma);
-        }
-        alpha = eigh_row16_sum(alpha);
-        beta = eigh_row16_sum(beta);
-        gamma = eigh_row16_sum(gamma);
-        const bool rot = act && eigh_rotation(alpha, beta, gamma, tol2, cs, sn);
-        if (rot) {
-#pragma unroll
-            for (int j = 0; j < NC; ++j) {
-                const int c = t + 16 * j;
-                if (c < n) {
-                    wp[c] = cs * a[j] - sn * b[j];
-                    wq[c] = sn * a[j] + cs * b[j];
-                }
-            }
-        }
-        return rot;
-    } else {
-        if (act) {
-            for (int c = t; c < n; c += 16) {
-                const double a = wp[c], b = wq[c];
-                alpha = fma(a, a, alpha);
-                beta = fma(b, b, beta);
-                gamma = fma(a, b, gamma);
-            }
-        }
-        alpha = eigh_row16_sum(alpha);
-        beta = eigh_row16_sum(beta);
-        gamma = eigh_row16_sum(gamma);
-        const bool rot = act && eigh_rotation(alpha, beta, gamma, tol2, cs, sn);
-        if (rot) {
-            for (int c = t; c < n; c += 16) {
-                const double a = wp[c], b = wq[c];
-                wp[c] = cs * a - sn * b;
-                wq[c] = sn * a + cs * b;
-            }
-        }
-        return rot;
-    }
-}
 #define EIGH_LDS_MAX 136
 template <bool IN_LDS, int NC>
 __global__ __launch_bounds__(EIGH_THREADS) void eigh_psd_kernel(int n, double *__restrict__ Wg, int64_t ldwg,
@@ -126,181 +11,15 @@
                                                                 const int *__restrict__ chol_flag) {
     extern __shared__ __attribute__((aligned(16))) double eigh_smem[];
     constexpr int NMAX = IN_LDS ? EIGH_LDS_MAX : 1024;
-    __shared__ int s_rot;
-    __shared__ int s_flag;
-    __shared__ double s_lam[NMAX];
-    __shared__ int s_rank[NMAX];
-    __shared__ double s_vec[NMAX];
+    __shared__ EighScratch<NMAX> sc;
     const int tid = threadIdx.x;
-    const int lane = tid & 63;
-    const int wave = __builtin_amdgcn_readfirstlane(tid >> 6);
     double *W = IN_LDS ? eigh_smem : Wg;
     const int64_t ldw = IN_LDS ? n : ldwg;
     if (IN_LDS) {
         for (int e = tid; e < n * n; e += EIGH_THREADS) W[e] = Wg[(int64_t)(e / n) * ldwg + (e % n)];
     }
     __syncthreads();
-    bool chol_ok = (!IN_LDS && chol_flag) ? (*chol_flag != 0) : false;
-    if (IN_LDS && n >= 4 && max_sweeps > 0 && precondition) {
-        int tx_log2 = 4;
-        while ((1 << tx_log2) < n) ++tx_log2;
-        const int TX = 1 << tx_log2, TY = EIGH_THREADS >> tx_log2;
-        const int tx = tid & (TX - 1), ty = tid >> tx_log2;
-        int fail = 0;
-        for (int j = 0; j < n; ++j) {
-            __syncthreads();
-            const double d = W[j * n + j];
-            if (!(d > 0.0)) {
-                fail = 1;
-                break;
-            }
-            const double invd = 1.0 / d;
-            for (int c = j + 1 + tx; c < n; c += TX) {
-                const double pj = W[j * n + c];
-                for (int i = j + 1 + ty; i <= c; i += TY) W[i * n + c] = fma(-W[j * n + i] * invd, pj, W[i * n + c]);
-            }
-        }
-        __syncthreads();
-        if (!fail) {
-            for (int i = tid; i < n; i += EIGH_THREADS) s_lam[i] = 1.0 / sqrt(W[i * n + i]);
-            __syncthreads();
-            for (int e = tid; e < n * n; e += EIGH_THREADS) {
-                const int i = e / n, c = e - i * n;
-                W[e] = (c >= i) ? W[e] * s_lam[i] : 0.0;
-            }
-            chol_ok = true;
-        } else {
-            for (int e = tid; e < n * n; e += EIGH_THREADS) W[e] = Wg[(int64_t)(e / n) * ldwg + (e % n)];
-        }
-        __syncthreads();
-    }
-
-    const int m = (n + 1) & ~1;
-    const double tol2 = tol * tol;
-    int sweep = 0, converged = (n <= 1);
-    for (; sweep < max_sweeps && !converged; ++sweep) {
-        if (tid == 0) s_rot = 0;
-        __syncthreads();
-        for (int step = 0; step < m - 1; ++step) {
-            for (int k0 = wave * EIGH_PW; k0 < m / 2; k0 += EIGH_WAVES * EIGH_PW) {
-                const int slot = lane >> 4, t = lane & 15;
-                const int k = k0 + slot;
-                bool act = k < m / 2;
-                int p = 0, q = 0;
-                if (act) {
-                    rr_pair(m, step, k, p, q);
-                    act = q < n;
-                }
-                double *wp = W + (int64_t)p * ldw, *wq = W + (int64_t)q * ldw;
-                const bool rot = eigh_pair_step<NC>(wp, wq, n, t, act, tol2);
-                const unsigned long long rb = __ballot(rot && t == 0);
-                if (lane == 0 && rb) atomicAdd(&s_rot, __popcll(rb));
-            }
-            __syncthreads();
-        }
-        converged = (s_rot == 0);
-        __syncthreads();
-    }
-
-    for (int i = wave; i < n; i += EIGH_WAVES) {
-        const double *wi = W + (int64_t)i * ldw;
-        double a = 0.0;
-        for (int c = lane; c < n; c += 64) a = fma(wi[c], wi[c], a);
-        a = sqrt(pk_wave_sum(a));
-        if (lane == 0) s_lam[i] = a;
-    }
-    __syncthreads();
-    if (tid == 0) {
-        double mx = 0.0;
-        for (int i = 0; i < n; ++i) mx = fmax(mx, s_lam[i]);
-        s_vec[0] = mx * 1e-100;
-    }
-    __syncthreads();
-    const double noise = s_vec[0];
-    __syncthreads();
-    for (int i = wave; i < n; i += EIGH_WAVES) {
-        double *wi = W + (int64_t)i * ldw;
-        const double a = s_lam[i];
-        const bool ok = (a > noise) && (a > 1e-290);
-        const double inv = ok ? 1.0 / a : 0.0;
-        for (int c = lane; c < n; c += 64) wi[c] *= inv;
-        if (lane == 0) s_rank[i] = ok ? 1 : 0;
-    }
-    __syncthreads();
-    if (chol_ok) {
-        for (int i = tid; i < n; i += EIGH_THREADS) s_lam[i] *= s_lam[i];
-        __syncthreads();
-    }
-    for (int i = 0; i < n; ++i) {
-        if (s_rank[i]) continue;
-        for (int j = 0; j < n; ++j) {
-            for (int c = tid; c < n; c += EIGH_THREADS) {
-                double v = (c == j) ? 1.0 : 0.0;
-                for (int r = 0; r < n; ++r) {
-                    if (!s_rank[r]) continue;
-                    const double *wr = W + (int64_t)r * ldw;
-                    v -= wr[j] * wr[c];
-                }
-                s_vec[c] = v;
-            }
-            __syncthreads();
-            if (tid == 0) {
-                double nn = 0.0;
-                for (int c = 0; c < n; ++c) nn += s_vec[c] * s_vec[c];
-                s_flag = (nn > 0.25);
-                if (s_flag) {
-                    const double inv = 1.0 / sqrt(nn);
-                    double *wi = W + (int64_t)i * ldw;
-                    for (int c = 0; c < n; ++c) wi[c] = s_vec[c] * inv;
-                    s_rank[i] = 1;
-                }
-            }
-            __syncthreads();
-            const int done = s_flag;
-            __syncthreads();
-            if (done) break;
-        }
-    }
-    __syncthreads();
-    for (int i = tid; i < n; i += EIGH_THREADS) {
-        const double li = s_lam[i];
-        int r = 0;
-        for (int j = 0; j < n; ++j) {
-            const double lj = s_lam[j];
-            r += (lj > li) || (lj == li && j < i);
-        }
-        s_rank[i] = r;
-        evals[r] = li;
-    }
-    __syncthreads();
-    for (int i = wave; i < n; i += EIGH_WAVES) {
-        const double *ri = W + (int64_t)i * ldw;
-        double best = 0.0;
-        int bestc = 0x7fffffff;
-        for (int c = lane; c < n; c += 64) {
-            double v = fabs(ri[c]);
-            if (v > best) {
-                best = v;
-                bestc = c;
-            }
-        }
-#pragma unroll
-        for (int off = 32; off > 0; off >>= 1) {
-            double ob = __shfl_xor(best, off, 64);
-            int oc = __shfl_xor(bestc, off, 64);
-            if (ob > best || (ob == best && oc < bestc)) {
-                best = ob;
-                bestc = oc;
-            }
-        }
-        const double sgn = (bestc != 0x7fffffff && ri[bestc] < 0.0) ? -1.0 : 1.0;
-        double *dst = Rg + (int64_t)s_rank[i] * ldrg;
-        for (int c = lane; c < n; c += 64) dst[c] = sgn * ri[c];
-    }
-    if (tid == 0 && info) {
-        info[0] = sweep;
-        info[1] = converged;
-    }
+    pk_eigh_psd_body<IN_LDS, NC, NMAX>(n, W, ldw, Wg, ldwg, Rg, ldrg, evals, max_sweeps, tol, info, precondition, chol_flag, sc);
 }
 
 #define EIGH_BLOCK_LDS (144 * 1024)
diff --git a/polara_amd/csrc/pk_common.h b/polara_amd/csrc/pk_common.h
--- a/polara_amd/csrc/pk_common.h
+++ b/polara_amd/csrc/pk_common.h
@@ -10,6 +10,10 @@
 
 void pk_set_error(const char *fmt, ...);
 int pk_option(const char *name, int dflt);
+
+#define PK_EIG_ROUND_MAX_DEGREE 24
+#define PK_EIG_ROUND_VERDICTS 18
+#define PK_EIG_ROUND_RECORD(l) (2 * (l) + PK_EIG_ROUND_VERDICTS + 4)
 
 #define PK_REQUIRE(cond, ...)                 \
     do {                                      \
diff --git a/polara_amd/csrc/small_dense_dev.h b/polara_amd/csrc/small_dense_dev.h
--- /dev/null
+++ b/polara_amd/csrc/small_dense_dev.h
@@ -0,0 +1,356 @@
+#pragma once
+#include "pk_common.h"
+#include <math.h>
+
+template <bool SCALED>
+__device__ __forceinline__ int pk_chol_rinv_body(int n, const double *__restrict__ G, int64_t ldg, double shift_rel,
+                                                 double *__restrict__ Rinv, int64_t ldr, double *A, int ld, double *s_shift,
+                                                 int tx_log2) {
+    const int tid = threadIdx.x;
+    const int TX = 1 << tx_log2, TY = (int)blockDim.x >> tx_log2;
+    const int tx = tid & (TX - 1), ty = tid >> tx_log2;
+    if (tid < 64) {
+        double tr = 0.0;
+        for (int i = tid; i < n; i += 64) tr += SCALED ? 1.0 : G[(int64_t)i * ldg + i];
+        for (int o = 32; o > 0; o >>= 1) tr += __shfl_xor(tr, o);
+        if (tid == 0) *s_shift = shift_rel * tr;
+    }
+    __syncthreads();
+    const double shift = *s_shift;
+    for (int i = ty; i < n; i += TY)
+        for (int c = tx; c < n; c += TX) {
+            double g = (c >= i) ? G[(int64_t)i * ldg + c] : 0.0;
+            if constexpr (SCALED) {
+                const double gi = G[(int64_t)i * ldg + i], gc = G[(int64_t)c * ldg + c];
+                g = (c > i) ? g / (sqrt(gi) * sqrt(gc)) : (c == i ? (gi > 0.0 ? 1.0 : -1.0) : 0.0);
+            }
+            A[i * ld + c] = (c > i) ? g : (c == i ? g + shift : 0.0);
+        }
+    int fail = 0;
+    for (int j = 0; j < n; ++j) {
+        __syncthreads();
+        const double d = A[j * ld + j];
+        if (!(d > 0.0)) {
+            fail = j + 1;
+            break;
+        }
+        const double invd = 1.0 / d;
+        for (int c = tx; c < n; c += TX) {
+            const double pj = (c == j) ? 1.0 : A[j * ld + c];
+            for (int i = j + 1 + ty; i < n; i += TY)
+                if (c <= j || c >= i) {
+                    const double f = A[j * ld + i] * invd;
+                    A[i * ld + c] = fma(-f, pj, A[i * ld + c]);
+                }
+        }
+    }
+    __syncthreads();
+    if (fail) return fail;
+    for (int k = ty; k < n; k += TY)
+        for (int c = tx; c < n; c += TX) {
+            double v = 0.0;
+            if (c >= k) {
+                const double rs = 1.0 / sqrt(A[c * ld + c]);
+                v = (c == k) ? rs : A[c * ld + k] * rs;
+                if constexpr (SCALED) v /= sqrt(G[(int64_t)k * ldg + k]);
+            }
+            Rinv[(int64_t)k * ldr + c] = v;
+        }
+    return 0;
+}
+
+#define EIGH_THREADS 1024
+#define EIGH_WAVES (EIGH_THREADS / 64)
+
+__device__ __forceinline__ void rr_pair(int m, int step, int k, int &p, int &q) {
+    const int r = m - 1;
+    if (k == 0) {
+        p = r;
+        q = step;
+    } else {
+        p = step + k;
+        p -= (p >= r) ? r : 0;
+        q = step - k + r;
+        q -= (q >= r) ? r : 0;
+    }
+    if (p > q) {
+        int t = p;
+        p = q;
+        q = t;
+    }
+}
+
+__device__ __forceinline__ double eigh_rsqrt(double x, int newton) {
+    double y = __builtin_amdgcn_rsq(x);
+    for (int i = 0; i < newton; ++i) y = y * fma(-0.5 * x, y * y, 1.5);
+    return y;
+}
+__device__ __forceinline__ bool eigh_rotation(double alpha, double beta, double gamma, double tol2, double &cs, double &sn) {
+    const int e = __builtin_amdgcn_frexp_exp(fmax(alpha, beta));
+    alpha = ldexp(alpha, -e);
+    beta = ldexp(beta, -e);
+    gamma = ldexp(gamma, -e);
+    if (!(gamma * gamma > tol2 * alpha * beta) || gamma == 0.0) return false;
+    const double d = beta - alpha, g2 = 2.0 * gamma;
+    const double x = fma(d, d, g2 * g2);
+    const double h = x * eigh_rsqrt(x, 2);
+    const double s = fabs(d) + h;
+    double r = __builtin_amdgcn_rcp(s);
+    r = r * fma(-s, r, 2.0);
+    r = r * fma(-s, r, 2.0);
+    const double t = (d >= 0.0 ? g2 : -g2) * r;
+    cs = eigh_rsqrt(fma(t, t, 1.0), 3);
+    sn = cs * t;
+    return true;
+}
+
+#define EIGH_PW 4
+
+template <int CTRL>
+__device__ __forceinline__ double eigh_dpp_add(double v) {
+    const int lo = __double2loint(v), hi = __double2hiint(v);
+    const int lo2 = __builtin_amdgcn_update_dpp(0, lo, CTRL, 0xf, 0xf, false);
+    const int hi2 = __builtin_amdgcn_update_dpp(0, hi, CTRL, 0xf, 0xf, false);
+    return v + __hiloint2double(hi2, lo2);
+}
+__device__ __forceinline__ double eigh_row16_sum(double v) {
+    v = eigh_dpp_add<0xB1>(v);
+    v = eigh_dpp_add<0x4E>(v);
+    v = eigh_dpp_add<0x141>(v);
+    v = eigh_dpp_add<0x140>(v);
+    return v;
+}
+
+template <int NC>
+__device__ __forceinline__ bool eigh_pair_step(double *wp, double *wq, int n, int t, bool act, double tol2) {
+    double alpha = 0.0, beta = 0.0, gamma = 0.0;
+    double cs = 1.0, sn = 0.0;
+    if constexpr (NC > 0) {
+        double a[NC], b[NC];
+#pragma unroll
+        for (int j = 0; j < NC; ++j) {
+            const int c = t + 16 * j;
+            const bool in = act && c < n;
+            a[j] = in ? wp[c] : 0.0;
+            b[j] = in ? wq[c] : 0.0;
+            alpha = fma(a[j], a[j], alpha);
+            beta = fma(b[j], b[j], beta);
+            gamma = fma(a[j], b[j], gamma);
+        }
+        alpha = eigh_row16_sum(alpha);
+        beta = eigh_row16_sum(beta);
+        gamma = eigh_row16_sum(gamma);
+        const bool rot = act && eigh_rotation(alpha, beta, gamma, tol2, cs, sn);
+        if (rot) {
+#pragma unroll
+            for (int j = 0; j < NC; ++j) {
+                const int c = t + 16 * j;
+                if (c < n) {
+                    wp[c] = cs * a[j] - sn * b[j];
+                    wq[c] = sn * a[j] + cs * b[j];
+                }
+            }
+        }
+        return rot;
+    } else {
+        if (act) {
+            for (int c = t; c < n; c += 16) {
+                const double a = wp[c], b = wq[c];
+                alpha = fma(a, a, alpha);
+                beta = fma(b, b, beta);
+                gamma = fma(a, b, gamma);
+            }
+        }
+        alpha = eigh_row16_sum(alpha);
+        beta = eigh_row16_sum(beta);
+        gamma = eigh_row16_sum(gamma);
+        const bool rot = act && eigh_rotation(alpha, beta, gamma, tol2, cs, sn);
+        if (rot) {
+            for (int c = t; c < n; c += 16) {
+                const double a = wp[c], b = wq[c];
+                wp[c] = cs * a - sn * b;
+                wq[c] = sn * a + cs * b;
+            }
+        }
+        return rot;
+    }
+}
+
+template <int NMAX>
+struct EighScratch {
+    int rot;
+    int flag;
+    double lam[NMAX];
+    int rank[NMAX];
+    double vec[NMAX];
+};
+
+template <bool IN_LDS, int NC, int NMAX>
+__device__ __forceinline__ void pk_eigh_psd_body(int n, double *W, int64_t ldw, const double *Sg, int64_t ldsg, double *R, int64_t ldr,
+                                                 double *evals, int max_sweeps, double tol, int *info, int precondition,
+                                                 const int *chol_flag, EighScratch<NMAX> &sc) {
+    const int tid = threadIdx.x;
+    const int lane = tid & 63;
+    const int wave = __builtin_amdgcn_readfirstlane(tid >> 6);
+    bool chol_ok = (!IN_LDS && chol_flag) ? (*chol_flag != 0) : false;
+    if (IN_LDS && n >= 4 && max_sweeps > 0 && precondition) {
+        int tx_log2 = 4;
+        while ((1 << tx_log2) < n) ++tx_log2;
+        const int TX = 1 << tx_log2, TY = EIGH_THREADS >> tx_log2;
+        const int tx = tid & (TX - 1), ty = tid >> tx_log2;
+        int fail = 0;
+        for (int j = 0; j < n; ++j) {
+            __syncthreads();
+            const double d = W[j * n + j];
+            if (!(d > 0.0)) {
+                fail = 1;
+                break;
+            }
+            const double invd = 1.0 / d;
+            for (int c = j + 1 + tx; c < n; c += TX) {
+                const double pj = W[j * n + c];
+                for (int i = j + 1 + ty; i <= c; i += TY) W[i * n + c] = fma(-W[j * n + i] * invd, pj, W[i * n + c]);
+            }
+        }
+        __syncthreads();
+        if (!fail) {
+            for (int i = tid; i < n; i += EIGH_THREADS) sc.lam[i] = 1.0 / sqrt(W[i * n + i]);
+            __syncthreads();
+            for (int e = tid; e < n * n; e += EIGH_THREADS) {
+                const int i = e / n, c = e - i * n;
+                W[e] = (c >= i) ? W[e] * sc.lam[i] : 0.0;
+            }
+            chol_ok = true;
+        } else {
+            for (int e = tid; e < n * n; e += EIGH_THREADS) W[e] = Sg[(int64_t)(e / n) * ldsg + (e % n)];
+        }
+        __syncthreads();
+    }
+
+    const int m = (n + 1) & ~1;
+    const double tol2 = tol * tol;
+    int sweep = 0, converged = (n <= 1);
+    for (; sweep < max_sweeps && !converged; ++sweep) {
+        if (tid == 0) sc.rot = 0;
+        __syncthreads();
+        for (int step = 0; step < m - 1; ++step) {
+            for (int k0 = wave * EIGH_PW; k0 < m / 2; k0 += EIGH_WAVES * EIGH_PW) {
+                const int slot = lane >> 4, t = lane & 15;
+                const int k = k0 + slot;
+                bool act = k < m / 2;
+                int p = 0, q = 0;
+                if (act) {
+                    rr_pair(m, step, k, p, q);
+                    act = q < n;
+                }
+                double *wp = W + (int64_t)p * ldw, *wq = W + (int64_t)q * ldw;
+                const bool rot = eigh_pair_step<NC>(wp, wq, n, t, act, tol2);
+                const unsigned long long rb = __ballot(rot && t == 0);
+                if (lane == 0 && rb) atomicAdd(&sc.rot, __popcll(rb));
+            }
+            __syncthreads();
+        }
+        converged = (sc.rot == 0);
+        __syncthreads();
+    }
+
+    for (int i = wave; i < n; i += EIGH_WAVES) {
+        const double *wi = W + (int64_t)i * ldw;
+        double a = 0.0;
+        for (int c = lane; c < n; c += 64) a = fma(wi[c], wi[c], a);
+        a = sqrt(pk_wave_sum(a));
+        if (lane == 0) sc.lam[i] = a;
+    }
+    __syncthreads();
+    if (tid == 0) {
+        double mx = 0.0;
+        for (int i = 0; i < n; ++i) mx = fmax(mx, sc.lam[i]);
+        sc.vec[0] = mx * 1e-100;
+    }
+    __syncthreads();
+    const double noise = sc.vec[0];
+    __syncthreads();
+    for (int i = wave; i < n; i += EIGH_WAVES) {
+        double *wi = W + (int64_t)i * ldw;
+        const double a = sc.lam[i];
+        const bool ok = (a > noise) && (a > 1e-290);
+        const double inv = ok ? 1.0 / a : 0.0;
+        for (int c = lane; c < n; c += 64) wi[c] *= inv;
+        if (lane == 0) sc.rank[i] = ok ? 1 : 0;
+    }
+    __syncthreads();
+    if (chol_ok) {
+        for (int i = tid; i < n; i += EIGH_THREADS) sc.lam[i] *= sc.lam[i];
+        __syncthreads();
+    }
+    for (int i = 0; i < n; ++i) {
+        if (sc.rank[i]) continue;
+        for (int j = 0; j < n; ++j) {
+            for (int c = tid; c < n; c += EIGH_THREADS) {
+                double v = (c == j) ? 1.0 : 0.0;
+                for (int r = 0; r < n; ++r) {
+                    if (!sc.rank[r]) continue;
+                    const double *wr = W + (int64_t)r * ldw;
+                    v -= wr[j] * wr[c];
+                }
+                sc.vec[c] = v;
+            }
+            __syncthreads();
+            if (tid == 0) {
+                double nn = 0.0;
+                for (int c = 0; c < n; ++c) nn += sc.vec[c] * sc.vec[c];
+                sc.flag = (nn > 0.25);
+                if (sc.flag) {
+                    const double inv = 1.0 / sqrt(nn);
+                    double *wi = W + (int64_t)i * ldw;
+                    for (int c = 0; c < n; ++c) wi[c] = sc.vec[c] * inv;
+                    sc.rank[i] = 1;
+                }
+            }
+            __syncthreads();
+            const int done = sc.flag;
+            __syncthreads();
+            if (done) break;
+        }
+    }
+    __syncthreads();
+    for (int i = tid; i < n; i += EIGH_THREADS) {
+        const double li = sc.lam[i];
+        int r = 0;
+        for (int j = 0; j < n; ++j) {
+            const double lj = sc.lam[j];
+            r += (lj > li) || (lj == li && j < i);
+        }
+        sc.rank[i] = r;
+        evals[r] = li;
+    }
+    __syncthreads();
+    for (int i = wave; i < n; i += EIGH_WAVES) {
+        const double *ri = W + (int64_t)i * ldw;
+        double best = 0.0;
+        int bestc = 0x7fffffff;
+        for (int c = lane; c < n; c += 64) {
+            double v = fabs(ri[c]);
+            if (v > best) {
+                best = v;
+                bestc = c;
+            }
+        }
+#pragma unroll
+        for (int off = 32; off > 0; off >>= 1) {
+            double ob = __shfl_xor(best, off, 64);
+            int oc = __shfl_xor(bestc, off, 64);
+            if (ob > best || (ob == best && oc < bestc)) {
+                best = ob;
+                bestc = oc;
+            }
+        }
+        const double sgn = (bestc != 0x7fffffff && ri[bestc] < 0.0) ? -1.0 : 1.0;
+        double *dst = R + (int64_t)sc.rank[i] * ldr;
+        for (int c = lane; c < n; c += 64) dst[c] = sgn * ri[c];
+    }
+    if (tid == 0 && info) {
+        info[0] = sweep;
+        info[1] = converged;
+    }
+}
diff --git a/polara_amd/ops.py b/polara_amd/ops.py
--- a/polara_amd/ops.py
+++ b/polara_amd/ops.py
@@ -1,4 +1,5 @@
 import ctypes as C
+import threading
 
 import numpy as np
 import torch
@@ -341,6 +342,7 @@
         self.seen_dense_tiles = None
         self._info = torch.zeros(2, dtype=torch.int32, device=self.device)
         self._ctx = None
+        self._ctx_lock = threading.Lock()
         self.timers = None
         self.warm_up_s = 0.0
         from . import runtime_info
@@ -864,7 +866,9 @@
                                             _ptr(Z), Z.stride(0), _ptr(out), out.stride(0)), 'pk_tsmm_sub_f64')
         return out
 
-    def sym_eig_topk(self, T, k, X0=None, tol=1e-13, max_outer=200, seed=0, stats=None, lam0=None, r0_rel=-1.0, width=None):
+    takes_eig_band = True
+
+    def sym_eig_topk(self, T, k, X0=None, tol=1e-13, max_outer=200, seed=0, stats=None, lam0=None, r0_rel=-1.0, width=None, band=0):
         n = int(T.shape[0])
         assert T.stride(1) == 1 and T.shape[1] == n
         if X0 is not None:
@@ -883,12 +887,15 @@
         lam = np.zeros(l)
         res = np.zeros(l)
         counts = np.zeros(5, dtype=np.int32)
-        rc = self.lib.pk_sym_eig_topk_f64(self._ctx, self.stream(), n, _ptr(T), T.stride(0), int(k), l,
-                                          _ptr(X0) if X0 is not None else None, l, int(X0.shape[0]) if X0 is not None else 0,
-                                          float(tol), int(max_outer), int(seed) & 0xFFFFFFFFFFFFFFFF, _ptr(basis), l,
-                                          lam.ctypes.data_as(C.c_void_p), res.ctypes.data_as(C.c_void_p),
-                                          counts.ctypes.data_as(C.c_void_p),
-                                          lam0.ctypes.data_as(C.c_void_p) if lam0 is not None else None, float(r0_rel))
+        band = int(band) if 0 < int(band) <= 1024 else 0
+        with self._ctx_lock:
+            if band:
+                _lib.check(self.lib.pk_ctx_set_option(self._ctx, b'eig_band', band), 'pk_ctx_set_option', self.lib, self._ctx)
+            try:
+                rc = self._sym_eig_topk_call(n, T, k, l, X0, tol, max_outer, seed, basis, lam, res, counts, lam0, r0_rel)
+            finally:
+                if band:
+                    self.lib.pk_ctx_set_option(self._ctx, b'eig_band', 0)
         if rc != 0:
             raise RuntimeError('pk_sym_eig_topk_f64: ' + (self.lib.pk_ctx_error(self._ctx) or b'').decode())
         if stats is not None:
@@ -896,6 +903,14 @@
             stats['steps'] = stats.get('steps', 0) + int(counts[4])
         n_lock, n_act = int(counts[0]), int(counts[1])
         return basis[:, :n_lock + n_act], lam[:n_lock + n_act], res[:n_act], n_lock, bool(counts[2])
+
+    def _sym_eig_topk_call(self, n, T, k, l, X0, tol, max_outer, seed, basis, lam, res, counts, lam0, r0_rel):
+        return self.lib.pk_sym_eig_topk_f64(self._ctx, self.stream(), n, _ptr(T), T.stride(0), int(k), l,
+                                          _ptr(X0) if X0 is not None else None, l, int(X0.shape[0]) if X0 is not None else 0,
+                                          float(tol), int(max_outer), int(seed) & 0xFFFFFFFFFFFFFFFF, _ptr(basis), l,
+                                          lam.ctypes.data_as(C.c_void_p), res.ctypes.data_as(C.c_void_p),
+                                          counts.ctypes.data_as(C.c_void_p),
+                                          lam0.ctypes.data_as(C.c_void_p) if lam0 is not None else None, float(r0_rel))
 
     def eigh_top(self, S, r):
         n = int(S.shape[0])
diff --git a/polara_amd/solver.py b/polara_amd/solver.py
--- a/polara_amd/solver.py
+++ b/polara_amd/solver.py
@@ -351,8 +351,10 @@
     if final:
         t_in = 0.3 * est_tol
     r0 = -1.0 if (lam0 is None or prior is None) else float(prior)
+    band = dict(band=2 * b) if getattr(ops, 'takes_eig_band', False) else {}
     while True:
-        basis, lam_all, res_in, n_lock, conv_in = ops.sym_eig_topk(Tj, k, X0, t_in, 200, seed, inner, lam0=lam0, r0_rel=r0, width=cold_width)
+        basis, lam_all, res_in, n_lock, conv_in = ops.sym_eig_topk(Tj, k, X0, t_in, 200, seed, inner, lam0=lam0, r0_rel=r0, width=cold_width,
+                                                                   **band)
         cold_width = None
         lam0, r0 = None, -1.0
         X0 = basis.contiguous()
```

Measured after the change: 187.9 million. Within noise of the previous version (-0.1%).
